# bepu/bepuphysics2

Measured on NVIDIA H100. Metric: constraint-iterations/sec (solver+integrator), higher is better.
Workload: dtype f32

## Files before the change

### bepuphysics2_b200/csrc/bepu_contacts.cuh

```cuda
#pragma once
#include "bepu_device_math.cuh"

namespace BEPU_NS {

constexpr int kLanes = 32;

struct GlobalRows { const float* ptr; };
struct GlobalAcc { float* ptr; };
struct StagedRows { uint32_t addr, bar, parity; };
struct StagedAcc { uint32_t addr; float* ptr; };
BEPU_DI float lds_f32(uint32_t addr) {
    float v;
    asm("ld.shared.f32 %0, [%1];" : "=f"(v) : "r"(addr));
    return v;
}
BEPU_DI void rows_ready(GlobalRows) {}
BEPU_DI void rows_ready(StagedRows p) {
    asm volatile(
        "{\n"
        ".reg .pred p;\n"
        "MBAR_WAIT:\n"
        "mbarrier.try_wait.parity.shared::cta.b64 p, [%0], %1;\n"
        "@p bra MBAR_DONE;\n"
        "bra MBAR_WAIT;\n"
        "MBAR_DONE:\n"
        "}\n" ::"r"(p.bar), "r"(p.parity)
        : "memory");
}
BEPU_DI float ldrow(const float* p, int r) { return __ldcg(p + r * kLanes); }
BEPU_DI float ldrow(GlobalRows p, int r) { return __ldcg(p.ptr + r * kLanes); }
BEPU_DI float ldrow(StagedRows p, int r) { return lds_f32(p.addr + r * (kLanes * 4)); }
template <class PR> BEPU_DI V3 ldrow3(PR p, int r) { return {ldrow(p, r), ldrow(p, r + 1), ldrow(p, r + 2)}; }
template <class PR> BEPU_DI Q4 ldrow4(PR p, int r) { return {ldrow(p, r), ldrow(p, r + 1), ldrow(p, r + 2), ldrow(p, r + 3)}; }
BEPU_DI float ldacc(GlobalAcc a, int r) { return a.ptr[r * kLanes]; }
BEPU_DI void stacc(GlobalAcc a, int r, float v) { a.ptr[r * kLanes] = v; }
BEPU_DI float ldacc(StagedAcc a, int r) { return lds_f32(a.addr + r * (kLanes * 4)); }
BEPU_DI void stacc(StagedAcc a, int r, float v) { __stcs(a.ptr + r * kLanes, v); }

BEPU_DI void penetration_apply(const Inertia& iA, const Inertia& iB, V3 normal, V3 angularA, V3 angularB, float impulse, Velocity& vA, Velocity& vB) {
    V3 dLinA = normal * (impulse * iA.inv_mass);
    V3 dAngA = transform(angularA * impulse, iA.t);
    V3 dLinB = normal * (impulse * iB.inv_mass);
    V3 dAngB = transform(angularB * impulse, iB.t);
    vA.lin = vA.lin + dLinA;
    vA.ang = vA.ang + dAngA;
    vB.lin = vB.lin - dLinB;
    vB.ang = vB.ang + dAngB;
}
BEPU_DI void penetration_warm_start(const Inertia& iA, const Inertia& iB, V3 normal, V3 offsetA, V3 offsetB, float accumulated, Velocity& vA, Velocity& vB) {
    penetration_apply(iA, iB, normal, cross(offsetA, normal), cross(normal, offsetB), accumulated, vA, vB);
}
BEPU_DI void penetration_solve(const Inertia& iA, const Inertia& iB, V3 normal, V3 offsetA, V3 offsetB, float depth, const Springiness& sp, float maxRecovery,
                               float inverseDt, float& accumulated, Velocity& vA, Velocity& vB) {
    V3 angularA = cross(offsetA, normal);
    V3 angularB = cross(normal, offsetB);
    float angularA0 = vector_sandwich(angularA, iA.t);
    float angularB0 = vector_sandwich(angularB, iB.t);
    float linear = iA.inv_mass + iB.inv_mass;
    float effectiveMass = sp.effective_mass_cfm_scale / (linear + angularA0 + angularB0);
    float biasVelocity = fmin_ps(depth * inverseDt, fmin_ps(depth * sp.position_error_to_velocity, maxRecovery));
    float csvaLinear = dot(vA.lin, normal);
    float csvaAngular = dot(vA.ang, angularA);
    float negatedCSVBLinear = dot(vB.lin, normal);
    float csvbAngular = dot(vB.ang, angularB);
    float negatedCSI = accumulated * sp.softness_impulse_scale + (csvaLinear - negatedCSVBLinear + csvaAngular + csvbAngular - biasVelocity) * effectiveMass;
    float previous = accumulated;
    accumulated = fmax_ps(0.0f, accumulated - negatedCSI);
    penetration_apply(iA, iB, normal, angularA, angularB, accumulated - previous, vA, vB);
}
BEPU_DI float updated_depth(float dt, V3 contactOffsetA, V3 offsetB, V3 normal, const Velocity& vA, const Velocity& vB, float depth) {
    V3 contactVelocityA = cross(vA.ang, contactOffsetA) + vA.lin;
    V3 contactOffsetB = contactOffsetA - offsetB;
    V3 contactVelocityB = cross(vB.ang, contactOffsetB) + vB.lin;
    float estimatedDepthChangeVelocity = dot(normal, contactVelocityA - contactVelocityB);
    return depth - estimatedDepthChangeVelocity * dt;
}

BEPU_DI void penetration1_apply(const Inertia& iA, V3 normal, V3 angularA, float impulse, Velocity& vA) {
    V3 dLinA = normal * (impulse * iA.inv_mass);
    V3 dAngA = transform(angularA * impulse, iA.t);
    vA.lin = vA.lin + dLinA;
    vA.ang = vA.ang + dAngA;
}
BEPU_DI void penetration1_solve(const Inertia& iA, V3 normal, V3 offsetA, float depth, const Springiness& sp, float maxRecovery, float inverseDt, float& accumulated,
                                Velocity& vA) {
    V3 angularA = cross(offsetA, normal);
    float angularA0 = vector_sandwich(angularA, iA.t);
    float effectiveMass = sp.effective_mass_cfm_scale / (iA.inv_mass + angularA0);
    float biasVelocity = fmin_ps(depth * inverseDt, fmin_ps(depth * sp.position_error_to_velocity, maxRecovery));
    float csvaLinear = dot(vA.lin, normal);
    float csvaAngular = dot(vA.ang, angularA);
    float negatedCSI = accumulated * sp.softness_impulse_scale + (csvaLinear + csvaAngular - biasVelocity) * effectiveMass;
    float previous = accumulated;
    accumulated = fmax_ps(0.0f, accumulated - negatedCSI);
    penetration1_apply(iA, normal, angularA, accumulated - previous, vA);
}
BEPU_DI float updated_depth1(float dt, V3 contactOffset, V3 normal, const Velocity& v, float depth) {
    V3 contactVelocity = cross(v.ang, contactOffset) + v.lin;
    return depth - dot(normal, contactVelocity) * dt;
}

struct TangentJacobians { M23 linearA, angularA, angularB; };
BEPU_DI TangentJacobians tangent_jacobians(V3 tX, V3 tY, V3 offsetA, V3 offsetB) {
    TangentJacobians j;
    j.linearA = {tX, tY};
    j.angularA = {cross(offsetA, tX), cross(offsetA, tY)};
    j.angularB = {cross(tX, offsetB), cross(tY, offsetB)};
    return j;
}
BEPU_DI void tangent_apply(const TangentJacobians& j, const Inertia& iA, const Inertia& iB, V2 impulse, Velocity& vA, Velocity& vB) {
    V3 linearImpulseA = transform(impulse, j.linearA);
    V3 angularImpulseA = transform(impulse, j.angularA);
    V3 angularImpulseB = transform(impulse, j.angularB);
    vA.lin = vA.lin + linearImpulseA * iA.inv_mass;
    vA.ang = vA.ang + transform(angularImpulseA, iA.t);
    vB.lin = vB.lin - linearImpulseA * iB.inv_mass;
    vB.ang = vB.ang + transform(angularImpulseB, iB.t);
}
BEPU_DI void tangent_solve(V3 tX, V3 tY, V3 offsetA, V3 offsetB, const Inertia& iA, const Inertia& iB, float maximumImpulse, V2& accumulated, Velocity& vA, Velocity& vB) {
    TangentJacobians j = tangent_jacobians(tX, tY, offsetA, offsetB);
    Sym2 linear = sandwich_scale(j.linearA, iA.inv_mass) + sandwich_scale(j.linearA, iB.inv_mass);
    Sym2 angular = matrix_sandwich(j.angularA, iA.t) + matrix_sandwich(j.angularB, iB.t);
    Sym2 effectiveMass = invert(linear + angular);
    V2 csvaLinear = transform_by_transpose(vA.lin, j.linearA);
    V2 csvaAngular = transform_by_transpose(vA.ang, j.angularA);
    V2 csvbLinear = transform_by_transpose(vB.lin, j.linearA);
    V2 csvbAngular = transform_by_transpose(vB.ang, j.angularB);
    V2 csv = (csvbLinear - csvaLinear) - (csvaAngular + csvbAngular);
    V2 csi = transform(csv, effectiveMass);
    V2 previous = accumulated;
    accumulated = accumulated + csi;
    float magnitude = length(accumulated);
    float scl = fmin_ps(1.0f, maximumImpulse / fmax_ps(1e-16f, magnitude));
    accumulated = accumulated * scl;
    tangent_apply(j, iA, iB, accumulated - previous, vA, vB);
}
BEPU_DI void tangent1_apply(const M23& linearA, const M23& angularA, const Inertia& iA, V2 impulse, Velocity& vA) {
    V3 linearImpulseA = transform(impulse, linearA);
    V3 angularImpulseA = transform(impulse, angularA);
    vA.lin = vA.lin + linearImpulseA * iA.inv_mass;
    vA.ang = vA.ang + transform(angularImpulseA, iA.t);
}
BEPU_DI void tangent1_solve(V3 tX, V3 tY, V3 offsetA, const Inertia& iA, float maximumImpulse, V2& accumulated, Velocity& vA) {
    M23 linearA{tX, tY};
    M23 angularA{cross(offsetA, tX), cross(offsetA, tY)};
    Sym2 effectiveMass = invert(sandwich_scale(linearA, iA.inv_mass) + matrix_sandwich(angularA, iA.t));
    V2 csv = transform_by_transpose(vA.lin, linearA) + transform_by_transpose(vA.ang, angularA);
    V2 negativeCSI = transform(csv, effectiveMass);
    V2 previous = accumulated;
    accumulated = accumulated - negativeCSI;
    float magnitude = length(accumulated);
    float scl = fmin_ps(1.0f, maximumImpulse / fmax_ps(1e-16f, magnitude));
    accumulated = accumulated * scl;
    tangent1_apply(linearA, angularA, iA, accumulated - previous, vA);
}

BEPU_DI void twist_apply(V3 axis, const Inertia& iA, const Inertia& iB, float impulse, Velocity& vA, Velocity& vB) {
    V3 worldImpulseA = axis * impulse;
    vA.ang = vA.ang + transform(worldImpulseA, iA.t);
    vB.ang = vB.ang - transform(worldImpulseA, iB.t);
}
BEPU_DI void twist_solve(V3 axis, const Inertia& iA, const Inertia& iB, float maximumImpulse, float& accumulated, Velocity& vA, Velocity& vB) {
    float inverseEffectiveMass = vector_sandwich(axis, iA.t) + vector_sandwich(axis, iB.t);
    float effectiveMass = (0.0f == inverseEffectiveMass) ? 0.0f : 1.0f / inverseEffectiveMass;
    float negatedCSI = (dot(vA.ang, axis) - dot(vB.ang, axis)) * effectiveMass;
    float previous = accumulated;
    accumulated = fmin_ps(maximumImpulse, fmax_ps(-maximumImpulse, accumulated - negatedCSI));
    twist_apply(axis, iA, iB, accumulated - previous, vA, vB);
}
BEPU_DI void twist1_apply(V3 axis, const Inertia& iA, float impulse, Velocity& vA) { vA.ang = vA.ang + transform(axis * impulse, iA.t); }
BEPU_DI void twist1_solve(V3 axis, const Inertia& iA, float maximumImpulse, float& accumulated, Velocity& vA) {
    float angularA = vector_sandwich(axis, iA.t);
    float effectiveMass = (0.0f == angularA) ? 0.0f : 1.0f / angularA;
    float negativeCSI = dot(vA.ang, axis) * effectiveMass;
    float previous = accumulated;
    accumulated = fmin_ps(maximumImpulse, fmax_ps(-maximumImpulse, accumulated - negativeCSI));
    twist1_apply(axis, iA, accumulated - previous, vA);
}

template <int N, bool TwoBody> struct ConvexLayout {
    static constexpr int kOffsetB = 4 * N;
    static constexpr int kNormal = TwoBody ? 4 * N + 3 : 4 * N;
    static constexpr int kFriction = kNormal + 3;
    static constexpr int kAngularFrequency = kNormal + 4;
    static constexpr int kTwiceDampingRatio = kNormal + 5;
    static constexpr int kMaxRecovery = kNormal + 6;
    static constexpr int kPrestepRows = kNormal + 7;
    static constexpr int kImpulseRows = N + 3;
};

template <int N> BEPU_DI V3 friction_center(const V3 (&offs)[N], const float (&depths)[N]) {
    float w[N];
#pragma unroll
    for (int i = 0; i < N; ++i) w[i] = depths[i] < 0.0f ? 0.0f : 1.0f;
    float weightSum = w[0];
#pragma unroll
    for (int i = 1; i < N; ++i) weightSum = weightSum + w[i];
    bool useFallback = weightSum == 0.0f;
    weightSum = useFallback ? (float)N : weightSum;
    float inverseWeightSum = 1.0f / weightSum;
    V3 c[N];
#pragma unroll
    for (int i = 0; i < N; ++i) c[i] = offs[i] * (useFallback ? inverseWeightSum : w[i] * inverseWeightSum);
    if constexpr (N == 2) return c[0] + c[1];
    else if constexpr (N == 3) return (c[0] + c[1]) + c[2];
    else return (c[0] + c[1]) + (c[2] + c[3]);
}

template <int N> struct ConvexTwoBody {
    typedef ConvexLayout<N, true> L;
    static constexpr int kBodies = 2;
    static constexpr int kPrestepRows = L::kPrestepRows;
    static constexpr int kImpulseRows = L::kImpulseRows;
    static constexpr bool kIncremental = true;
    static constexpr bool kNeedsPose = false;

    template <class PR, class AR> BEPU_DI static void warm_start(const Inertia& iA, const Inertia& iB, PR p, AR a, Velocity& vA, Velocity& vB) {
        V3 normal = ldrow3(p, L::kNormal), offsetB = ldrow3(p, L::kOffsetB);
        V3 x, z;
        build_orthonormal_basis(normal, x, z);
        V3 offs[N];
        float depths[N];
#pragma unroll
        for (int i = 0; i < N; ++i) { offs[i] = ldrow3(p, 4 * i); depths[i] = ldrow(p, 4 * i + 3); }
        V3 centerA;
        if constexpr (N == 1) centerA = offs[0]; else centerA = friction_center<N>(offs, depths);
        V3 centerB = centerA - offsetB;
        tangent_apply(tangent_jacobians(x, z, centerA, centerB), iA, iB, V2{ldacc(a, 0), ldacc(a, 1)}, vA, vB);
#pragma unroll 1
        for (int i = 0; i < N; ++i) {
            V3 offset = ldrow3(p, 4 * i);
            penetration_warm_start(iA, iB, normal, offset, offset - offsetB, ldacc(a, 2 + i), vA, vB);
        }
        twist_apply(normal, iA, iB, ldacc(a, N + 2), vA, vB);
    }
    template <class PR, class AR> BEPU_DI static void solve(const Inertia& iA, const Inertia& iB, float dt, float inverseDt, PR p, AR a, Velocity& vA, Velocity& vB) {
        V3 normal = ldrow3(p, L::kNormal), offsetB = ldrow3(p, L::kOffsetB);
        float friction = ldrow(p, L::kFriction), maxRecovery = ldrow(p, L::kMaxRecovery);
        Springiness sp = compute_springiness(ldrow(p, L::kAngularFrequency), ldrow(p, L::kTwiceDampingRatio), dt);
        if constexpr (N > 1) {
            V3 offs[N];
            float depths[N];
#pragma unroll
            for (int i = 0; i < N; ++i) { offs[i] = ldrow3(p, 4 * i); depths[i] = ldrow(p, 4 * i + 3); }
            const V3 centerA = friction_center<N>(offs, depths);
            float penSum = 0.0f, twistSum = 0.0f;
#pragma unroll 1
            for (int i = 0; i < N; ++i) {
                V3 offset = ldrow3(p, 4 * i);
                float pen = ldacc(a, 2 + i);
                penetration_solve(iA, iB, normal, offset, offset - offsetB, ldrow(p, 4 * i + 3), sp, maxRecovery, inverseDt, pen, vA, vB);
                stacc(a, 2 + i, pen);
                const float lever = pen * distance(centerA, offset);
                penSum = i == 0 ? pen : penSum + pen;
                twistSum = i == 0 ? lever : twistSum + lever;
            }
            V3 x, z;
            build_orthonormal_basis(normal, x, z);
            V2 tangent{ldacc(a, 0), ldacc(a, 1)};
            float twist = ldacc(a, N + 2);
            const float premultiplied = (1.0f / N) * friction;
            tangent_solve(x, z, centerA, centerA - offsetB, iA, iB, premultiplied * penSum, tangent, vA, vB);
            twist_solve(normal, iA, iB, premultiplied * twistSum, twist, vA, vB);
            stacc(a, 0, tangent.x);
            stacc(a, 1, tangent.y);
            stacc(a, N + 2, twist);
        } else
        {
        V3 offs[N];
        float depths[N], pen[N];
#pragma unroll
        for (int i = 0; i < N; ++i) { offs[i] = ldrow3(p, 4 * i); depths[i] = ldrow(p, 4 * i + 3); pen[i] = ldacc(a, 2 + i); }
#pragma unroll
        for (int i = 0; i < N; ++i) penetration_solve(iA, iB, normal, offs[i], offs[i] - offsetB, depths[i], sp, maxRecovery, inverseDt, pen[i], vA, vB);
        V3 x, z;
        build_orthonormal_basis(normal, x, z);
        V2 tangent{ldacc(a, 0), ldacc(a, 1)};
        float twist = ldacc(a, N + 2);
        if constexpr (N == 1) {
            float maximumTangentImpulse = friction * pen[0];
            tangent_solve(x, z, offs[0], offs[0] - offsetB, iA, iB, maximumTangentImpulse, tangent, vA, vB);
            float maximumTwistImpulse = friction * pen[0] * fmax_ps(0.0f, depths[0]);
            twist_solve(normal, iA, iB, maximumTwistImpulse, twist, vA, vB);
        } else {
            float premultiplied = (1.0f / N) * friction;
            float penSum = pen[0];
#pragma unroll
            for (int i = 1; i < N; ++i) penSum = penSum + pen[i];
            V3 centerA = friction_center<N>(offs, depths);
            tangent_solve(x, z, centerA, centerA - offsetB, iA, iB, premultiplied * penSum, tangent, vA, vB);
            float twistSum = pen[0] * distance(centerA, offs[0]);
#pragma unroll
            for (int i = 1; i < N; ++i) twistSum = twistSum + pen[i] * distance(centerA, offs[i]);
            twist_solve(normal, iA, iB, premultiplied * twistSum, twist, vA, vB);
        }
        stacc(a, 0, tangent.x);
        stacc(a, 1, tangent.y);
#pragma unroll
        for (int i = 0; i < N; ++i) stacc(a, 2 + i, pen[i]);
        stacc(a, N + 2, twist);
        }
    }
    BEPU_DI static void incremental_update(float dt, const Velocity& vA, const Velocity& vB, float* p) {
        V3 normal = ldrow3(p, L::kNormal), offsetB = ldrow3(p, L::kOffsetB);
#pragma unroll
        for (int i = 0; i < N; ++i) p[(4 * i + 3) * kLanes] = updated_depth(dt, ldrow3(p, 4 * i), offsetB, normal, vA, vB, ldrow(p, 4 * i + 3));
    }
};

template <int N> struct ConvexOneBody {
    typedef ConvexLayout<N, false> L;
    static constexpr int kBodies = 1;
    static constexpr int kPrestepRows = L::kPrestepRows;
    static constexpr int kImpulseRows = L::kImpulseRows;
    static constexpr bool kIncremental = true;
    static constexpr bool kNeedsPose = false;

    template <class PR, class AR> BEPU_DI static void warm_start(const Inertia& iA, PR p, AR a, Velocity& vA) {
        V3 normal = ldrow3(p, L::kNormal);
        V3 x, z;
        build_orthonormal_basis(normal, x, z);
        V3 offs[N];
        float depths[N];
#pragma unroll
        for (int i = 0; i < N; ++i) { offs[i] = ldrow3(p, 4 * i); depths[i] = ldrow(p, 4 * i + 3); }
        V3 centerA;
        if constexpr (N == 1) centerA = offs[0]; else centerA = friction_center<N>(offs, depths);
        tangent1_apply(M23{x, z}, M23{cross(centerA, x), cross(centerA, z)}, iA, V2{ldacc(a, 0), ldacc(a, 1)}, vA);
#pragma unroll 1
        for (int i = 0; i < N; ++i) penetration1_apply(iA, normal, cross(ldrow3(p, 4 * i), normal), ldacc(a, 2 + i), vA);
        twist1_apply(normal, iA, ldacc(a, N + 2), vA);
    }
    template <class PR, class AR> BEPU_DI static void solve(const Inertia& iA, float dt, float inverseDt, PR p, AR a, Velocity& vA) {
        V3 normal = ldrow3(p, L::kNormal);
        float friction = ldrow(p, L::kFriction), maxRecovery = ldrow(p, L::kMaxRecovery);
        Springiness sp = compute_springiness(ldrow(p, L::kAngularFrequency), ldrow(p, L::kTwiceDampingRatio), dt);
        if constexpr (N > 1) {
            V3 offs[N];
            float depths[N];
#pragma unroll
            for (int i = 0; i < N; ++i) { offs[i] = ldrow3(p, 4 * i); depths[i] = ldrow(p, 4 * i + 3); }
            const V3 centerA = friction_center<N>(offs, depths);
            float penSum = 0.0f, twistSum = 0.0f;
#pragma unroll 1
            for (int i = 0; i < N; ++i) {
                V3 offset = ldrow3(p, 4 * i);
                float pen = ldacc(a, 2 + i);
                penetration1_solve(iA, normal, offset, ldrow(p, 4 * i + 3), sp, maxRecovery, inverseDt, pen, vA);
                stacc(a, 2 + i, pen);
                const float lever = pen * distance(centerA, offset);
                penSum = i == 0 ? pen : penSum + pen;
                twistSum = i == 0 ? lever : twistSum + lever;
            }
            V3 x, z;
            build_orthonormal_basis(normal, x, z);
            V2 tangent{ldacc(a, 0), ldacc(a, 1)};
            float twist = ldacc(a, N + 2);
            const float premultiplied = (1.0f / N) * friction;
            tangent1_solve(x, z, centerA, iA, premultiplied * penSum, tangent, vA);
            twist1_solve(normal, iA, premultiplied * twistSum, twist, vA);
            stacc(a, 0, tangent.x);
            stacc(a, 1, tangent.y);
            stacc(a, N + 2, twist);
        } else
        {
        V3 offs[N];
        float depths[N], pen[N];
#pragma unroll
        for (int i = 0; i < N; ++i) { offs[i] = ldrow3(p, 4 * i); depths[i] = ldrow(p, 4 * i + 3); pen[i] = ldacc(a, 2 + i); }
#pragma unroll
        for (int i = 0; i < N; ++i) penetration1_solve(iA, normal, offs[i], depths[i], sp, maxRecovery, inverseDt, pen[i], vA);
        V3 x, z;
        build_orthonormal_basis(normal, x, z);
        V2 tangent{ldacc(a, 0), ldacc(a, 1)};
        float twist = ldacc(a, N + 2);
        if constexpr (N == 1) {
            tangent1_solve(x, z, offs[0], iA, friction * pen[0], tangent, vA);
            twist1_solve(normal, iA, friction * pen[0] * fmax_ps(0.0f, depths[0]), twist, vA);
        } else {
            float premultiplied = (1.0f / N) * friction;
            float penSum = pen[0];
#pragma unroll
            for (int i = 1; i < N; ++i) penSum = penSum + pen[i];
            V3 centerA = friction_center<N>(offs, depths);
            tangent1_solve(x, z, centerA, iA, premultiplied * penSum, tangent, vA);
            float twistSum = pen[0] * distance(centerA, offs[0]);
#pragma unroll
            for (int i = 1; i < N; ++i) twistSum = twistSum + pen[i] * distance(centerA, offs[i]);
            twist1_solve(normal, iA, premultiplied * twistSum, twist, vA);
        }
        stacc(a, 0, tangent.x);
        stacc(a, 1, tangent.y);
#pragma unroll
        for (int i = 0; i < N; ++i) stacc(a, 2 + i, pen[i]);
        stacc(a, N + 2, twist);
        }
    }
    BEPU_DI static void incremental_update(float dt, const Velocity& vA, float* p) {
        V3 normal = ldrow3(p, L::kNormal);
#pragma unroll
        for (int i = 0; i < N; ++i) p[(4 * i + 3) * kLanes] = updated_depth1(dt, ldrow3(p, 4 * i), normal, vA, ldrow(p, 4 * i + 3));
    }
};

#define BEPU_CONTACT_LOOP _Pragma("unroll 1")
template <int N, bool TwoBody> struct NonconvexLayout {
    static constexpr int kOffsetB = 4;
    static constexpr int kContacts = TwoBody ? 7 : 4;
    static constexpr int kPrestepRows = kContacts + 7 * N;
    static constexpr int kImpulseRows = 3 * N;
};
template <int N> struct NonconvexTwoBody {
    typedef NonconvexLayout<N, true> L;
    static constexpr int kBodies = 2;
    static constexpr int kPrestepRows = L::kPrestepRows;
    static constexpr int kImpulseRows = L::kImpulseRows;
    static constexpr bool kIncremental = true;
    static constexpr bool kNeedsPose = false;
    template <class PR, class AR> BEPU_DI static void warm_start(const Inertia& iA, const Inertia& iB, PR p, AR a, Velocity& vA, Velocity& vB) {
        V3 offsetB = ldrow3(p, L::kOffsetB);
BEPU_CONTACT_LOOP
        for (int i = 0; i < N; ++i) {
            const int c = L::kContacts + 7 * i;
            V3 offset = ldrow3(p, c), normal = ldrow3(p, c + 4);
            V3 x, z;
            build_orthonormal_basis(normal, x, z);
            V3 contactOffsetB = offset - offsetB;
            tangent_apply(tangent_jacobians(x, z, offset, contactOffsetB), iA, iB, V2{ldacc(a, 3 * i), ldacc(a, 3 * i + 1)}, vA, vB);
            penetration_warm_start(iA, iB, normal, offset, contactOffsetB, ldacc(a, 3 * i + 2), vA, vB);
        }
    }
    template <class PR, class AR> BEPU_DI static void solve(const Inertia& iA, const Inertia& iB, float dt, float inverseDt, PR p, AR a, Velocity& vA, Velocity& vB) {
        V3 offsetB = ldrow3(p, L::kOffsetB);
        float friction = ldrow(p, 0), maxRecovery = ldrow(p, 3);
        Springiness sp = compute_springiness(ldrow(p, 1), ldrow(p, 2), dt);
BEPU_CONTACT_LOOP
        for (int i = 0; i < N; ++i) {
            const int c = L::kContacts + 7 * i;
            V3 offset = ldrow3(p, c), normal = ldrow3(p, c + 4);
            float depth = ldrow(p, c + 3);
            V2 tangent{ldacc(a, 3 * i), ldacc(a, 3 * i + 1)};
            float pen = ldacc(a, 3 * i + 2);
            V3 contactOffsetB = offset - offsetB;
            penetration_solve(iA, iB, normal, offset, contactOffsetB, depth, sp, maxRecovery, inverseDt, pen, vA, vB);
            V3 x, z;
            build_orthonormal_basis(normal, x, z);
            tangent_solve(x, z, offset, contactOffsetB, iA, iB, friction * pen, tangent, vA, vB);
            stacc(a, 3 * i, tangent.x);
            stacc(a, 3 * i + 1, tangent.y);
            stacc(a, 3 * i + 2, pen);
        }
    }
    BEPU_DI static void incremental_update(float dt, const Velocity& vA, const Velocity& vB, float* p) {
        V3 offsetB = ldrow3(p, L::kOffsetB);
#pragma unroll
        for (int i = 0; i < N; ++i) {
            const int c = L::kContacts + 7 * i;
            p[(c + 3) * kLanes] = updated_depth(dt, ldrow3(p, c), offsetB, ldrow3(p, c + 4), vA, vB, ldrow(p, c + 3));
        }
    }
};
template <int N> struct NonconvexOneBody {
    typedef NonconvexLayout<N, false> L;
    static constexpr int kBodies = 1;
    static constexpr int kPrestepRows = L::kPrestepRows;
    static constexpr int kImpulseRows = L::kImpulseRows;
    static constexpr bool kIncremental = true;
    static constexpr bool kNeedsPose = false;
    template <class PR, class AR> BEPU_DI static void warm_start(const Inertia& iA, PR p, AR a, Velocity& vA) {
BEPU_CONTACT_LOOP
        for (int i = 0; i < N; ++i) {
            const int c = L::kContacts + 7 * i;
            V3 offset = ldrow3(p, c), normal = ldrow3(p, c + 4);
            V3 x, z;
            build_orthonormal_basis(normal, x, z);
            tangent1_apply(M23{x, z}, M23{cross(offset, x), cross(offset, z)}, iA, V2{ldacc(a, 3 * i), ldacc(a, 3 * i + 1)}, vA);
            penetration1_apply(iA, normal, cross(offset, normal), ldacc(a, 3 * i + 2), vA);
        }
    }
    template <class PR, class AR> BEPU_DI static void solve(const Inertia& iA, float dt, float inverseDt, PR p, AR a, Velocity& vA) {
        float friction = ldrow(p, 0), maxRecovery = ldrow(p, 3);
        Springiness sp = compute_springiness(ldrow(p, 1), ldrow(p, 2), dt);
BEPU_CONTACT_LOOP
        for (int i = 0; i < N; ++i) {
            const int c = L::kContacts + 7 * i;
            V3 offset = ldrow3(p, c), normal = ldrow3(p, c + 4);
            float depth = ldrow(p, c + 3);
            V2 tangent{ldacc(a, 3 * i), ldacc(a, 3 * i + 1)};
            float pen = ldacc(a, 3 * i + 2);
            penetration1_solve(iA, normal, offset, depth, sp, maxRecovery, inverseDt, pen, vA);
            V3 x, z;
            build_orthonormal_basis(normal, x, z);
            tangent1_solve(x, z, offset, iA, friction * pen, tangent, vA);
            stacc(a, 3 * i, tangent.x);
            stacc(a, 3 * i + 1, tangent.y);
            stacc(a, 3 * i + 2, pen);
        }
    }
    BEPU_DI static void incremental_update(float dt, const Velocity& vA, float* p) {
#pragma unroll
        for (int i = 0; i < N; ++i) {
            const int c = L::kContacts + 7 * i;
            p[(c + 3) * kLanes] = updated_depth1(dt, ldrow3(p, c), ldrow3(p, c + 4), vA, ldrow(p, c + 3));
        }
    }
};

}
```

### bepuphysics2_b200/csrc/bepu_device_types.h

```cpp
#pragma once
#include <cuda_runtime.h>
#include <stdint.h>

namespace bepucuda {

constexpr uint32_t kRefIndexMask = 0x0FFFFFFFu;
constexpr uint32_t kRefBundleIntegratesBit = 1u << 28;
constexpr uint32_t kRefIntegrateBit = 1u << 29;
constexpr uint32_t kRefKinematicBit = 1u << 30;
constexpr int32_t kRefEmpty = -1;

struct BodyBuffers {
    float4* pose;
    float4* velocity;
    float4* inertia_local;
    float4* inertia_world;
    const uint8_t* constrained;
    int32_t count;
};

struct DeviceTypeBatch {
    int32_t type_id;
    int32_t bundle_count;
    int32_t device_batch;
    int32_t pad;
    int32_t* refs;
    float* prestep;
    float* impulses;
};

struct FrameParams {
    float dt;
    float inverse_dt;
    float gravity_dt[3];
    float linear_damping_dt;
    float angular_damping_dt;
    float final_dt;
    float final_gravity_dt[3];
    float final_linear_damping_dt;
    float final_angular_damping_dt;
    int32_t final_steps;
    int32_t angular_mode;
    int32_t integrate_velocity_for_kinematics;
    uint32_t exchange_base;
    uint32_t shard_solve_index;
    int32_t tune[4];
};

enum Stage : int32_t {
    kStageWarmStartFirst = 0,
    kStageWarmStart = 1,
    kStageSolve = 2,
    kStageIncremental = 3,
    kStageKinematicFirst = 4,
    kStageKinematic = 5,
    kStageFinalPose = 6,
};

struct WorkItem {
    int32_t type_batch;
    int32_t bundle;
};

struct alignas(32) WorkRecord {
    int32_t* refs;
    float* prestep;
    float* impulses;
    int32_t type_id;
    int32_t live_lanes;
};

struct StageOp {
    int32_t stage;
    int32_t work_begin;
    int32_t work_count;
    int32_t pad;
};

constexpr int kMaxShardRanks = 8;
struct ShardPeers {
    float4* pose[kMaxShardRanks];
    float4* velocity[kMaxShardRanks];
    float4* inertia_world[kMaxShardRanks];
    unsigned long long* flags[kMaxShardRanks];
    int32_t rank, rank_count;
};
struct ShardStage {
    uint32_t exchange_index;
    int32_t* error_flag;
};
constexpr int kShardCounterSlot = 16;
constexpr int kShardTargetSlot = 32;
constexpr int kShardMaxExchanges = 4096;
constexpr size_t kShardFlagBlockWords = kShardTargetSlot + (size_t)kMaxShardRanks * kShardMaxExchanges;
constexpr int32_t kRecordBoundaryBit = 1 << 30;
constexpr uint32_t kPushOwnerBit = 1u << 31;

struct TypeInfo {
    int32_t bodies, prestep_rows, impulse_rows, incremental;
    int32_t solve_bytes, warm_start_bytes, incremental_bytes;
    const char* name;
};
const TypeInfo* get_type_info(int type_id);

}
```

### bepuphysics2_b200/csrc/bepu_layout_kernels.h

```cpp
#pragma once
#include "bepu_device_types.h"

namespace bepucuda {

void launch_split_bodies(const void* raw, int body_count, const BodyBuffers& B, cudaStream_t s);
void launch_merge_bodies(void* raw, int body_count, const BodyBuffers& B, cudaStream_t s);
struct TransposeDesc {
    int32_t* src_refs;
    float* src_prestep;
    float* src_impulses;
    const int32_t* map;
    int32_t src_count;
    int32_t bodies, prestep_rows, impulse_rows;
    int32_t src_bundle_base;
    int32_t flags;
    const int32_t* features_old;
    const int32_t* features_new;
};
constexpr int32_t kDescResidentImpulses = 1, kDescRedistribute = 2;
enum { kTransposeRefs = 1, kTransposePrestep = 2, kTransposeImpulses = 4 };
void launch_transpose_in_all(const DeviceTypeBatch* tbs, const TransposeDesc* descs, const WorkItem* work, int work_count, int W, int what, cudaStream_t s);
void launch_transpose_out_all(const DeviceTypeBatch* tbs, const TransposeDesc* descs, const WorkItem* work, int work_count, int W, int what, cudaStream_t s);
void launch_fill_i32(int32_t* p, size_t n, int32_t v, cudaStream_t s);
void launch_redistribute_impulses(const DeviceTypeBatch* tbs, const TransposeDesc* descs, const WorkItem* work, int work_count, cudaStream_t s);
void launch_scatter_body_motion(const void* raw, int body_count, const BodyBuffers& B, cudaStream_t s);
void launch_gather_body_motion(void* raw, int body_count, const BodyBuffers& B, cudaStream_t s);
struct CopyChunk {
    void* dst;
    const void* src;
    size_t bytes;
};
void launch_batched_copy(const CopyChunk* chunks, int chunk_count, cudaStream_t s);
void launch_ownership_pass1(const DeviceTypeBatch* tbs, const WorkItem* work, int work_count, const int32_t* bodies_per_type, int sync_batch_count, int body_count,
                            int32_t* first_batch, int32_t* sync_refcount, unsigned long long* sync_mask, int32_t* error_flag, cudaStream_t s);
void launch_ownership_rest(const DeviceTypeBatch* tbs, const WorkItem* work, int work_count, const int32_t* bodies_per_type, int body_count, const int32_t* first_batch,
                           const int32_t* sync_refcount, const unsigned long long* sync_mask, uint8_t* constrained, const int32_t* kinematics, int kinematic_count,
                           int32_t* error_flag, const TransposeDesc* descs, int W, int32_t* source_bundle_flags, cudaStream_t s);
void launch_collect_stage(const DeviceTypeBatch* tbs, const WorkItem* work, int work_count, const int32_t* bodies_per_type, int stage, const BodyBuffers& B, int32_t* staging,
                          cudaStream_t s);
void launch_apply_stage(const int32_t* staging, int planes, const BodyBuffers& B, cudaStream_t s);
void launch_widen_u8(const uint8_t* in, int32_t* out, size_t n, cudaStream_t s);
void launch_narrow_i32(const int32_t* in, uint8_t* out, size_t n, cudaStream_t s);

void launch_shard_exchange(const uint32_t* pushes, int push_count, int what, const BodyBuffers& B, const ShardPeers& peers, const FrameParams* fp, uint32_t exchange_index,
                           int32_t* error_flag, cudaStream_t s);

void launch_fill_peer_masks(const int32_t* refs, uint32_t* peer_masks, size_t count, const uint8_t* body_masks, int rank, cudaStream_t s);
void launch_boundary_flags(const WorkRecord* records, int count, const int32_t* bodies_per_type, long long peer_delta, uint8_t* flags, cudaStream_t s);

void launch_pack_ref_rows(const WorkRecord* records, int count, int32_t* rows, cudaStream_t s);

constexpr int kLaunchPdl = 1, kLaunchPrefetchRows = 2;
struct SolverLaunchers {
    void (*constraint_stage)(int stage, const WorkRecord* records, const int32_t* ref_rows, int work_count, const BodyBuffers& B, const FrameParams* fp, int launch_flags, cudaStream_t s);
    void (*kinematic_stage)(int stage, const int32_t* kinematics, int count, const BodyBuffers& B, const FrameParams* fp, cudaStream_t s);
    void (*final_pose)(const BodyBuffers& B, const FrameParams* fp, cudaStream_t s);
    void (*constraint_stage_sharded)(int stage, const WorkRecord* records, const int32_t* ref_rows, int work_count, const BodyBuffers& B, const FrameParams* fp, int launch_flags, const ShardPeers& peers,
                                     long long peer_delta, const ShardStage& shard, cudaStream_t s);
};
const SolverLaunchers* get_launchers_bepu_fast();
const SolverLaunchers* get_launchers_bepu_strict();

}
```

### bepuphysics2_b200/csrc/bepu_solver_kernels.cu

```cuda
#include <atomic>
#include "bepu_solver_kernels.cuh"
#include "bepu_layout_kernels.h"

namespace BEPU_NS {

void launch_stage_warm_start_first(const WorkRecord* records, const int32_t* ref_rows, int work_count, const BodyBuffers& B, const FrameParams* fp, int launch_flags, cudaStream_t s);
void launch_stage_warm_start(const WorkRecord* records, const int32_t* ref_rows, int work_count, const BodyBuffers& B, const FrameParams* fp, int launch_flags, cudaStream_t s);
void launch_stage_solve(const WorkRecord* records, const int32_t* ref_rows, int work_count, const BodyBuffers& B, const FrameParams* fp, int launch_flags, cudaStream_t s);
void launch_stage_warm_start_first_sharded(const WorkRecord* records, const int32_t* ref_rows, int work_count, const BodyBuffers& B, const FrameParams* fp, int launch_flags, const ShardPeers& peers, long long peer_delta, const ShardStage& shard, cudaStream_t s);
void launch_stage_warm_start_sharded(const WorkRecord* records, const int32_t* ref_rows, int work_count, const BodyBuffers& B, const FrameParams* fp, int launch_flags, const ShardPeers& peers, long long peer_delta, const ShardStage& shard, cudaStream_t s);
void launch_stage_solve_sharded(const WorkRecord* records, const int32_t* ref_rows, int work_count, const BodyBuffers& B, const FrameParams* fp, int launch_flags, const ShardPeers& peers, long long peer_delta, const ShardStage& shard, cudaStream_t s);

#ifndef BEPU_DEEP_MINB
#define BEPU_DEEP_MINB 12
#endif
constexpr int kDeepBatchBundles = 2150;
template <int STAGE, int MINB>
static void launch_stage_variant(const WorkRecord* records, const int32_t* ref_rows, int work_count, const BodyBuffers& B, const FrameParams* fp, int launch_flags, cudaStream_t s) {
    static std::atomic<bool> carveout_set[64] = {};
    int device = 0;
    cudaGetDevice(&device);
    if (!carveout_set[device & 63]) {
        cudaFuncSetAttribute(constraint_stage_kernel<STAGE, MINB>, cudaFuncAttributePreferredSharedMemoryCarveout, cudaSharedmemCarveoutMaxShared);
        carveout_set[device & 63] = true;
    }
    const unsigned blocks = (unsigned)(((size_t)work_count * 32 + kStageBlockThreads - 1) / kStageBlockThreads);
    cudaLaunchConfig_t cfg{};
    cfg.gridDim = dim3(blocks);
    cfg.blockDim = dim3(kStageBlockThreads);
    cfg.dynamicSmemBytes = 0;
    cfg.stream = s;
    cudaLaunchAttribute attr[1];
    attr[0].id = cudaLaunchAttributeProgrammaticStreamSerialization;
    attr[0].val.programmaticStreamSerializationAllowed = 1;
    cfg.attrs = attr;
    cfg.numAttrs = (launch_flags & bepucuda::kLaunchPdl) ? 1 : 0;
    cudaLaunchKernelEx(&cfg, constraint_stage_kernel<STAGE, MINB>, records, ref_rows, work_count, B, fp, (launch_flags & bepucuda::kLaunchPrefetchRows) ? kStagePrefetchRows : 0);
}
template <int STAGE, int MINB>
static void launch_stage_variant_sharded(const WorkRecord* records, const int32_t* ref_rows, int work_count, const BodyBuffers& B, const FrameParams* fp, int launch_flags, const ShardPeers& peers, long long peer_delta,
                                         const ShardStage& shard, cudaStream_t s) {
    static std::atomic<bool> carveout_set[64] = {};
    int device = 0;
    cudaGetDevice(&device);
    if (!carveout_set[device & 63]) {
        cudaFuncSetAttribute(constraint_stage_kernel_sharded<STAGE, MINB>, cudaFuncAttributePreferredSharedMemoryCarveout, cudaSharedmemCarveoutMaxShared);
        carveout_set[device & 63] = true;
    }
    const unsigned blocks = (unsigned)(((size_t)work_count * 32 + kStageBlockThreads - 1) / kStageBlockThreads);
    cudaLaunchConfig_t cfg{};
    cfg.gridDim = dim3(blocks);
    cfg.blockDim = dim3(kStageBlockThreads);
    cfg.stream = s;
    cudaLaunchAttribute attr[1];
    attr[0].id = cudaLaunchAttributeProgrammaticStreamSerialization;
    attr[0].val.programmaticStreamSerializationAllowed = 1;
    cfg.attrs = attr;
    cfg.numAttrs = (launch_flags & bepucuda::kLaunchPdl) ? 1 : 0;
    cudaLaunchKernelEx(&cfg, constraint_stage_kernel_sharded<STAGE, MINB>, records, ref_rows, work_count, B, fp, (launch_flags & bepucuda::kLaunchPrefetchRows) ? kStagePrefetchRows : 0, peers,
                       peer_delta, shard);
}
template <int STAGE>
static void launch_stage_sharded_t(const WorkRecord* records, const int32_t* ref_rows, int work_count, const BodyBuffers& B, const FrameParams* fp, int launch_flags, const ShardPeers& peers, long long peer_delta,
                                   const ShardStage& shard, cudaStream_t s) {
    if (work_count >= kDeepBatchBundles) launch_stage_variant_sharded<STAGE, BEPU_DEEP_MINB>(records, ref_rows, work_count, B, fp, launch_flags, peers, peer_delta, shard, s);
    else launch_stage_variant_sharded<STAGE, 1>(records, ref_rows, work_count, B, fp, launch_flags, peers, peer_delta, shard, s);
}
template <int STAGE>
static void launch_stage_t(const WorkRecord* records, const int32_t* ref_rows, int work_count, const BodyBuffers& B, const FrameParams* fp, int launch_flags, cudaStream_t s) {
    if (STAGE != kStageIncremental && work_count >= kDeepBatchBundles) launch_stage_variant<STAGE, BEPU_DEEP_MINB>(records, ref_rows, work_count, B, fp, launch_flags, s);
    else launch_stage_variant<STAGE, 1>(records, ref_rows, work_count, B, fp, launch_flags, s);
}

#if BEPU_UNIT == 0
void launch_stage_warm_start_first(const WorkRecord* records, const int32_t* ref_rows, int work_count, const BodyBuffers& B, const FrameParams* fp, int launch_flags, cudaStream_t s) {
    launch_stage_t<kStageWarmStartFirst>(records, ref_rows, work_count, B, fp, launch_flags, s);
}
void launch_stage_warm_start_first_sharded(const WorkRecord* records, const int32_t* ref_rows, int work_count, const BodyBuffers& B, const FrameParams* fp, int launch_flags, const ShardPeers& peers, long long peer_delta, const ShardStage& shard, cudaStream_t s) {
    launch_stage_sharded_t<kStageWarmStartFirst>(records, ref_rows, work_count, B, fp, launch_flags, peers, peer_delta, shard, s);
}
#elif BEPU_UNIT == 1
void launch_stage_warm_start(const WorkRecord* records, const int32_t* ref_rows, int work_count, const BodyBuffers& B, const FrameParams* fp, int launch_flags, cudaStream_t s) {
    launch_stage_t<kStageWarmStart>(records, ref_rows, work_count, B, fp, launch_flags, s);
}
void launch_stage_warm_start_sharded(const WorkRecord* records, const int32_t* ref_rows, int work_count, const BodyBuffers& B, const FrameParams* fp, int launch_flags, const ShardPeers& peers, long long peer_delta, const ShardStage& shard, cudaStream_t s) {
    launch_stage_sharded_t<kStageWarmStart>(records, ref_rows, work_count, B, fp, launch_flags, peers, peer_delta, shard, s);
}
#elif BEPU_UNIT == 2
void launch_stage_solve(const WorkRecord* records, const int32_t* ref_rows, int work_count, const BodyBuffers& B, const FrameParams* fp, int launch_flags, cudaStream_t s) {
    launch_stage_t<kStageSolve>(records, ref_rows, work_count, B, fp, launch_flags, s);
}
void launch_stage_solve_sharded(const WorkRecord* records, const int32_t* ref_rows, int work_count, const BodyBuffers& B, const FrameParams* fp, int launch_flags, const ShardPeers& peers, long long peer_delta, const ShardStage& shard, cudaStream_t s) {
    launch_stage_sharded_t<kStageSolve>(records, ref_rows, work_count, B, fp, launch_flags, peers, peer_delta, shard, s);
}
#elif BEPU_UNIT == 3
static void launch_constraint_stage(int stage, const WorkRecord* records, const int32_t* ref_rows, int work_count, const BodyBuffers& B, const FrameParams* fp, int launch_flags, cudaStream_t s) {
    if (work_count <= 0) return;
    switch (stage) {
        case kStageWarmStartFirst: launch_stage_warm_start_first(records, ref_rows, work_count, B, fp, launch_flags, s); break;
        case kStageWarmStart: launch_stage_warm_start(records, ref_rows, work_count, B, fp, launch_flags, s); break;
        case kStageSolve: launch_stage_solve(records, ref_rows, work_count, B, fp, launch_flags, s); break;
        case kStageIncremental: launch_stage_t<kStageIncremental>(records, ref_rows, work_count, B, fp, launch_flags, s); break;
        default: break;
    }
}
static void launch_constraint_stage_sharded(int stage, const WorkRecord* records, const int32_t* ref_rows, int work_count, const BodyBuffers& B, const FrameParams* fp, int launch_flags, const ShardPeers& peers,
                                            long long peer_delta, const ShardStage& shard, cudaStream_t s) {
    if (work_count <= 0) return;
    switch (stage) {
        case kStageWarmStartFirst: launch_stage_warm_start_first_sharded(records, ref_rows, work_count, B, fp, launch_flags, peers, peer_delta, shard, s); break;
        case kStageWarmStart: launch_stage_warm_start_sharded(records, ref_rows, work_count, B, fp, launch_flags, peers, peer_delta, shard, s); break;
        case kStageSolve: launch_stage_solve_sharded(records, ref_rows, work_count, B, fp, launch_flags, peers, peer_delta, shard, s); break;
        default: break;
    }
}
static void launch_kinematic_stage(int stage, const int32_t* kinematics, int count, const BodyBuffers& B, const FrameParams* fp, cudaStream_t s) {
    if (count <= 0) return;
    const unsigned blocks = (unsigned)((count + 127) / 128);
    if (stage == kStageKinematicFirst) kinematic_stage_kernel<kStageKinematicFirst><<<blocks, 128, 0, s>>>(kinematics, count, B, fp);
    else kinematic_stage_kernel<kStageKinematic><<<blocks, 128, 0, s>>>(kinematics, count, B, fp);
}
static void launch_final_pose(const BodyBuffers& B, const FrameParams* fp, cudaStream_t s) {
    if (B.count <= 0) return;
    final_pose_kernel<<<(unsigned)((B.count + 255) / 256), 256, 0, s>>>(B, fp);
}
static const bepucuda::SolverLaunchers kLaunchers = {&launch_constraint_stage, &launch_kinematic_stage, &launch_final_pose, &launch_constraint_stage_sharded};
#else
#error "BEPU_UNIT must be 0..3"
#endif

}

#if BEPU_UNIT == 3
namespace bepucuda {
#define BEPU_CAT2(a, b) a##b
#define BEPU_CAT(a, b) BEPU_CAT2(a, b)
const SolverLaunchers* BEPU_CAT(get_launchers_, BEPU_NS)() { return &BEPU_NS::kLaunchers; }
}
#endif
```

### bepuphysics2_b200/csrc/bepu_solver_kernels.cuh

```cuda
#pragma once
#include "bepu_contacts.cuh"
#include "bepu_joints_more.cuh"
#include "bepu_integration.cuh"
#include "bepu_device_types.h"

namespace BEPU_NS {

using namespace bepucuda;

struct F8 { float a, b, c, d, e, f, g, h; };
#define BEPU_BODY_LD "ld.global.L1::no_allocate.L2::cache_hint.v4.f32"
#define BEPU_BODY_ST "st.global.L1::no_allocate.L2::cache_hint.v4.f32"
BEPU_DI uint64_t l2_evict_last_policy() {
    uint64_t policy;
    asm("createpolicy.fractional.L2::evict_last.b64 %0, 1.0;" : "=l"(policy));
    return policy;
}
BEPU_DI F8 ld256(const float4* p) {
    F8 r;
    asm volatile(BEPU_BODY_LD " {%0,%1,%2,%3}, [%8], %9;\n\t" BEPU_BODY_LD " {%4,%5,%6,%7}, [%8+16], %9;"
                 : "=f"(r.a), "=f"(r.b), "=f"(r.c), "=f"(r.d), "=f"(r.e), "=f"(r.f), "=f"(r.g), "=f"(r.h)
                 : "l"(p), "l"(l2_evict_last_policy())
                 : "memory");
    return r;
}
BEPU_DI void st256(float4* p, float a, float b, float c, float d, float e, float f, float g, float h) {
    asm volatile(BEPU_BODY_ST " [%0], {%1,%2,%3,%4}, %9;\n\t" BEPU_BODY_ST " [%0+16], {%5,%6,%7,%8}, %9;" ::"l"(p), "f"(a), "f"(b), "f"(c), "f"(d), "f"(e), "f"(f), "f"(g), "f"(h),
                 "l"(l2_evict_last_policy())
                 : "memory");
}
BEPU_DI void load_velocity(const float4* vel, uint32_t i, Velocity& v) {
    const F8 r = ld256(vel + 2 * (size_t)i);
    v.lin = {r.a, r.b, r.c};
    v.ang = {r.e, r.f, r.g};
}
BEPU_DI void store_velocity(float4* vel, uint32_t i, const Velocity& v) { st256(vel + 2 * (size_t)i, v.lin.x, v.lin.y, v.lin.z, 0.0f, v.ang.x, v.ang.y, v.ang.z, 0.0f); }
BEPU_DI void load_inertia(const float4* in, uint32_t i, Inertia& r) {
    const F8 x = ld256(in + 2 * (size_t)i);
    r.t = {x.a, x.b, x.c, x.d, x.e, x.f};
    r.inv_mass = x.g;
}
BEPU_DI void store_inertia(float4* in, uint32_t i, const Inertia& r) { st256(in + 2 * (size_t)i, r.t.xx, r.t.yx, r.t.yy, r.t.zx, r.t.zy, r.t.zz, r.inv_mass, 0.0f); }
BEPU_DI void load_pose(const float4* pose, uint32_t i, V3& pos, Q4& q) {
    const F8 x = ld256(pose + 2 * (size_t)i);
    q = {x.a, x.b, x.c, x.d};
    pos = {x.e, x.f, x.g};
}
BEPU_DI void store_pose(float4* pose, uint32_t i, V3 pos, Q4 q) { st256(pose + 2 * (size_t)i, q.x, q.y, q.z, q.w, pos.x, pos.y, pos.z, 0.0f); }

template <int STAGE, bool NeedsPose>
BEPU_DI void warm_start_body(uint32_t enc, const BodyBuffers& B, const FrameParams& fp, BodyState& b, Velocity& v) {
    const uint32_t idx = enc & kRefIndexMask;
    if (enc & kRefIntegrateBit) {
        Inertia local;
        load_inertia(B.inertia_local, idx, local);
        load_pose(B.pose, idx, b.pos, b.q);
        b.inertia.inv_mass = local.inv_mass;
        if (STAGE == kStageWarmStart) {
            b.pos = b.pos + v.lin * fp.dt;
            Q4 previousOrientation = b.q;
            b.q = integrate_orientation(b.q, v.ang, fp.dt * 0.5f);
            b.inertia.t = rotate_inverse_inertia(local.t, b.q);
            if (fp.angular_mode == 1) integrate_angular_conserve_momentum(previousOrientation, local.t, b.inertia.t, v.ang);
            else if (fp.angular_mode == 2) integrate_angular_gyroscopic(b.q, local.t, v.ang, fp.dt);
            store_pose(B.pose, idx, b.pos, b.q);
        } else {
            b.inertia.t = rotate_inverse_inertia(local.t, b.q);
            if (fp.angular_mode == 1) {
                Q4 previousOrientation = integrate_orientation(b.q, v.ang, fp.dt * -0.5f);
                integrate_angular_conserve_momentum(previousOrientation, local.t, b.inertia.t, v.ang);
            } else if (fp.angular_mode == 2) {
                integrate_angular_gyroscopic(b.q, local.t, v.ang, fp.dt);
            }
        }
        callback_integrate_velocity(v, fp.gravity_dt[0], fp.gravity_dt[1], fp.gravity_dt[2], fp.linear_damping_dt, fp.angular_damping_dt);
        store_inertia(B.inertia_world, idx, b.inertia);
    } else {
        load_inertia(B.inertia_world, idx, b.inertia);
        if (NeedsPose) load_pose(B.pose, idx, b.pos, b.q);
        if (STAGE == kStageWarmStartFirst && fp.angular_mode != 0 && (enc & kRefBundleIntegratesBit) && !(enc & kRefKinematicBit)) {
            Inertia local;
            load_inertia(B.inertia_local, idx, local);
            V3 pos;
            Q4 q;
            load_pose(B.pose, idx, pos, q);
            if (fp.angular_mode == 1) integrate_angular_conserve_momentum(integrate_orientation(q, v.ang, fp.dt * -0.5f), local.t, b.inertia.t, v.ang);
            else integrate_angular_gyroscopic(q, local.t, v.ang, fp.dt);
        }
    }
}
template <int STAGE, bool NeedsPose>
BEPU_DI void gather_for_warm_start(uint32_t enc, const BodyBuffers& B, const FrameParams& fp, BodyState& b, Velocity& v) {
    load_velocity(B.velocity, enc & kRefIndexMask, v);
    warm_start_body<STAGE, NeedsPose>(enc, B, fp, b, v);
}

template <class T, class PR, class AR> BEPU_DI void call_warm_start(const BodyState* b, PR p, AR a, Velocity* v) {
    if constexpr (T::kNeedsPose) T::warm_start(b, p, a, v);
    else if constexpr (T::kBodies == 2) T::warm_start(b[0].inertia, b[1].inertia, p, a, v[0], v[1]);
    else T::warm_start(b[0].inertia, p, a, v[0]);
}
template <class T, class PR, class AR> BEPU_DI void call_solve(const BodyState* b, float dt, float inverseDt, PR p, AR a, Velocity* v) {
    if constexpr (T::kNeedsPose) T::solve(b, dt, inverseDt, p, a, v);
    else if constexpr (T::kBodies == 2) T::solve(b[0].inertia, b[1].inertia, dt, inverseDt, p, a, v[0], v[1]);
    else T::solve(b[0].inertia, dt, inverseDt, p, a, v[0]);
}
template <class T> BEPU_DI void call_incremental(float dt, const Velocity* v, float* p) {
    if constexpr (T::kIncremental) {
        if constexpr (T::kBodies == 2) T::incremental_update(dt, v[0], v[1], p);
        else T::incremental_update(dt, v[0], p);
    }
}

BEPU_DI uint32_t ldg_nc_u32(const void* p) {
    uint32_t v;
    asm volatile("ld.global.nc.u32 %0, [%1];" : "=r"(v) : "l"(p));
    return v;
}
BEPU_DI void push_record(float4* const* arrays, uint32_t mask, uint32_t idx, float a, float b, float c, float d, float e, float f, float g, float h) {
    while (mask) {
        const int q = __ffs((int)mask) - 1;
        mask &= mask - 1u;
        float4* dst = arrays[q] + 2 * (size_t)idx;
        dst[0] = make_float4(a, b, c, d);
        dst[1] = make_float4(e, f, g, h);
    }
}
template <class T, int STAGE, bool kSharded, class PR, class AR>
BEPU_DI void run_lane(const int32_t* refs, PR p, AR a, float* p_rw, uint32_t enc0, uint32_t enc1, const BodyBuffers& B, const FrameParams& fp, const ShardPeers* peers = nullptr,
                      long long peer_delta = 0) {
    constexpr int NB = T::kBodies;
    uint32_t enc[NB];
    enc[0] = enc0;
    if constexpr (NB > 1) enc[1] = enc1;
#pragma unroll
    for (int s = 2; s < NB; ++s) enc[s] = (uint32_t)__ldg(refs + s * kLanes);
    uint32_t push_to[kSharded ? NB : 1];
    if constexpr (kSharded) {
#pragma unroll
        for (int s = 0; s < NB; ++s) push_to[s] = peer_delta != 0 ? ldg_nc_u32(refs + peer_delta + s * kLanes) : 0u;
    }
    if ((int32_t)enc[0] == kRefEmpty) return;
    BodyState b[NB];
    Velocity v[NB];
    if constexpr (STAGE == kStageIncremental) {
#pragma unroll
        for (int s = 0; s < NB; ++s) load_velocity(B.velocity, enc[s] & kRefIndexMask, v[s]);
        call_incremental<T>(fp.dt, v, p_rw);
    } else if constexpr (STAGE == kStageSolve) {
#pragma unroll
        for (int s = 0; s < NB; ++s) {
            const uint32_t idx = enc[s] & kRefIndexMask;
            load_velocity(B.velocity, idx, v[s]);
            load_inertia(B.inertia_world, idx, b[s].inertia);
            if (T::kNeedsPose) load_pose(B.pose, idx, b[s].pos, b[s].q);
        }
        rows_ready(p);
        call_solve<T>(b, fp.dt, fp.inverse_dt, p, a, v);
#pragma unroll
        for (int s = 0; s < NB; ++s)
            if (!(enc[s] & kRefKinematicBit)) {
                store_velocity(B.velocity, enc[s] & kRefIndexMask, v[s]);
                if constexpr (kSharded) {
                    const uint32_t mask = push_to[s];
                    if (mask) push_record(peers->velocity, mask, enc[s] & kRefIndexMask, v[s].lin.x, v[s].lin.y, v[s].lin.z, 0.0f, v[s].ang.x, v[s].ang.y, v[s].ang.z, 0.0f);
                }
            }
    } else {
#pragma unroll
        for (int s = 0; s < NB; ++s) gather_for_warm_start<STAGE, T::kNeedsPose>(enc[s], B, fp, b[s], v[s]);
        rows_ready(p);
        call_warm_start<T>(b, p, a, v);
#pragma unroll
        for (int s = 0; s < NB; ++s)
            if (!(enc[s] & kRefKinematicBit)) {
                const uint32_t idx = enc[s] & kRefIndexMask;
                store_velocity(B.velocity, idx, v[s]);
                if constexpr (kSharded) {
                    const uint32_t mask = push_to[s];
                    if (mask) {
                        push_record(peers->velocity, mask, idx, v[s].lin.x, v[s].lin.y, v[s].lin.z, 0.0f, v[s].ang.x, v[s].ang.y, v[s].ang.z, 0.0f);
                        if (enc[s] & kRefIntegrateBit) {
                            const Inertia& in = b[s].inertia;
                            push_record(peers->inertia_world, mask, idx, in.t.xx, in.t.yx, in.t.yy, in.t.zx, in.t.zy, in.t.zz, in.inv_mass, 0.0f);
                            if (STAGE == kStageWarmStart) push_record(peers->pose, mask, idx, b[s].q.x, b[s].q.y, b[s].q.z, b[s].q.w, b[s].pos.x, b[s].pos.y, b[s].pos.z, 0.0f);
                        }
                    }
                }
            }
    }
}
template <class T, int STAGE, class PR, class AR>
BEPU_DI void run_lane(const int32_t* refs, PR p, AR a, float* p_rw, uint32_t enc0, uint32_t enc1, const BodyBuffers& B, const FrameParams& fp) {
    run_lane<T, STAGE, false>(refs, p, a, p_rw, enc0, enc1, B, fp);
}

BEPU_DI int4 ldg_nc_v4(const void* p) {
    int4 v;
    asm volatile("ld.global.nc.v4.s32 {%0,%1,%2,%3}, [%4];" : "=r"(v.x), "=r"(v.y), "=r"(v.z), "=r"(v.w) : "l"(p));
    return v;
}
BEPU_DI WorkRecord load_record(const WorkRecord* r) {
    const int4 lo = ldg_nc_v4(r), hi = ldg_nc_v4(reinterpret_cast<const int4*>(r) + 1);
    WorkRecord w;
    w.refs = reinterpret_cast<int32_t*>((unsigned long long)(unsigned int)lo.x | ((unsigned long long)(unsigned int)lo.y << 32));
    w.prestep = reinterpret_cast<float*>((unsigned long long)(unsigned int)lo.z | ((unsigned long long)(unsigned int)lo.w << 32));
    w.impulses = reinterpret_cast<float*>((unsigned long long)(unsigned int)hi.x | ((unsigned long long)(unsigned int)hi.y << 32));
    w.type_id = hi.z;
    w.live_lanes = hi.w;
    return w;
}

#define BEPU_CONTACT_TYPES(X)                                                                                                     \
    X(0, ConvexOneBody<1>) X(1, ConvexOneBody<2>) X(2, ConvexOneBody<3>) X(3, ConvexOneBody<4>)                                   \
    X(4, ConvexTwoBody<1>) X(5, ConvexTwoBody<2>) X(6, ConvexTwoBody<3>) X(7, ConvexTwoBody<4>)                                   \
    X(8, NonconvexOneBody<2>) X(9, NonconvexOneBody<3>) X(10, NonconvexOneBody<4>)                                                \
    X(15, NonconvexTwoBody<2>) X(16, NonconvexTwoBody<3>) X(17, NonconvexTwoBody<4>)

template <int STAGE, bool kSharded, class PR, class AR>
BEPU_DI void run_bundle_rows(const WorkRecord& rec, int lane, PR p, AR a, uint32_t enc0, uint32_t enc1, const BodyBuffers& B, const FrameParams& fp, const ShardPeers* peers = nullptr,
                             long long peer_delta = 0) {
    const int32_t* refs = rec.refs + lane;
    float* p_rw = rec.prestep + lane;
    switch (rec.type_id) {
#define BEPU_CASE(ID, T) \
    case ID: run_lane<T, STAGE, kSharded>(refs, p, a, p_rw, enc0, enc1, B, fp, peers, peer_delta); break;
        BEPU_CONTACT_TYPES(BEPU_CASE)
        BEPU_JOINT_TYPES(BEPU_CASE)
        BEPU_JOINT_TYPES_MORE(BEPU_CASE)
#undef BEPU_CASE
        default: break;
    }
}
template <int STAGE, class PR, class AR>
BEPU_DI void run_bundle_rows(const WorkRecord& rec, int lane, PR p, AR a, uint32_t enc0, uint32_t enc1, const BodyBuffers& B, const FrameParams& fp) {
    run_bundle_rows<STAGE, false>(rec, lane, p, a, enc0, enc1, B, fp);
}
template <int STAGE>
BEPU_DI void run_bundle(const WorkRecord& rec, int lane, uint32_t enc0, uint32_t enc1, const BodyBuffers& B, const FrameParams& fp) {
    run_bundle_rows<STAGE>(rec, lane, GlobalRows{rec.prestep + lane}, GlobalAcc{rec.impulses + lane}, enc0, enc1, B, fp);
}
template <int STAGE> BEPU_DI void run_bundle(const WorkRecord& rec, int lane, const BodyBuffers& B, const FrameParams& fp) {
    const uint32_t enc0 = ldg_nc_u32(rec.refs + lane), enc1 = ldg_nc_u32(rec.refs + kLanes + lane);
    run_bundle<STAGE>(rec, lane, enc0, enc1, B, fp);
}

struct StageRowCounts { uint8_t prestep[64], impulses[64]; };
__host__ __device__ constexpr StageRowCounts make_stage_row_counts() {
    StageRowCounts c{};
#define BEPU_ROWS(ID, T) c.prestep[ID] = (uint8_t)T::kPrestepRows; c.impulses[ID] = (uint8_t)T::kImpulseRows;
    BEPU_CONTACT_TYPES(BEPU_ROWS)
    BEPU_JOINT_TYPES(BEPU_ROWS)
    BEPU_JOINT_TYPES_MORE(BEPU_ROWS)
#undef BEPU_ROWS
    return c;
}
__constant__ StageRowCounts kStageRowCounts = make_stage_row_counts();
constexpr int kStageSlabRows = 48;
constexpr int kStageSlabBytes = kStageSlabRows * kLanes * 4;

BEPU_DI uint32_t smem_u32(const void* p) { return (uint32_t)__cvta_generic_to_shared(p); }
BEPU_DI void mbar_init(uint32_t bar, uint32_t count) {
    asm volatile("mbarrier.init.shared::cta.b64 [%0], %1;" ::"r"(bar), "r"(count) : "memory");
    asm volatile("fence.mbarrier_init.release.cluster;" ::: "memory");
    asm volatile("fence.proxy.async.shared::cta;" ::: "memory");
}
BEPU_DI void mbar_expect_tx(uint32_t bar, uint32_t bytes) { asm volatile("mbarrier.arrive.expect_tx.shared::cta.b64 _, [%0], %1;" ::"r"(bar), "r"(bytes) : "memory"); }
BEPU_DI uint64_t l2_evict_first_policy() {
    uint64_t policy;
    asm volatile("createpolicy.fractional.L2::evict_first.b64 %0, 1.0;" : "=l"(policy));
    return policy;
}
BEPU_DI void bulk_copy_g2s(uint32_t dst, const void* src, uint32_t bytes, uint32_t bar, uint64_t policy) {
    asm volatile("cp.async.bulk.shared::cluster.global.mbarrier::complete_tx::bytes.L2::cache_hint [%0], [%1], %2, [%3], %4;" ::"r"(dst), "l"(src), "r"(bytes), "r"(bar),
                 "l"(policy)
                 : "memory");
}

#ifndef BEPU_STAGE_BLOCK_THREADS
#define BEPU_STAGE_BLOCK_THREADS 64
#endif
constexpr int kStageBlockThreads = BEPU_STAGE_BLOCK_THREADS;

constexpr int kStagePrefetchRows = 1;
BEPU_DI void shard_announce(const ShardPeers& peers, int lane) {
    if (lane < peers.rank_count && lane != peers.rank)
        asm volatile("red.release.sys.global.add.u64 [%0], 1;" ::"l"(peers.flags[lane] + kShardCounterSlot + peers.rank) : "memory");
}
BEPU_DI void shard_wait(const ShardPeers& peers, int lane, uint32_t solve_index, uint32_t exchange_point, int32_t* error_flag) {
    if (lane < peers.rank_count && lane != peers.rank) {
        const unsigned long long* mine = peers.flags[peers.rank];
        const unsigned long long* targets = mine + kShardTargetSlot + (size_t)lane * kShardMaxExchanges;
        const unsigned long long want = (unsigned long long)solve_index * targets[kShardMaxExchanges - 1] + targets[exchange_point];
        unsigned long long seen;
        unsigned int spins = 0;
        do {
            asm volatile("ld.acquire.sys.global.u64 %0, [%1];" : "=l"(seen) : "l"(mine + kShardCounterSlot + lane) : "memory");
        } while (seen < want && ++spins < 100000000u);
        if (seen < want) atomicExch(error_flag, 5);
    }
    __syncwarp();
}
template <int STAGE, bool kSharded>
BEPU_DI void constraint_stage_body(const WorkRecord* __restrict__ records, const int32_t* __restrict__ ref_rows, int work_count, const BodyBuffers& B, const FrameParams* __restrict__ fpp, int flags, const ShardPeers* peers,
                                   long long peer_delta, const ShardStage* shard = nullptr) {
    constexpr bool kStaged = STAGE != kStageIncremental;
    constexpr int kWarps = kStageBlockThreads / 32;
    __shared__ __align__(128) float slab[kStaged ? kWarps * kStageSlabRows * kLanes : 1];
    __shared__ __align__(8) unsigned long long bars[kWarps];
    const int warp_in_block = threadIdx.x >> 5;
    const int global_warp = (blockIdx.x * kStageBlockThreads + threadIdx.x) >> 5;
    const int lane = threadIdx.x & 31;
    WorkRecord rec{};
    uint32_t enc0 = (uint32_t)kRefEmpty, enc1 = 0;
    const int warp = global_warp;
    const bool active = warp < work_count;
    const uint32_t slab_addr = kStaged ? smem_u32(slab) + warp_in_block * kStageSlabBytes : 0;
    const uint32_t bar = smem_u32(&bars[warp_in_block]);
    const bool early_rows = kStaged && (flags & kStagePrefetchRows);
    uint32_t prestep_bytes = 0, impulse_bytes = 0;
    if (active) {
        rec = load_record(records + warp);
        if constexpr (kStaged) {
            prestep_bytes = kStageRowCounts.prestep[rec.type_id] * (kLanes * 4);
            impulse_bytes = kStageRowCounts.impulses[rec.type_id] * (kLanes * 4);
            if (lane == 0) {
                mbar_init(bar, 1);
                if (early_rows) {
                    const uint64_t policy = l2_evict_first_policy();
                    mbar_expect_tx(bar, prestep_bytes + impulse_bytes);
                    bulk_copy_g2s(slab_addr, rec.prestep, prestep_bytes, bar, policy);
                    bulk_copy_g2s(slab_addr + prestep_bytes, rec.impulses, impulse_bytes, bar, policy);
                }
            }
        }
        enc0 = ldg_nc_u32(ref_rows + (size_t)warp * (2 * kLanes) + lane);
        enc1 = ldg_nc_u32(ref_rows + (size_t)warp * (2 * kLanes) + kLanes + lane);
    }
    const FrameParams fp = *fpp;
    asm volatile("griddepcontrol.wait;" ::: "memory");
    asm volatile("griddepcontrol.launch_dependents;");
    bool boundary = false;
    if constexpr (kSharded) {
        boundary = active && (rec.live_lanes & kRecordBoundaryBit) != 0;
        if (boundary && shard->exchange_index > 0 && !(fp.tune[0] & 1)) shard_wait(*peers, lane, fp.shard_solve_index, shard->exchange_index - 1u, shard->error_flag);
    }
    if (!active) return;
    if constexpr (kStaged) {
        if (!early_rows && lane == 0) {
            const uint64_t policy = l2_evict_first_policy();
            mbar_expect_tx(bar, prestep_bytes + impulse_bytes);
            bulk_copy_g2s(slab_addr, rec.prestep, prestep_bytes, bar, policy);
            bulk_copy_g2s(slab_addr + prestep_bytes, rec.impulses, impulse_bytes, bar, policy);
        }
        __syncwarp();
        run_bundle_rows<STAGE, kSharded>(rec, lane, StagedRows{slab_addr + lane * 4, bar, 0u}, StagedAcc{slab_addr + prestep_bytes + lane * 4, rec.impulses + lane}, enc0, enc1, B, fp,
                                         peers, boundary && !(fp.tune[0] & 4) ? peer_delta : 0);
        if constexpr (kSharded) {
            if (boundary && !(fp.tune[0] & 2)) {
                __syncwarp();
                shard_announce(*peers, lane);
            }
        }
    } else {
        run_bundle<STAGE>(rec, lane, enc0, enc1, B, fp);
    }
}

template <int STAGE, int MINB>
__global__ void __launch_bounds__(kStageBlockThreads, MINB) constraint_stage_kernel(const WorkRecord* __restrict__ records, const int32_t* __restrict__ ref_rows, int work_count, BodyBuffers B, const FrameParams* __restrict__ fpp, int flags) {
    constraint_stage_body<STAGE, false>(records, ref_rows, work_count, B, fpp, flags, nullptr, 0);
}
template <int STAGE, int MINB>
__global__ void __launch_bounds__(kStageBlockThreads, MINB)
constraint_stage_kernel_sharded(const WorkRecord* __restrict__ records, const int32_t* __restrict__ ref_rows, int work_count, BodyBuffers B, const FrameParams* __restrict__ fpp, int flags, const __grid_constant__ ShardPeers peers,
                                long long peer_delta, const __grid_constant__ ShardStage shard) {
    constraint_stage_body<STAGE, true>(records, ref_rows, work_count, B, fpp, flags, &peers, peer_delta, &shard);
}

template <int STAGE> BEPU_DI void run_kinematic(int i, const int32_t* kinematics, const BodyBuffers& B, const FrameParams& fp) {
    const uint32_t idx = (uint32_t)kinematics[i];
    Velocity v;
    load_velocity(B.velocity, idx, v);
    if (STAGE == kStageKinematic) {
        V3 pos;
        Q4 q;
        load_pose(B.pose, idx, pos, q);
        pos = pos + v.lin * fp.dt;
        q = integrate_orientation(q, v.ang, fp.dt * 0.5f);
        store_pose(B.pose, idx, pos, q);
    }
    if (fp.integrate_velocity_for_kinematics) {
        callback_integrate_velocity(v, fp.gravity_dt[0], fp.gravity_dt[1], fp.gravity_dt[2], fp.linear_damping_dt, fp.angular_damping_dt);
        store_velocity(B.velocity, idx, v);
    }
}
template <int STAGE>
__global__ void kinematic_stage_kernel(const int32_t* __restrict__ kinematics, int count, BodyBuffers B, const FrameParams* __restrict__ fpp) {
    const int i = blockIdx.x * blockDim.x + threadIdx.x;
    if (i >= count) return;
    const FrameParams fp = *fpp;
    run_kinematic<STAGE>(i, kinematics, B, fp);
}

BEPU_DI void run_final_pose(int i, const BodyBuffers& B, const FrameParams& fp) {
    V3 pos;
    Q4 q;
    Velocity v;
    load_pose(B.pose, i, pos, q);
    load_velocity(B.velocity, i, v);
    if (B.constrained[i]) {
        q = integrate_orientation(q, v.ang, fp.dt * 0.5f);
        pos = pos + v.lin * fp.dt;
        store_pose(B.pose, i, pos, q);
        return;
    }
    Inertia local;
    load_inertia(B.inertia_local, i, local);
    const bool kinematic = local.inv_mass == 0.0f && local.t.xx == 0.0f && local.t.yx == 0.0f && local.t.yy == 0.0f && local.t.zx == 0.0f && local.t.zy == 0.0f && local.t.zz == 0.0f;
    const bool integrateVelocity = fp.integrate_velocity_for_kinematics || !kinematic;
    const float dt = fp.final_dt, halfDt = fp.final_dt * 0.5f;
    for (int step = 0; step < fp.final_steps; ++step) {
        if (integrateVelocity)
            callback_integrate_velocity(v, fp.final_gravity_dt[0], fp.final_gravity_dt[1], fp.final_gravity_dt[2], fp.final_linear_damping_dt, fp.final_angular_damping_dt);
        pos = pos + v.lin * dt;
        if (fp.angular_mode == 1) {
            Q4 previousOrientation = q;
            q = integrate_orientation(q, v.ang, halfDt);
            integrate_angular_conserve_momentum(previousOrientation, local.t, rotate_inverse_inertia(local.t, q), v.ang);
        } else if (fp.angular_mode == 2) {
            q = integrate_orientation(q, v.ang, halfDt);
            integrate_angular_gyroscopic(q, local.t, v.ang, dt);
        } else {
            q = integrate_orientation(q, v.ang, halfDt);
        }
    }
    store_pose(B.pose, i, pos, q);
    if (integrateVelocity) store_velocity(B.velocity, i, v);
}
static __global__ void final_pose_kernel(BodyBuffers B, const FrameParams* __restrict__ fpp) {
    const int i = blockIdx.x * blockDim.x + threadIdx.x;
    if (i >= B.count) return;
    const FrameParams fp = *fpp;
    run_final_pose(i, B, fp);
}

}
```

### bepuphysics2_b200/csrc/bepucuda_api.cu

```cuda
#include <algorithm>
#include <cmath>
#include <cstdio>
#include <cstdlib>
#include <cstring>
#include <map>
#include <string>
#include <vector>

#include "../../include/bepucuda.h"
#include "bepu_layout_kernels.h"
#include "bepu_coloring.h"
#include "bepu_bounds.h"

using namespace bepucuda;

namespace bepucuda {

static TypeInfo make_contact(int bodies, int prestep, int impulses, int contacts, const char* name) {
    TypeInfo t{};
    t.bodies = bodies; t.prestep_rows = prestep; t.impulse_rows = impulses; t.incremental = 1; t.name = name;
    const int body_rw = 13 + 6;
    t.solve_bytes = 4 * (prestep + 2 * impulses + bodies + bodies * body_rw);
    t.warm_start_bytes = 4 * (prestep + impulses + bodies + bodies * body_rw);
    t.incremental_bytes = 4 * (prestep + contacts + bodies + 6 * bodies);
    return t;
}
static TypeInfo make_joint(int bodies, int prestep, int impulses, int solve_r, int solve_w, int ws_r, int ws_w, const char* name) {
    TypeInfo t{};
    t.bodies = bodies; t.prestep_rows = prestep; t.impulse_rows = impulses; t.incremental = 0; t.name = name;
    t.solve_bytes = 4 * (prestep + 2 * impulses + bodies + solve_r + solve_w);
    t.warm_start_bytes = 4 * (prestep + impulses + bodies + ws_r + ws_w);
    t.incremental_bytes = 0;
    return t;
}
struct Registry {
    TypeInfo types[64];
    bool present[64];
    Registry() {
        std::memset(present, 0, sizeof(present));
        auto add = [&](int id, TypeInfo t) { types[id] = t; present[id] = true; };
        add(0, make_contact(1, 11, 4, 1, "Contact1OneBody")); add(1, make_contact(1, 15, 5, 2, "Contact2OneBody"));
        add(2, make_contact(1, 19, 6, 3, "Contact3OneBody")); add(3, make_contact(1, 23, 7, 4, "Contact4OneBody"));
        add(4, make_contact(2, 14, 4, 1, "Contact1")); add(5, make_contact(2, 18, 5, 2, "Contact2"));
        add(6, make_contact(2, 22, 6, 3, "Contact3")); add(7, make_contact(2, 26, 7, 4, "Contact4"));
        add(8, make_contact(1, 18, 6, 2, "Contact2NonconvexOneBody")); add(9, make_contact(1, 25, 9, 3, "Contact3NonconvexOneBody"));
        add(10, make_contact(1, 32, 12, 4, "Contact4NonconvexOneBody"));
        add(15, make_contact(2, 21, 6, 2, "Contact2Nonconvex")); add(16, make_contact(2, 28, 9, 3, "Contact3Nonconvex"));
        add(17, make_contact(2, 35, 12, 4, "Contact4Nonconvex"));
#define BEPU_REGISTER_JOINTS
#include "bepu_joint_registry.inc"
#undef BEPU_REGISTER_JOINTS
    }
};
static const Registry& registry() {
    static Registry r;
    return r;
}
const TypeInfo* get_type_info(int type_id) {
    if (type_id < 0 || type_id >= 64 || !registry().present[type_id]) return nullptr;
    return &registry().types[type_id];
}

struct DeviceBuffer {
    void* ptr = nullptr;
    size_t capacity = 0;
    cudaError_t reserve(size_t bytes) {
        if (bytes <= capacity) return cudaSuccess;
        if (ptr) cudaFree(ptr);
        ptr = nullptr;
        capacity = 0;
        size_t want = bytes + bytes / 4 + 256;
        cudaError_t e = cudaMalloc(&ptr, want);
        if (e == cudaSuccess) capacity = want;
        return e;
    }
    void release() {
        if (ptr) cudaFree(ptr);
        ptr = nullptr;
        capacity = 0;
    }
    template <class T> T* as() const { return (T*)ptr; }
};

struct ChunkArena {
    struct Chunk { char* base; size_t size, used; };
    std::vector<Chunk> chunks;
    bool pinned_host = false;
    size_t min_chunk = (size_t)64 << 20;
    void reset() { for (auto& c : chunks) c.used = 0; }
    void* alloc(size_t bytes, cudaError_t* err) {
        bytes = (bytes + 255) & ~(size_t)255;
        for (auto& c : chunks)
            if (c.size - c.used >= bytes) {
                void* p = c.base + c.used;
                c.used += bytes;
                return p;
            }
        Chunk c{};
        c.size = std::max(bytes, min_chunk);
        cudaError_t e = pinned_host ? cudaMallocHost((void**)&c.base, c.size) : cudaMalloc((void**)&c.base, c.size);
        if (e != cudaSuccess) { if (err) *err = e; return nullptr; }
        c.used = bytes;
        chunks.push_back(c);
        return chunks.back().base;
    }
    void release() {
        for (auto& c : chunks) { if (pinned_host) cudaFreeHost(c.base); else cudaFree(c.base); }
        chunks.clear();
    }
};

struct SourceTypeBatch {
    int batch_index, type_batch_index, type_id, count;
    int live = 0;
    float* host_impulses;
    int32_t* raw_refs;
    float* raw_prestep;
    float* raw_impulses;
    size_t refs_bytes, prestep_bytes, impulse_bytes;
    std::vector<int32_t> host_refs;
    std::vector<int> device_tbs;
    int32_t* raw_features_old = nullptr;
    int32_t* raw_features_new = nullptr;
    size_t feature_bytes = 0;
    bool resident_impulses = false, redistribute = false;
};

}

struct bepucuda_ctx {
    bepucuda_config cfg{};
    int32_t tune[4] = {0, 0, 0, 0};
    int device = 0;
    cudaStream_t stream = nullptr;
    cudaEvent_t ev_solve_begin = nullptr, ev_solve_end = nullptr, ev_up_begin = nullptr, ev_up_end = nullptr, ev_down_begin = nullptr, ev_down_end = nullptr;
    bool up_open = false, have_solve = false, have_down = false, have_up = false;
    std::string error;
    const SolverLaunchers* launchers = nullptr;

    std::vector<int32_t> iterations{1};
    int fallback_threshold = 64;
    bepucuda_integrator_desc integ{};
    bool integ_set = false;

    int body_count = 0;
    DeviceBuffer raw_bodies, pose, velocity, inertia_local, inertia_world, constrained, first_batch, sync_refcount, sync_mask;
    BodyBuffers B{};

    int W = 8;
    int batch_count = 0;
    bool constraints_open = false, constraints_ready = false, data_dirty = false, descs_dirty = false;
    std::vector<SourceTypeBatch> sources;
    ChunkArena raw_arena, pinned_arena;
    DeviceBuffer record_table, ref_rows, source_bundle_flags, refs32, prestep32, impulses32, tb_table, tdesc_table, work_table, map_table, bodies_per_type, kinematics_dev, program_dev, frame_params_dev, error_dev;
    std::vector<DeviceTypeBatch> tbs;
    std::vector<TransposeDesc> tdescs;
    std::vector<WorkItem> work;
    std::vector<int32_t> bundle_live;
    std::vector<WorkRecord> records;
    std::vector<std::pair<int, int>> batch_work;
    bool exchange_failed = false;
    bepucuda_exchange_fn exchange = nullptr;
    void* exchange_user = nullptr;
    DeviceBuffer exchange_staging;
    bool peer_mode = false;
    ShardPeers peers{};
    DeviceBuffer shard_flags, pushes_dev, peer32, body_masks_dev, boundary_flags_dev;
    uint32_t shard_solve_index = 0;
    std::vector<int> boundary_count;
    std::vector<uint8_t> body_masks;
    size_t refs_words = 0;
    std::vector<void*> opened_ipc;
    std::vector<int32_t> global_first_batch;
    std::vector<uint8_t> global_constrained;
    std::map<int, std::vector<uint32_t>> pushes_by_batch;
    std::vector<std::pair<size_t, int>> push_range;
    uint32_t exchange_counter = 0;
    uint32_t exchanges_per_solve = 0;
    int inc_work_begin = 0, inc_work_count = 0;
    int all_work_count = 0;
    int sync_batch_count = 0, fallback_levels = 0;
    std::vector<int32_t> kinematics;
    std::vector<StageOp> program;
    FrameParams* frame_params_host = nullptr;

    cudaGraph_t graph = nullptr;
    cudaGraphExec_t graph_exec = nullptr;
    bool graph_valid = false;

    bepucuda_timings timings{};
    int64_t h2d_accum = 0;
    struct HostRange { char* host; size_t bytes; char* dev; };
    std::vector<HostRange> host_ranges;
    std::vector<CopyChunk> pending_h2d;
    DeviceBuffer chunk_table;
    struct ChunkStage { void* host = nullptr; size_t capacity = 0; cudaEvent_t done = nullptr; };
    ChunkStage chunk_stage[4];
    int chunk_stage_next = 0;
    cudaEvent_t user_events[16] = {};
    DeviceBuffer body_shapes, body_activities, body_bounds;
    int shape_count = -1;
    DeviceBuffer color_refs, color_priorities, color_body_min, color_body_mask, color_out, color_lists, color_counts;
    std::vector<cudaEvent_t> profile_events;
};

namespace {

int fail(bepucuda_ctx* c, int code, const std::string& msg) {
    if (c) c->error = msg;
    return code;
}
int cuda_fail(bepucuda_ctx* c, cudaError_t e, const char* what) {
    return fail(c, e == cudaErrorMemoryAllocation ? BEPUCUDA_ERR_OUT_OF_MEMORY : BEPUCUDA_ERR_CUDA, std::string(what) + ": " + cudaGetErrorString(e));
}
#define CK(call)                                                  \
    do {                                                          \
        cudaError_t _e = (call);                                  \
        if (_e != cudaSuccess) return cuda_fail(ctx, _e, #call);  \
    } while (0)

void open_upload_window(bepucuda_ctx* ctx) {
    if (!ctx->up_open) {
        cudaEventRecord(ctx->ev_up_begin, ctx->stream);
        ctx->up_open = true;
    }
}

char* map_host(bepucuda_ctx* ctx, const void* ptr, size_t bytes) {
    const char* p = (const char*)ptr;
    for (auto& r : ctx->host_ranges)
        if (p >= r.host && p + bytes <= r.host + r.bytes) return r.dev + (p - r.host);
    return nullptr;
}
void queue_chunks(std::vector<CopyChunk>& list, void* dst, const void* src, size_t bytes) {
    const size_t kChunk = (size_t)64 << 10;
    for (size_t off = 0; off < bytes; off += kChunk) list.push_back({(char*)dst + off, (const char*)src + off, std::min(kChunk, bytes - off)});
}
int flush_chunks(bepucuda_ctx* ctx, std::vector<CopyChunk>& list) {
    if (list.empty()) return BEPUCUDA_OK;
    const size_t bytes = list.size() * sizeof(CopyChunk);
    CK(ctx->chunk_table.reserve(bytes));
    auto& st = ctx->chunk_stage[ctx->chunk_stage_next];
    ctx->chunk_stage_next = (ctx->chunk_stage_next + 1) & 3;
    if (!st.done) CK(cudaEventCreateWithFlags(&st.done, cudaEventDisableTiming));
    CK(cudaEventSynchronize(st.done));
    if (st.capacity < bytes) {
        if (st.host) cudaFreeHost(st.host);
        st.host = nullptr;
        st.capacity = 0;
        CK(cudaMallocHost(&st.host, bytes * 2));
        st.capacity = bytes * 2;
    }
    std::memcpy(st.host, list.data(), bytes);
    CK(cudaMemcpyAsync(ctx->chunk_table.ptr, st.host, bytes, cudaMemcpyHostToDevice, ctx->stream));
    launch_batched_copy(ctx->chunk_table.as<CopyChunk>(), (int)list.size(), ctx->stream);
    CK(cudaGetLastError());
    CK(cudaEventRecord(st.done, ctx->stream));
    list.clear();
    return BEPUCUDA_OK;
}

int copy_in(bepucuda_ctx* ctx, void* dst, const void* src, size_t bytes) {
    if (bytes == 0) return BEPUCUDA_OK;
    if (char* alias = map_host(ctx, src, bytes)) {
        queue_chunks(ctx->pending_h2d, dst, alias, bytes);
        ctx->h2d_accum += (int64_t)bytes;
        return BEPUCUDA_OK;
    }
    if (bytes < ((size_t)256 << 10)) {
        cudaError_t e = cudaSuccess;
        void* stage = ctx->pinned_arena.alloc(bytes, &e);
        if (!stage) return cuda_fail(ctx, e, "pinned staging");
        std::memcpy(stage, src, bytes);
        CK(cudaMemcpyAsync(dst, stage, bytes, cudaMemcpyHostToDevice, ctx->stream));
    } else {
        CK(cudaMemcpyAsync(dst, src, bytes, cudaMemcpyHostToDevice, ctx->stream));
    }
    ctx->h2d_accum += (int64_t)bytes;
    return BEPUCUDA_OK;
}

void invalidate_graph(bepucuda_ctx* ctx) {
    if (ctx->graph_exec) cudaGraphExecDestroy(ctx->graph_exec);
    if (ctx->graph) cudaGraphDestroy(ctx->graph);
    ctx->graph_exec = nullptr;
    ctx->graph = nullptr;
    ctx->graph_valid = false;
}

void issue_stage_sequence(bepucuda_ctx* ctx, cudaStream_t s, int64_t* launches) {
    const WorkRecord* records = ctx->record_table.as<WorkRecord>();
    const int32_t* ref_rows = ctx->ref_rows.as<int32_t>();
    const FrameParams* fp = ctx->frame_params_dev.as<FrameParams>();
    const int32_t* kin = ctx->kinematics_dev.as<int32_t>();
    int64_t n = 0;
    const bool pdl = ctx->cfg.reserved[1] == 0;
    const StageOp* previous = nullptr;
    uint32_t exchange_index = 0;
    const bool fused_pushes = ctx->peer_mode && !ctx->body_masks.empty();
    for (const StageOp& op : ctx->program) {
        if (ctx->peer_mode && op.pad == -1) {
            launch_shard_exchange(nullptr, 0, 1, ctx->B, ctx->peers, fp, exchange_index++, ctx->error_dev.as<int32_t>(), s);
            ++n;
            continue;
        }
        if (ctx->peer_mode && op.pad >= 2 && op.stage <= kStageSolve) {
            if (op.work_count > 0) {
                bool prefetch = previous != nullptr && previous->stage != kStageIncremental && !(previous->stage <= kStageSolve && previous->work_begin == op.work_begin && previous->work_count > 0);
                const int launch_flags = (pdl ? kLaunchPdl : 0) | (prefetch ? kLaunchPrefetchRows : 0);
                if (fused_pushes) {
                    const ShardStage shard{exchange_index, ctx->error_dev.as<int32_t>()};
                    ctx->launchers->constraint_stage_sharded(op.stage, records + op.work_begin, ref_rows + (size_t)op.work_begin * 64, op.work_count, ctx->B, fp, launch_flags, ctx->peers,
                                                             (long long)(ctx->peer32.as<int32_t>() - ctx->refs32.as<int32_t>()), shard, s);
                    ++exchange_index;
                    ++n;
                    previous = &op;
                    continue;
                }
                ctx->launchers->constraint_stage(op.stage, records + op.work_begin, ref_rows + (size_t)op.work_begin * 64, op.work_count, ctx->B, fp, launch_flags, s);
                ++n;
            }
            if (fused_pushes) { ++exchange_index; continue; }
            const auto& range = ctx->push_range[op.pad - 2];
            launch_shard_exchange(ctx->pushes_dev.as<uint32_t>() + range.first, range.second, op.stage == kStageSolve ? 1 : (op.stage == kStageWarmStart ? 3 : 2), ctx->B, ctx->peers, fp,
                                  exchange_index++, ctx->error_dev.as<int32_t>(), s);
            ++n;
            if (op.work_count > 0) previous = &op;
            continue;
        }
        switch (op.stage) {
            case kStageWarmStartFirst: case kStageWarmStart: case kStageSolve: case kStageIncremental:
                if (op.work_count > 0) {
                    bool prefetch = op.stage != kStageIncremental && previous != nullptr && previous->stage != kStageIncremental;
                    if (prefetch && previous->stage <= kStageSolve && previous->work_begin == op.work_begin) prefetch = false;
                    if (ctx->exchange) {
                        ctx->launchers->constraint_stage(op.stage, records + op.work_begin, ref_rows + (size_t)op.work_begin * 64, op.work_count, ctx->B, fp, 0, s);
                        ++n;
                        if (op.stage != kStageIncremental) {
                            const int planes = op.stage == kStageSolve ? 1 : (op.stage == kStageWarmStart ? 3 : 2);
                            const size_t words = (size_t)ctx->body_count * 8 * planes;
                            cudaMemsetAsync(ctx->exchange_staging.ptr, 0, words * 4, s);
                            launch_collect_stage(ctx->tb_table.as<DeviceTypeBatch>(), ctx->work_table.as<WorkItem>() + op.work_begin, op.work_count, ctx->bodies_per_type.as<int32_t>(), op.stage,
                                                 ctx->B, ctx->exchange_staging.as<int32_t>(), s);
                            if (ctx->exchange(ctx->exchange_user, ctx->exchange_staging.ptr, (int64_t)words, 0, (void*)s) != 0) ctx->exchange_failed = true;
                            launch_apply_stage(ctx->exchange_staging.as<int32_t>(), planes, ctx->B, s);
                            n += 2;
                        }
                        previous = &op;
                        break;
                    }
                    ctx->launchers->constraint_stage(op.stage, records + op.work_begin, ref_rows + (size_t)op.work_begin * 64, op.work_count, ctx->B, fp, (pdl ? kLaunchPdl : 0) | (prefetch ? kLaunchPrefetchRows : 0), s);
                    previous = &op;
                    ++n;
                }
                break;
            case kStageKinematicFirst: case kStageKinematic:
                if (op.work_count > 0) { ctx->launchers->kinematic_stage(op.stage, kin, op.work_count, ctx->B, fp, s); previous = &op; ++n; }
                break;
            case kStageFinalPose:
                if (ctx->B.count > 0) { ctx->launchers->final_pose(ctx->B, fp, s); previous = &op; ++n; }
                break;
        }
    }
    if (launches) *launches = n;
    ctx->exchanges_per_solve = exchange_index;
}

void build_program(bepucuda_ctx* ctx) {
    ctx->program.clear();
    const int substeps = (int)ctx->iterations.size();
    const int kin = (int)ctx->kinematics.size();
    for (int s = 0; s < substeps; ++s) {
        if (s > 0) {
            if (ctx->peer_mode) ctx->program.push_back({kStageKinematic, 0, 0, -1});
            if (ctx->inc_work_count > 0) ctx->program.push_back({kStageIncremental, ctx->inc_work_begin, ctx->inc_work_count, 0});
            if (kin > 0) ctx->program.push_back({kStageKinematic, 0, kin, 0});
        } else if (ctx->integ.integrate_velocity_for_kinematics && kin > 0) {
            ctx->program.push_back({kStageKinematicFirst, 0, kin, 0});
        }
        if (ctx->peer_mode) ctx->program.push_back({kStageKinematic, 0, 0, -1});
        for (size_t b = 0; b < ctx->batch_work.size(); ++b) {
            auto& bw = ctx->batch_work[b];
            if (bw.second > 0 || (ctx->peer_mode && (int)b < ctx->sync_batch_count)) ctx->program.push_back({s == 0 ? kStageWarmStartFirst : kStageWarmStart, bw.first, bw.second, ctx->peer_mode ? (int)b + 2 : 0});
        }
        for (int it = 0; it < ctx->iterations[s]; ++it)
            for (size_t b = 0; b < ctx->batch_work.size(); ++b) {
                auto& bw = ctx->batch_work[b];
                if (bw.second > 0 || (ctx->peer_mode && (int)b < ctx->sync_batch_count)) ctx->program.push_back({kStageSolve, bw.first, bw.second, ctx->peer_mode ? (int)b + 2 : 0});
            }
    }
    if (ctx->peer_mode) ctx->program.push_back({kStageKinematic, 0, 0, -1});
    ctx->program.push_back({kStageFinalPose, 0, ctx->body_count, 0});
}

int upload_program(bepucuda_ctx* ctx) {
    build_program(ctx);
    if (ctx->peer_mode && !ctx->body_masks.empty() && ctx->boundary_count.size() == ctx->batch_work.size()) {
        std::vector<unsigned long long> targets((size_t)kShardMaxExchanges, 0ull);
        unsigned long long arrived = 0;
        size_t e = 0;
        for (const StageOp& op : ctx->program) {
            if (op.pad != -1 && !(op.pad >= 2 && op.stage <= kStageSolve)) continue;
            if (e + 1 >= (size_t)kShardMaxExchanges) return fail(ctx, BEPUCUDA_ERR_BAD_STATE, "peer sharding: more than 4095 exchange points per solve");
            if (op.pad >= 2 && op.work_count > 0) arrived += (unsigned long long)ctx->boundary_count[(size_t)(op.pad - 2)];
            targets[e++] = arrived;
        }
        targets[(size_t)kShardMaxExchanges - 1] = arrived;
        CK(cudaStreamSynchronize(ctx->stream));
        for (int q = 0; q < ctx->peers.rank_count; ++q)
            if (q != ctx->peers.rank)
                CK(cudaMemcpy(ctx->peers.flags[q] + kShardTargetSlot + (size_t)ctx->peers.rank * kShardMaxExchanges, targets.data(), targets.size() * 8, cudaMemcpyDefault));
        CK(cudaMemset((unsigned long long*)ctx->shard_flags.ptr + kShardCounterSlot, 0, kMaxShardRanks * 8));
        ctx->shard_solve_index = 0;
    }
    CK(ctx->program_dev.reserve(ctx->program.size() * sizeof(StageOp)));
    CK(cudaMemcpyAsync(ctx->program_dev.ptr, ctx->program.data(), ctx->program.size() * sizeof(StageOp), cudaMemcpyHostToDevice, ctx->stream));
    CK(cudaStreamSynchronize(ctx->stream));
    invalidate_graph(ctx);
    int64_t stages = 0;
    for (auto& op : ctx->program) stages += (op.work_count > 0 || op.stage == kStageFinalPose) ? 1 : 0;
    ctx->timings.stage_count = stages;
    return BEPUCUDA_OK;
}

void compute_frame_params(bepucuda_ctx* ctx, float dt, FrameParams* fp) {
    const int substeps = (int)ctx->iterations.size();
    const float substepDt = dt / substeps;
    auto clamp01 = [](float v) { return v < 0.f ? 0.f : (v > 1.f ? 1.f : v); };
    const bepucuda_integrator_desc& d = ctx->integ;
    fp->dt = substepDt;
    fp->inverse_dt = 1.0f / substepDt;
    fp->linear_damping_dt = powf(clamp01(1 - d.linear_damping), substepDt);
    fp->angular_damping_dt = powf(clamp01(1 - d.angular_damping), substepDt);
    for (int i = 0; i < 3; ++i) fp->gravity_dt[i] = d.gravity[i] * substepDt;
    const float finalDt = d.allow_substeps_for_unconstrained ? substepDt : dt;
    fp->final_dt = finalDt;
    fp->final_linear_damping_dt = powf(clamp01(1 - d.linear_damping), finalDt);
    fp->final_angular_damping_dt = powf(clamp01(1 - d.angular_damping), finalDt);
    for (int i = 0; i < 3; ++i) fp->final_gravity_dt[i] = d.gravity[i] * finalDt;
    fp->final_steps = d.allow_substeps_for_unconstrained ? substeps : 1;
    fp->angular_mode = d.angular_integration_mode;
    fp->integrate_velocity_for_kinematics = d.integrate_velocity_for_kinematics;
    for (int i = 0; i < 4; ++i) fp->tune[i] = ctx->tune[i];
}

int refresh_device_rows(bepucuda_ctx* ctx) {
    if (!ctx->data_dirty) return BEPUCUDA_OK;
    { int rc = flush_chunks(ctx, ctx->pending_h2d); if (rc != BEPUCUDA_OK) return rc; }
    bool any_redistribute = false;
    if (ctx->descs_dirty) {
        for (SourceTypeBatch& s : ctx->sources)
            for (int tb : s.device_tbs) {
                TransposeDesc& d = ctx->tdescs[tb];
                d.flags = (s.resident_impulses ? kDescResidentImpulses : 0) | (s.redistribute ? kDescRedistribute : 0);
                d.features_old = s.raw_features_old;
                d.features_new = s.raw_features_new;
                any_redistribute |= s.redistribute;
            }
        CK(cudaMemcpyAsync(ctx->tdesc_table.ptr, ctx->tdescs.data(), ctx->tdescs.size() * sizeof(TransposeDesc), cudaMemcpyHostToDevice, ctx->stream));
    }
    launch_transpose_in_all(ctx->tb_table.as<DeviceTypeBatch>(), ctx->tdesc_table.as<TransposeDesc>(), ctx->work_table.as<WorkItem>(), ctx->all_work_count, ctx->W,
                            kTransposePrestep | kTransposeImpulses, ctx->stream);
    if (any_redistribute) {
        launch_redistribute_impulses(ctx->tb_table.as<DeviceTypeBatch>(), ctx->tdesc_table.as<TransposeDesc>(), ctx->work_table.as<WorkItem>(), ctx->all_work_count, ctx->stream);
        for (SourceTypeBatch& s : ctx->sources)
            if (s.redistribute) {
                std::swap(s.raw_features_old, s.raw_features_new);
                s.redistribute = false;
            }
    } else {
        ctx->descs_dirty = false;
    }
    CK(cudaGetLastError());
    ctx->data_dirty = false;
    return BEPUCUDA_OK;
}

}

extern "C" {

int32_t bepucuda_type_info(int32_t type_id, int32_t* bodies_per_constraint, int32_t* prestep_floats, int32_t* impulse_floats) {
    const TypeInfo* t = get_type_info(type_id);
    if (!t) return BEPUCUDA_ERR_UNSUPPORTED_TYPE;
    if (bodies_per_constraint) *bodies_per_constraint = t->bodies;
    if (prestep_floats) *prestep_floats = t->prestep_rows;
    if (impulse_floats) *impulse_floats = t->impulse_rows;
    return BEPUCUDA_OK;
}

int32_t bepucuda_create(const bepucuda_config* cfg, bepucuda_ctx** out) {
    if (!cfg || !out) return BEPUCUDA_ERR_INVALID_ARGUMENT;
    *out = nullptr;
    int count = 0;
    if (cudaGetDeviceCount(&count) != cudaSuccess || count <= 0) return BEPUCUDA_ERR_NO_DEVICE;
    if (cfg->device_ordinal < 0 || cfg->device_ordinal >= count) return BEPUCUDA_ERR_INVALID_ARGUMENT;
    if (cfg->execution_mode != BEPUCUDA_EXEC_GRAPH && cfg->execution_mode != BEPUCUDA_EXEC_STREAM) return BEPUCUDA_ERR_INVALID_ARGUMENT;
    bepucuda_ctx* ctx = new bepucuda_ctx();
    ctx->cfg = *cfg;
    if (const char* tune = getenv("BEPUCUDA_TUNE")) sscanf(tune, "%d,%d,%d,%d", &ctx->tune[0], &ctx->tune[1], &ctx->tune[2], &ctx->tune[3]);
    ctx->device = cfg->device_ordinal;
    ctx->launchers = cfg->strict_fp ? get_launchers_bepu_strict() : get_launchers_bepu_fast();
    ctx->pinned_arena.pinned_host = true;
    ctx->pinned_arena.min_chunk = (size_t)16 << 20;
    cudaError_t e = cudaSetDevice(ctx->device);
    if (e == cudaSuccess) e = cudaStreamCreateWithFlags(&ctx->stream, cudaStreamNonBlocking);
    cudaEvent_t* evs[] = {&ctx->ev_solve_begin, &ctx->ev_solve_end, &ctx->ev_up_begin, &ctx->ev_up_end, &ctx->ev_down_begin, &ctx->ev_down_end};
    for (auto ev : evs)
        if (e == cudaSuccess) e = cudaEventCreate(ev);
    if (e == cudaSuccess) e = cudaMallocHost((void**)&ctx->frame_params_host, sizeof(FrameParams));
    if (e == cudaSuccess) e = ctx->frame_params_dev.reserve(sizeof(FrameParams));
    if (e == cudaSuccess) e = ctx->error_dev.reserve(8 * sizeof(int32_t));
    if (e != cudaSuccess) {
        bepucuda_destroy(ctx);
        return e == cudaErrorMemoryAllocation ? BEPUCUDA_ERR_OUT_OF_MEMORY : BEPUCUDA_ERR_CUDA;
    }
    ctx->integ.gravity[0] = 0; ctx->integ.gravity[1] = -10; ctx->integ.gravity[2] = 0;
    ctx->integ.linear_damping = 0.03f;
    ctx->integ.angular_damping = 0.03f;
    *out = ctx;
    return BEPUCUDA_OK;
}

int32_t bepucuda_destroy(bepucuda_ctx* ctx) {
    if (!ctx) return BEPUCUDA_OK;
    cudaSetDevice(ctx->device);
    if (ctx->stream) cudaStreamSynchronize(ctx->stream);
    invalidate_graph(ctx);
    for (void* p : ctx->opened_ipc) cudaIpcCloseMemHandle(p);
    DeviceBuffer* bufs[] = {&ctx->shard_flags, &ctx->pushes_dev, &ctx->peer32, &ctx->body_masks_dev, &ctx->boundary_flags_dev, &ctx->raw_bodies, &ctx->pose, &ctx->velocity, &ctx->inertia_local, &ctx->inertia_world, &ctx->constrained, &ctx->first_batch, &ctx->sync_refcount,
                            &ctx->sync_mask, &ctx->chunk_table, &ctx->record_table, &ctx->ref_rows, &ctx->body_shapes, &ctx->body_activities, &ctx->body_bounds, &ctx->color_refs, &ctx->color_priorities, &ctx->color_body_min, &ctx->color_body_mask, &ctx->color_out, &ctx->color_lists, &ctx->color_counts, &ctx->source_bundle_flags, &ctx->refs32, &ctx->prestep32, &ctx->impulses32, &ctx->tb_table, &ctx->tdesc_table, &ctx->work_table, &ctx->map_table,
                            &ctx->bodies_per_type, &ctx->kinematics_dev, &ctx->program_dev, &ctx->frame_params_dev, &ctx->error_dev, &ctx->exchange_staging};
    for (auto b : bufs) b->release();
    ctx->raw_arena.release();
    ctx->pinned_arena.release();
    if (ctx->frame_params_host) cudaFreeHost(ctx->frame_params_host);
    for (auto ev : ctx->user_events)
        if (ev) cudaEventDestroy(ev);
    for (auto& st : ctx->chunk_stage) {
        if (st.host) cudaFreeHost(st.host);
        if (st.done) cudaEventDestroy(st.done);
    }
    for (auto ev : ctx->profile_events) cudaEventDestroy(ev);
    cudaEvent_t evs[] = {ctx->ev_solve_begin, ctx->ev_solve_end, ctx->ev_up_begin, ctx->ev_up_end, ctx->ev_down_begin, ctx->ev_down_end};
    for (auto ev : evs)
        if (ev) cudaEventDestroy(ev);
    if (ctx->stream) cudaStreamDestroy(ctx->stream);
    delete ctx;
    return BEPUCUDA_OK;
}

const char* bepucuda_last_error(bepucuda_ctx* ctx) { return ctx ? ctx->error.c_str() : "null context"; }

int32_t bepucuda_host_register(bepucuda_ctx* ctx, void* ptr, int64_t bytes) {
    if (!ctx || !ptr || bytes <= 0) return fail(ctx, BEPUCUDA_ERR_INVALID_ARGUMENT, "host_register: bad arguments");
    CK(cudaSetDevice(ctx->device));
    CK(cudaHostRegister(ptr, (size_t)bytes, cudaHostRegisterMapped | cudaHostRegisterPortable));
    void* dev = nullptr;
    CK(cudaHostGetDevicePointer(&dev, ptr, 0));
    ctx->host_ranges.push_back({(char*)ptr, (size_t)bytes, (char*)dev});
    return BEPUCUDA_OK;
}
int32_t bepucuda_host_unregister(bepucuda_ctx* ctx, void* ptr) {
    if (!ctx || !ptr) return fail(ctx, BEPUCUDA_ERR_INVALID_ARGUMENT, "host_unregister: bad arguments");
    CK(cudaSetDevice(ctx->device));
    CK(cudaStreamSynchronize(ctx->stream));
    CK(cudaHostUnregister(ptr));
    for (size_t i = 0; i < ctx->host_ranges.size(); ++i)
        if (ctx->host_ranges[i].host == (char*)ptr) { ctx->host_ranges.erase(ctx->host_ranges.begin() + i); break; }
    return BEPUCUDA_OK;
}

int32_t bepucuda_set_solve_description(bepucuda_ctx* ctx, int32_t substep_count, const int32_t* its, int32_t fallback_batch_threshold) {
    if (!ctx || substep_count < 1 || !its || fallback_batch_threshold < 1) return fail(ctx, BEPUCUDA_ERR_INVALID_ARGUMENT, "set_solve_description: bad arguments");
    for (int i = 0; i < substep_count; ++i)
        if (its[i] < 0) return fail(ctx, BEPUCUDA_ERR_INVALID_ARGUMENT, "set_solve_description: negative iteration count");
    std::vector<int32_t> v(its, its + substep_count);
    const bool threshold_changed = fallback_batch_threshold != ctx->fallback_threshold;
    const bool changed = v != ctx->iterations || threshold_changed;
    ctx->iterations = v;
    ctx->fallback_threshold = fallback_batch_threshold;
    if (threshold_changed && ctx->constraints_ready) ctx->constraints_ready = false;
    if (changed && ctx->constraints_ready) {
        CK(cudaSetDevice(ctx->device));
        return upload_program(ctx);
    }
    return BEPUCUDA_OK;
}

int32_t bepucuda_set_integrator(bepucuda_ctx* ctx, const bepucuda_integrator_desc* desc) {
    if (!ctx || !desc) return fail(ctx, BEPUCUDA_ERR_INVALID_ARGUMENT, "set_integrator: bad arguments");
    if (desc->angular_integration_mode < 0 || desc->angular_integration_mode > 2) return fail(ctx, BEPUCUDA_ERR_INVALID_ARGUMENT, "set_integrator: unknown AngularIntegrationMode");
    const bool kin_changed = (desc->integrate_velocity_for_kinematics != 0) != (ctx->integ.integrate_velocity_for_kinematics != 0);
    ctx->integ = *desc;
    ctx->integ_set = true;
    if (kin_changed && ctx->constraints_ready) {
        CK(cudaSetDevice(ctx->device));
        return upload_program(ctx);
    }
    return BEPUCUDA_OK;
}

int32_t bepucuda_upload_bodies(bepucuda_ctx* ctx, const void* body_dynamics, int32_t body_count) {
    if (!ctx || body_count < 0 || (body_count > 0 && !body_dynamics)) return fail(ctx, BEPUCUDA_ERR_INVALID_ARGUMENT, "upload_bodies: bad arguments");
    if ((uint32_t)body_count > kRefIndexMask) return fail(ctx, BEPUCUDA_ERR_INVALID_ARGUMENT, "upload_bodies: too many bodies");
    CK(cudaSetDevice(ctx->device));
    open_upload_window(ctx);
    const size_t n = (size_t)body_count;
    if (body_count != ctx->body_count) {
        if (ctx->constraints_ready) ctx->constraints_ready = false;
        invalidate_graph(ctx);
    }
    CK(ctx->raw_bodies.reserve(n * 128));
    CK(ctx->pose.reserve(n * 32));
    CK(ctx->velocity.reserve(n * 32));
    CK(ctx->inertia_local.reserve(n * 32));
    CK(ctx->inertia_world.reserve(n * 32));
    const size_t old_constrained_cap = ctx->constrained.capacity;
    CK(ctx->constrained.reserve(n + 1));
    if (ctx->constrained.capacity != old_constrained_cap) CK(cudaMemsetAsync(ctx->constrained.ptr, 0, ctx->constrained.capacity, ctx->stream));
    ctx->body_count = body_count;
    BodyBuffers B{};
    B.pose = ctx->pose.as<float4>();
    B.velocity = ctx->velocity.as<float4>();
    B.inertia_local = ctx->inertia_local.as<float4>();
    B.inertia_world = ctx->inertia_world.as<float4>();
    B.constrained = ctx->constrained.as<uint8_t>();
    B.count = body_count;
    if (B.pose != ctx->B.pose || B.velocity != ctx->B.velocity || B.inertia_local != ctx->B.inertia_local || B.inertia_world != ctx->B.inertia_world ||
        B.constrained != ctx->B.constrained || B.count != ctx->B.count)
        invalidate_graph(ctx);
    ctx->B = B;
    if (body_count > 0) {
        CK(cudaMemcpyAsync(ctx->raw_bodies.ptr, body_dynamics, n * 128, cudaMemcpyHostToDevice, ctx->stream));
        ctx->h2d_accum += (int64_t)n * 128;
        launch_split_bodies(ctx->raw_bodies.ptr, body_count, ctx->B, ctx->stream);
        CK(cudaGetLastError());
    }
    return BEPUCUDA_OK;
}

int32_t bepucuda_begin_constraints(bepucuda_ctx* ctx, int32_t source_bundle_width, int32_t batch_count) {
    if (!ctx || source_bundle_width < 1 || source_bundle_width > 64 || batch_count < 0) return fail(ctx, BEPUCUDA_ERR_INVALID_ARGUMENT, "begin_constraints: bad arguments");
    CK(cudaSetDevice(ctx->device));
    CK(cudaStreamSynchronize(ctx->stream));
    open_upload_window(ctx);
    ctx->W = source_bundle_width;
    ctx->batch_count = batch_count;
    ctx->sources.clear();
    ctx->pending_h2d.clear();
    ctx->raw_arena.reset();
    ctx->pinned_arena.reset();
    ctx->constraints_open = true;
    ctx->constraints_ready = false;
    invalidate_graph(ctx);
    return BEPUCUDA_OK;
}

int32_t bepucuda_upload_type_batch(bepucuda_ctx* ctx, int32_t batch_index, int32_t type_batch_index, int32_t type_id, int32_t constraint_count,
                                   const int32_t* body_references, const float* prestep, float* accumulated_impulses) {
    if (!ctx) return BEPUCUDA_ERR_INVALID_ARGUMENT;
    if (!ctx->constraints_open) return fail(ctx, BEPUCUDA_ERR_BAD_STATE, "upload_type_batch outside begin/end_constraints");
    if (batch_index < 0 || batch_index >= ctx->batch_count || type_batch_index < 0 || constraint_count < 0)
        return fail(ctx, BEPUCUDA_ERR_INVALID_ARGUMENT, "upload_type_batch: bad indices");
    const TypeInfo* t = get_type_info(type_id);
    if (!t) return fail(ctx, BEPUCUDA_ERR_UNSUPPORTED_TYPE, "upload_type_batch: unsupported constraint type id " + std::to_string(type_id));
    if (constraint_count == 0) return BEPUCUDA_OK;
    if (!body_references || !prestep || !accumulated_impulses) return fail(ctx, BEPUCUDA_ERR_INVALID_ARGUMENT, "upload_type_batch: null buffer");
    CK(cudaSetDevice(ctx->device));
    const int W = ctx->W;
    const size_t bundles = ((size_t)constraint_count + W - 1) / W;
    SourceTypeBatch s{};
    s.batch_index = batch_index; s.type_batch_index = type_batch_index; s.type_id = type_id; s.count = constraint_count;
    s.host_impulses = accumulated_impulses;
    s.refs_bytes = bundles * t->bodies * W * 4;
    s.prestep_bytes = bundles * t->prestep_rows * W * 4;
    s.impulse_bytes = bundles * t->impulse_rows * W * 4;
    cudaError_t e = cudaSuccess;
    s.raw_refs = (int32_t*)ctx->raw_arena.alloc(s.refs_bytes, &e);
    s.raw_prestep = (float*)ctx->raw_arena.alloc(s.prestep_bytes, &e);
    s.raw_impulses = (float*)ctx->raw_arena.alloc(s.impulse_bytes, &e);
    if (!s.raw_refs || !s.raw_prestep || !s.raw_impulses) return cuda_fail(ctx, e, "raw arena");
    int rc;
    if ((rc = copy_in(ctx, s.raw_refs, body_references, s.refs_bytes)) != BEPUCUDA_OK) return rc;
// ... 49 lines not shown
            d.bundle_count = (s.count + 31) / 32;
            d.device_batch = s.batch_index;
            TransposeDesc td{s.raw_refs, s.raw_prestep, s.raw_impulses, nullptr, s.count, t->bodies, t->prestep_rows, t->impulse_rows, source_bundle_base[si], 0, nullptr, nullptr};
            s.device_tbs.push_back((int)ctx->tbs.size());
            batch_tbs[s.batch_index].push_back((int)ctx->tbs.size());
            ctx->tbs.push_back(d);
            ctx->tdescs.push_back(td);
            map_offset.push_back(SIZE_MAX);
            s.live = s.count;
            constraint_count += s.count;
        }
        if (ctx->peer_mode) {
            while ((int)batch_tbs.size() < std::min(ctx->batch_count, ctx->fallback_threshold)) batch_tbs.emplace_back();
            for (const SourceTypeBatch& src : ctx->sources)
                if (src.batch_index >= ctx->fallback_threshold) return fail(ctx, BEPUCUDA_ERR_BAD_STATE, "end_constraints: the sequential fallback batch is not supported across ranks");
        }
        if (ctx->exchange && !ctx->peer_mode) {
            for (const SourceTypeBatch& src : ctx->sources)
                if (src.batch_index >= ctx->fallback_threshold) return fail(ctx, BEPUCUDA_ERR_BAD_STATE, "end_constraints: the sequential fallback batch is not supported with an exchange callback");
        }
        (void)current_batch;
        ctx->sync_batch_count = (int)batch_tbs.size();
    }
    {
        std::vector<int32_t> last_level;
        struct Slot { int level; int source; int constraint; };
        std::vector<Slot> slots;
        bool any = false;
        for (size_t si = 0; si < ctx->sources.size(); ++si) {
            SourceTypeBatch& s = ctx->sources[si];
            if (s.batch_index < ctx->fallback_threshold) continue;
            if (!any) { last_level.assign((size_t)ctx->body_count, 0); any = true; }
            s.live = 0;
            const TypeInfo* t = get_type_info(s.type_id);
            const int nb = t->bodies;
            const int bundles = (s.count + W - 1) / W;
            std::vector<int> lane_level(W);
            for (int k = 0; k < bundles; ++k) {
                for (int l = 0; l < W; ++l) {
                    lane_level[l] = 0;
                    const int c = k * W + l;
                    if (c >= s.count) continue;
                    const int32_t first = s.host_refs[((size_t)k * nb) * W + l];
                    if (first < 0) continue;
                    int lvl = 0;
                    for (int b = 0; b < nb; ++b) {
                        const int32_t enc = s.host_refs[((size_t)k * nb + b) * W + l];
                        if (enc < 0 || ((uint32_t)enc & kRefKinematicBit)) continue;
                        const uint32_t idx = (uint32_t)enc & kRefIndexMask;
                        if ((int)idx >= ctx->body_count) return fail(ctx, BEPUCUDA_ERR_INVALID_ARGUMENT, "end_constraints: body reference out of range");
                        lvl = std::max(lvl, last_level[idx]);
                    }
                    lane_level[l] = lvl + 1;
                }
                for (int l = 0; l < W; ++l) {
                    if (lane_level[l] == 0) continue;
                    for (int b = 0; b < nb; ++b) {
                        const int32_t enc = s.host_refs[((size_t)k * nb + b) * W + l];
                        if (enc < 0 || ((uint32_t)enc & kRefKinematicBit)) continue;
                        last_level[(uint32_t)enc & kRefIndexMask] = lane_level[l];
                    }
                    for (int l2 = 0; l2 < l; ++l2) {
                        if (lane_level[l2] == 0) continue;
                        for (int b = 0; b < nb; ++b) {
                            const int32_t e1 = s.host_refs[((size_t)k * nb + b) * W + l];
                            if (e1 < 0 || ((uint32_t)e1 & kRefKinematicBit)) continue;
                            for (int b2 = 0; b2 < nb; ++b2) {
                                const int32_t e2 = s.host_refs[((size_t)k * nb + b2) * W + l2];
                                if (e2 >= 0 && !((uint32_t)e2 & kRefKinematicBit) && (((uint32_t)e1 ^ (uint32_t)e2) & kRefIndexMask) == 0)
                                    return fail(ctx, BEPUCUDA_ERR_BATCH_INVARIANT, "end_constraints: a fallback bundle references the same dynamic body more than once");
                            }
                        }
                    }
                    slots.push_back({lane_level[l], (int)si, k * W + l});
                    ++s.live;
                    ++constraint_count;
                }
            }
        }
        if (any) {
            std::stable_sort(slots.begin(), slots.end(), [](const Slot& a, const Slot& b) { return a.level != b.level ? a.level < b.level : a.source < b.source; });
            size_t i = 0;
            while (i < slots.size()) {
                const int level = slots[i].level;
                batch_tbs.emplace_back();
                ++ctx->fallback_levels;
                while (i < slots.size() && slots[i].level == level) {
                    const int source = slots[i].source;
                    size_t j = i;
                    while (j < slots.size() && slots[j].level == level && slots[j].source == source) ++j;
                    SourceTypeBatch& s = ctx->sources[source];
                    const TypeInfo* t = get_type_info(s.type_id);
                    const int n = (int)(j - i);
                    DeviceTypeBatch d{};
                    d.type_id = s.type_id;
                    d.bundle_count = (n + 31) / 32;
                    d.device_batch = (int)batch_tbs.size() - 1;
                    map_offset.push_back(maps.size());
                    for (size_t q = i; q < j; ++q) maps.push_back(slots[q].constraint);
                    for (int q = n; q < d.bundle_count * 32; ++q) maps.push_back(-1);
                    TransposeDesc td{s.raw_refs, s.raw_prestep, s.raw_impulses, nullptr, s.count, t->bodies, t->prestep_rows, t->impulse_rows, source_bundle_base[source], 0, nullptr, nullptr};
                    s.device_tbs.push_back((int)ctx->tbs.size());
                    batch_tbs.back().push_back((int)ctx->tbs.size());
                    ctx->tbs.push_back(d);
                    ctx->tdescs.push_back(td);
                    i = j;
                }
            }
        }
    }

    size_t refs_floats = 0, prestep_floats = 0, impulse_floats = 0;
    std::vector<size_t> ro(ctx->tbs.size()), po(ctx->tbs.size()), io(ctx->tbs.size());
    for (size_t i = 0; i < ctx->tbs.size(); ++i) {
        const TypeInfo* t = get_type_info(ctx->tbs[i].type_id);
        ro[i] = refs_floats; po[i] = prestep_floats; io[i] = impulse_floats;
        refs_floats += (size_t)ctx->tbs[i].bundle_count * t->bodies * 32;
        prestep_floats += (size_t)ctx->tbs[i].bundle_count * t->prestep_rows * 32;
        impulse_floats += (size_t)ctx->tbs[i].bundle_count * t->impulse_rows * 32;
    }
    CK(ctx->refs32.reserve(refs_floats * 4 + 1024));
    ctx->refs_words = refs_floats;
    CK(ctx->prestep32.reserve(prestep_floats * 4 + 4));
    CK(ctx->impulses32.reserve(impulse_floats * 4 + 4));
    CK(ctx->map_table.reserve(maps.size() * 4 + 4));
    for (size_t i = 0; i < ctx->tbs.size(); ++i) {
        ctx->tbs[i].refs = ctx->refs32.as<int32_t>() + ro[i];
        ctx->tbs[i].prestep = ctx->prestep32.as<float>() + po[i];
        ctx->tbs[i].impulses = ctx->impulses32.as<float>() + io[i];
        ctx->tdescs[i].map = map_offset[i] == SIZE_MAX ? nullptr : ctx->map_table.as<int32_t>() + map_offset[i];
    }

    ctx->work.clear();
    ctx->bundle_live.clear();
    ctx->batch_work.clear();
    auto live_in_bundle = [&](int tb, int k) {
        if (map_offset[tb] == SIZE_MAX) return std::max(0, std::min(32, ctx->tdescs[tb].src_count - k * 32));
        int n = 0;
        for (int l = 0; l < 32; ++l) n += maps[map_offset[tb] + (size_t)k * 32 + l] >= 0;
        return n;
    };
    for (auto& list : batch_tbs) {
        const int begin = (int)ctx->work.size();
        for (int tb : list)
            for (int k = 0; k < ctx->tbs[tb].bundle_count; ++k) { ctx->work.push_back({tb, k}); ctx->bundle_live.push_back(live_in_bundle(tb, k)); }
        ctx->batch_work.push_back({begin, (int)ctx->work.size() - begin});
    }
    ctx->all_work_count = (int)ctx->work.size();
    ctx->inc_work_begin = (int)ctx->work.size();
    for (size_t tb = 0; tb < ctx->tbs.size(); ++tb)
        if (get_type_info(ctx->tbs[tb].type_id)->incremental)
            for (int k = 0; k < ctx->tbs[tb].bundle_count; ++k) { ctx->work.push_back({(int)tb, k}); ctx->bundle_live.push_back(live_in_bundle((int)tb, k)); }
    ctx->inc_work_count = (int)ctx->work.size() - ctx->inc_work_begin;

    ctx->records.resize(ctx->work.size());
    for (size_t i = 0; i < ctx->work.size(); ++i) {
        const WorkItem& w = ctx->work[i];
        const DeviceTypeBatch& tb = ctx->tbs[w.type_batch];
        const TypeInfo* t = get_type_info(tb.type_id);
        WorkRecord r{};
        r.refs = tb.refs + (size_t)w.bundle * t->bodies * 32;
        r.prestep = tb.prestep + (size_t)w.bundle * t->prestep_rows * 32;
        r.impulses = tb.impulses + (size_t)w.bundle * t->impulse_rows * 32;
        r.type_id = tb.type_id;
        r.live_lanes = ctx->bundle_live[i];
        ctx->records[i] = r;
    }

    int32_t bodies_per_type[64];
    for (int i = 0; i < 64; ++i) bodies_per_type[i] = get_type_info(i) ? get_type_info(i)->bodies : 0;
    CK(ctx->tb_table.reserve(ctx->tbs.size() * sizeof(DeviceTypeBatch) + 16));
    CK(ctx->tdesc_table.reserve(ctx->tdescs.size() * sizeof(TransposeDesc) + 16));
    CK(ctx->work_table.reserve(ctx->work.size() * sizeof(WorkItem) + 16));
    CK(ctx->record_table.reserve(ctx->records.size() * sizeof(WorkRecord) + 64));
    CK(ctx->bodies_per_type.reserve(sizeof(bodies_per_type)));
    CK(ctx->kinematics_dev.reserve(ctx->kinematics.size() * 4 + 4));
    if (!ctx->tbs.empty()) CK(cudaMemcpyAsync(ctx->tb_table.ptr, ctx->tbs.data(), ctx->tbs.size() * sizeof(DeviceTypeBatch), cudaMemcpyHostToDevice, ctx->stream));
    if (!ctx->tdescs.empty()) CK(cudaMemcpyAsync(ctx->tdesc_table.ptr, ctx->tdescs.data(), ctx->tdescs.size() * sizeof(TransposeDesc), cudaMemcpyHostToDevice, ctx->stream));
    if (!ctx->work.empty()) CK(cudaMemcpyAsync(ctx->work_table.ptr, ctx->work.data(), ctx->work.size() * sizeof(WorkItem), cudaMemcpyHostToDevice, ctx->stream));
    if (!ctx->records.empty()) CK(cudaMemcpyAsync(ctx->record_table.ptr, ctx->records.data(), ctx->records.size() * sizeof(WorkRecord), cudaMemcpyHostToDevice, ctx->stream));
    if (!maps.empty()) CK(cudaMemcpyAsync(ctx->map_table.ptr, maps.data(), maps.size() * 4, cudaMemcpyHostToDevice, ctx->stream));
    CK(cudaMemcpyAsync(ctx->bodies_per_type.ptr, bodies_per_type, sizeof(bodies_per_type), cudaMemcpyHostToDevice, ctx->stream));
    if (!ctx->kinematics.empty()) CK(cudaMemcpyAsync(ctx->kinematics_dev.ptr, ctx->kinematics.data(), ctx->kinematics.size() * 4, cudaMemcpyHostToDevice, ctx->stream));

    { int rc = flush_chunks(ctx, ctx->pending_h2d); if (rc != BEPUCUDA_OK) return rc; }
    launch_transpose_in_all(ctx->tb_table.as<DeviceTypeBatch>(), ctx->tdesc_table.as<TransposeDesc>(), ctx->work_table.as<WorkItem>(), ctx->all_work_count, W,
                            kTransposeRefs | kTransposePrestep | kTransposeImpulses, ctx->stream);
    const size_t nb = (size_t)std::max(ctx->body_count, 1);
    CK(ctx->first_batch.reserve(nb * 4));
    CK(ctx->sync_refcount.reserve(nb * 4));
    CK(ctx->sync_mask.reserve(nb * 8));
    launch_fill_i32(ctx->first_batch.as<int32_t>(), nb, 0x7fffffff, ctx->stream);
    CK(cudaMemsetAsync(ctx->sync_refcount.ptr, 0, nb * 4, ctx->stream));
    CK(cudaMemsetAsync(ctx->sync_mask.ptr, 0, nb * 8, ctx->stream));
    CK(cudaMemsetAsync(ctx->constrained.ptr, 0, nb, ctx->stream));
    CK(cudaMemsetAsync(ctx->error_dev.ptr, 0, 32, ctx->stream));
    CK(ctx->source_bundle_flags.reserve((size_t)std::max(total_source_bundles, 1) * 16));
    CK(cudaMemsetAsync(ctx->source_bundle_flags.ptr, 0, (size_t)std::max(total_source_bundles, 1) * 16, ctx->stream));
    launch_ownership_pass1(ctx->tb_table.as<DeviceTypeBatch>(), ctx->work_table.as<WorkItem>(), ctx->all_work_count, ctx->bodies_per_type.as<int32_t>(), ctx->sync_batch_count,
                           ctx->body_count, ctx->first_batch.as<int32_t>(), ctx->sync_refcount.as<int32_t>(), (unsigned long long*)ctx->sync_mask.ptr, ctx->error_dev.as<int32_t>(),
                           ctx->stream);
    if (ctx->peer_mode && nb > 0) {
        if ((int)ctx->global_first_batch.size() != ctx->body_count) return fail(ctx, BEPUCUDA_ERR_BAD_STATE, "end_constraints: bepucuda_shard_set_global was not called for this body count");
        CK(cudaMemcpyAsync(ctx->first_batch.ptr, ctx->global_first_batch.data(), (size_t)ctx->body_count * 4, cudaMemcpyHostToDevice, ctx->stream));
    }
    if (ctx->exchange && !ctx->peer_mode && nb > 0) {
        if (ctx->exchange(ctx->exchange_user, ctx->first_batch.ptr, (int64_t)ctx->body_count, 1, (void*)ctx->stream) != 0)
            return fail(ctx, BEPUCUDA_ERR_CUDA, "end_constraints: the exchange callback failed (first-batch minimum)");
    }
    launch_ownership_rest(ctx->tb_table.as<DeviceTypeBatch>(), ctx->work_table.as<WorkItem>(), ctx->all_work_count, ctx->bodies_per_type.as<int32_t>(), ctx->body_count,
                          ctx->first_batch.as<int32_t>(), ctx->sync_refcount.as<int32_t>(), (const unsigned long long*)ctx->sync_mask.ptr, ctx->constrained.as<uint8_t>(),
                          ctx->kinematics_dev.as<int32_t>(), (int)ctx->kinematics.size(), ctx->error_dev.as<int32_t>(), ctx->tdesc_table.as<TransposeDesc>(), W,
                          ctx->source_bundle_flags.as<int32_t>(), ctx->stream);
    if (ctx->peer_mode && nb > 0) {
        CK(cudaMemcpyAsync(ctx->constrained.ptr, ctx->global_constrained.data(), (size_t)ctx->body_count, cudaMemcpyHostToDevice, ctx->stream));
        std::vector<uint32_t> all;
        ctx->push_range.assign(ctx->sync_batch_count, {0, 0});
        for (int b = 0; b < ctx->sync_batch_count; ++b) {
            auto it = ctx->pushes_by_batch.find(b);
            if (it == ctx->pushes_by_batch.end()) continue;
            ctx->push_range[b] = {all.size(), (int)it->second.size()};
            all.insert(all.end(), it->second.begin(), it->second.end());
        }
        CK(ctx->pushes_dev.reserve(all.size() * 4 + 16));
        if (!all.empty()) CK(cudaMemcpy(ctx->pushes_dev.ptr, all.data(), all.size() * 4, cudaMemcpyHostToDevice));
    }
    if (ctx->exchange && !ctx->peer_mode && nb > 0) {
        CK(ctx->exchange_staging.reserve((size_t)nb * 24 * 4));
        launch_widen_u8(ctx->constrained.as<uint8_t>(), ctx->exchange_staging.as<int32_t>(), (size_t)ctx->body_count, ctx->stream);
        if (ctx->exchange(ctx->exchange_user, ctx->exchange_staging.ptr, (int64_t)ctx->body_count, 0, (void*)ctx->stream) != 0)
            return fail(ctx, BEPUCUDA_ERR_CUDA, "end_constraints: the exchange callback failed (constrained mask)");
        launch_narrow_i32(ctx->exchange_staging.as<int32_t>(), ctx->constrained.as<uint8_t>(), (size_t)ctx->body_count, ctx->stream);
    }
    if (ctx->peer_mode && !ctx->body_masks.empty()) {
        if ((int)ctx->body_masks.size() != ctx->body_count) return fail(ctx, BEPUCUDA_ERR_BAD_STATE, "end_constraints: bepucuda_shard_set_body_masks was called for another body count");
        CK(ctx->peer32.reserve(ctx->refs_words * 4 + 1024));
        CK(ctx->body_masks_dev.reserve((size_t)ctx->body_count + 16));
        CK(cudaMemcpyAsync(ctx->body_masks_dev.ptr, ctx->body_masks.data(), (size_t)ctx->body_count, cudaMemcpyHostToDevice, ctx->stream));
        launch_fill_peer_masks(ctx->refs32.as<int32_t>(), ctx->peer32.as<uint32_t>(), ctx->refs_words, ctx->body_masks_dev.as<uint8_t>(), ctx->peers.rank, ctx->stream);
        const int n_rec = ctx->all_work_count;
        CK(ctx->boundary_flags_dev.reserve((size_t)n_rec + 16));
        launch_boundary_flags(ctx->record_table.as<WorkRecord>(), n_rec, ctx->bodies_per_type.as<int32_t>(), (long long)(ctx->peer32.as<int32_t>() - ctx->refs32.as<int32_t>()),
                              ctx->boundary_flags_dev.as<uint8_t>(), ctx->stream);
        std::vector<uint8_t> is_boundary((size_t)n_rec);
        if (n_rec > 0) CK(cudaMemcpyAsync(is_boundary.data(), ctx->boundary_flags_dev.ptr, (size_t)n_rec, cudaMemcpyDeviceToHost, ctx->stream));
        CK(cudaStreamSynchronize(ctx->stream));
        ctx->boundary_count.assign(ctx->batch_work.size(), 0);
        std::vector<WorkRecord> sorted;
        for (size_t b = 0; b < ctx->batch_work.size(); ++b) {
            const int begin = ctx->batch_work[b].first, count = ctx->batch_work[b].second;
            sorted.clear();
            for (int pass = 0; pass < 2; ++pass)
                for (int i = begin; i < begin + count; ++i)
                    if ((is_boundary[(size_t)i] != 0) == (pass == 0)) {
                        WorkRecord r = ctx->records[(size_t)i];
                        r.live_lanes = (r.live_lanes & ~kRecordBoundaryBit) | (pass == 0 ? kRecordBoundaryBit : 0);
                        sorted.push_back(r);
                        ctx->boundary_count[b] += pass == 0;
                    }
            std::copy(sorted.begin(), sorted.end(), ctx->records.begin() + begin);
        }
        if (n_rec > 0) CK(cudaMemcpyAsync(ctx->record_table.ptr, ctx->records.data(), (size_t)n_rec * sizeof(WorkRecord), cudaMemcpyHostToDevice, ctx->stream));
    }
    CK(ctx->ref_rows.reserve((size_t)std::max<size_t>(ctx->records.size(), 1) * 64 * 4));
    launch_pack_ref_rows(ctx->record_table.as<WorkRecord>(), (int)ctx->records.size(), ctx->ref_rows.as<int32_t>(), ctx->stream);
    CK(cudaGetLastError());
    int32_t err = 0;
    CK(cudaMemcpyAsync(&err, ctx->error_dev.ptr, 4, cudaMemcpyDeviceToHost, ctx->stream));
    CK(cudaStreamSynchronize(ctx->stream));
    if (err == 1) return fail(ctx, BEPUCUDA_ERR_BATCH_INVARIANT, "end_constraints: a synchronized batch references the same dynamic body more than once");
    if (err == 2) return fail(ctx, BEPUCUDA_ERR_INVALID_ARGUMENT, "end_constraints: body reference out of range");

    ctx->timings.constraint_count = constraint_count;
    ctx->timings.device_batch_count = (int)batch_tbs.size();
    ctx->timings.fallback_level_count = ctx->fallback_levels;
    ctx->constraints_open = false;
    ctx->constraints_ready = true;
    ctx->data_dirty = false;
    return upload_program(ctx);
}

int32_t bepucuda_update_type_batch(bepucuda_ctx* ctx, int32_t batch_index, int32_t type_batch_index, const float* prestep, float* accumulated_impulses) {
    if (!ctx || !prestep || !accumulated_impulses) return fail(ctx, BEPUCUDA_ERR_INVALID_ARGUMENT, "update_type_batch: bad arguments");
    if (!ctx->constraints_ready) return fail(ctx, BEPUCUDA_ERR_BAD_STATE, "update_type_batch before end_constraints");
    CK(cudaSetDevice(ctx->device));
    open_upload_window(ctx);
    for (auto& s : ctx->sources)
        if (s.batch_index == batch_index && s.type_batch_index == type_batch_index) {
            char* alias_p = map_host(ctx, prestep, s.prestep_bytes);
            char* alias_i = map_host(ctx, accumulated_impulses, s.impulse_bytes);
            if (alias_p && alias_i) {
                queue_chunks(ctx->pending_h2d, s.raw_prestep, alias_p, s.prestep_bytes);
                queue_chunks(ctx->pending_h2d, s.raw_impulses, alias_i, s.impulse_bytes);
            } else {
                CK(cudaMemcpyAsync(s.raw_prestep, prestep, s.prestep_bytes, cudaMemcpyHostToDevice, ctx->stream));
                CK(cudaMemcpyAsync(s.raw_impulses, accumulated_impulses, s.impulse_bytes, cudaMemcpyHostToDevice, ctx->stream));
            }
            ctx->h2d_accum += (int64_t)(s.prestep_bytes + s.impulse_bytes);
            s.host_impulses = accumulated_impulses;
            if (s.resident_impulses) { s.resident_impulses = false; s.redistribute = false; ctx->descs_dirty = true; }
            ctx->data_dirty = true;
            return BEPUCUDA_OK;
        }
    return fail(ctx, BEPUCUDA_ERR_INVALID_ARGUMENT, "update_type_batch: unknown type batch");
}

// ... 142 lines not shown
    }
    if (ctx->cfg.execution_mode == BEPUCUDA_EXEC_STREAM) {
        issue_stage_sequence(ctx, ctx->stream, &launches);
        CK(cudaGetLastError());
        if (ctx->exchange_failed) return fail(ctx, BEPUCUDA_ERR_CUDA, "solve: the exchange callback failed");
    }
    CK(cudaEventRecord(ctx->ev_solve_end, ctx->stream));
    if (ctx->peer_mode) { ctx->exchange_counter += ctx->exchanges_per_solve; ++ctx->shard_solve_index; }
    ctx->have_solve = true;
    ctx->timings.kernel_launches = launches;

    int64_t ci = 0, bytes = 0;
    const int substeps = (int)ctx->iterations.size();
    for (const SourceTypeBatch& s : ctx->sources) {
        const TypeInfo* t = get_type_info(s.type_id);
        const int64_t n = s.live;
        for (int sub = 0; sub < substeps; ++sub) {
            ci += n * ctx->iterations[sub];
            bytes += n * ((int64_t)t->warm_start_bytes + (int64_t)ctx->iterations[sub] * t->solve_bytes + (sub > 0 ? t->incremental_bytes : 0));
        }
    }
    bytes += (int64_t)ctx->body_count * 108;
    ctx->timings.constraint_iterations = ci;
    ctx->timings.algorithmic_bytes = bytes;
    return BEPUCUDA_OK;
}

static int check_device_error_flag(bepucuda_ctx* ctx) {
    if (ctx->peer_mode && ctx->tune[3]) {
        unsigned long long acc[4] = {};
        cudaMemcpy(acc, (unsigned long long*)ctx->shard_flags.ptr + kMaxShardRanks, sizeof(acc), cudaMemcpyDeviceToHost);
        if (acc[3]) fprintf(stderr, "[bepucuda shard rank %d] exchange phases, mean over %llu: push+fence %.2f us, signal %.2f us, wait %.2f us\n", ctx->peers.rank, acc[3],
                            acc[0] / 1e3 / acc[3], acc[1] / 1e3 / acc[3], acc[2] / 1e3 / acc[3]);
    }
    if (ctx->peer_mode) {
        int32_t e = 0;
        CK(cudaMemcpyAsync(&e, ctx->error_dev.ptr, 4, cudaMemcpyDeviceToHost, ctx->stream));
        CK(cudaStreamSynchronize(ctx->stream));
        if (e == 5) return fail(ctx, BEPUCUDA_ERR_CUDA, "sharded solve: a peer rank never reached an exchange point (flag barrier timed out); results are invalid");
    }
    return BEPUCUDA_OK;
}

int32_t bepucuda_synchronize(bepucuda_ctx* ctx) {
    if (!ctx) return BEPUCUDA_ERR_INVALID_ARGUMENT;
    CK(cudaSetDevice(ctx->device));
    CK(cudaStreamSynchronize(ctx->stream));
    return check_device_error_flag(ctx);
}

int32_t bepucuda_download_bodies(bepucuda_ctx* ctx, void* out, int32_t body_count) {
    if (!ctx || !out || body_count < 0 || body_count > ctx->body_count) return fail(ctx, BEPUCUDA_ERR_INVALID_ARGUMENT, "download_bodies: bad arguments");
    CK(cudaSetDevice(ctx->device));
    CK(cudaEventRecord(ctx->ev_down_begin, ctx->stream));
    launch_merge_bodies(ctx->raw_bodies.ptr, body_count, ctx->B, ctx->stream);
    CK(cudaGetLastError());
    CK(cudaMemcpyAsync(out, ctx->raw_bodies.ptr, (size_t)body_count * 128, cudaMemcpyDeviceToHost, ctx->stream));
    CK(cudaEventRecord(ctx->ev_down_end, ctx->stream));
    CK(cudaStreamSynchronize(ctx->stream));
    ctx->have_down = true;
    ctx->timings.d2h_bytes = (int64_t)body_count * 128;
    return BEPUCUDA_OK;
}

int32_t bepucuda_download_impulses(bepucuda_ctx* ctx) {
    if (!ctx) return BEPUCUDA_ERR_INVALID_ARGUMENT;
    if (!ctx->constraints_ready) return fail(ctx, BEPUCUDA_ERR_BAD_STATE, "download_impulses before end_constraints");
    CK(cudaSetDevice(ctx->device));
    launch_transpose_out_all(ctx->tb_table.as<DeviceTypeBatch>(), ctx->tdesc_table.as<TransposeDesc>(), ctx->work_table.as<WorkItem>(), ctx->all_work_count, ctx->W,
                             kTransposeImpulses, ctx->stream);
    CK(cudaGetLastError());
    int64_t bytes = 0;
    std::vector<CopyChunk> d2h;
    for (auto& s : ctx->sources) {
        if (char* alias = map_host(ctx, s.host_impulses, s.impulse_bytes)) queue_chunks(d2h, alias, s.raw_impulses, s.impulse_bytes);
        else CK(cudaMemcpyAsync(s.host_impulses, s.raw_impulses, s.impulse_bytes, cudaMemcpyDeviceToHost, ctx->stream));
        bytes += (int64_t)s.impulse_bytes;
    }
    { int rc = flush_chunks(ctx, d2h); if (rc != BEPUCUDA_OK) return rc; }
    CK(cudaStreamSynchronize(ctx->stream));
    ctx->timings.d2h_bytes += bytes;
    return BEPUCUDA_OK;
}

int32_t bepucuda_download_prestep(bepucuda_ctx* ctx, int32_t batch_index, int32_t type_batch_index, float* prestep_out) {
    if (!ctx || !prestep_out) return fail(ctx, BEPUCUDA_ERR_INVALID_ARGUMENT, "download_prestep: bad arguments");
    if (!ctx->constraints_ready) return fail(ctx, BEPUCUDA_ERR_BAD_STATE, "download_prestep before end_constraints");
    CK(cudaSetDevice(ctx->device));
    for (auto& s : ctx->sources)
        if (s.batch_index == batch_index && s.type_batch_index == type_batch_index) {
            launch_transpose_out_all(ctx->tb_table.as<DeviceTypeBatch>(), ctx->tdesc_table.as<TransposeDesc>(), ctx->work_table.as<WorkItem>(), ctx->all_work_count, ctx->W,
                                     kTransposePrestep, ctx->stream);
            CK(cudaGetLastError());
            CK(cudaMemcpyAsync(prestep_out, s.raw_prestep, s.prestep_bytes, cudaMemcpyDeviceToHost, ctx->stream));
            CK(cudaStreamSynchronize(ctx->stream));
            return BEPUCUDA_OK;
        }
    return fail(ctx, BEPUCUDA_ERR_INVALID_ARGUMENT, "download_prestep: unknown type batch");
}

int32_t bepucuda_get_timings(bepucuda_ctx* ctx, bepucuda_timings* out) {
    if (!ctx || !out) return BEPUCUDA_ERR_INVALID_ARGUMENT;
    CK(cudaSetDevice(ctx->device));
    CK(cudaStreamSynchronize(ctx->stream));
    { int rc = check_device_error_flag(ctx); if (rc != BEPUCUDA_OK) return rc; }
    if (ctx->have_solve) cudaEventElapsedTime(&ctx->timings.solve_ms, ctx->ev_solve_begin, ctx->ev_solve_end);
    if (ctx->have_up && !ctx->up_open) cudaEventElapsedTime(&ctx->timings.upload_ms, ctx->ev_up_begin, ctx->ev_up_end);
    if (ctx->have_down) cudaEventElapsedTime(&ctx->timings.download_ms, ctx->ev_down_begin, ctx->ev_down_end);
    *out = ctx->timings;
    return BEPUCUDA_OK;
}

int32_t bepucuda_event_record(bepucuda_ctx* ctx, int32_t slot) {
    if (!ctx || slot < 0 || slot >= 16) return fail(ctx, BEPUCUDA_ERR_INVALID_ARGUMENT, "event_record: bad slot");
    CK(cudaSetDevice(ctx->device));
    if (!ctx->user_events[slot]) CK(cudaEventCreate(&ctx->user_events[slot]));
    CK(cudaEventRecord(ctx->user_events[slot], ctx->stream));
    return BEPUCUDA_OK;
}
int32_t bepucuda_event_elapsed_ms(bepucuda_ctx* ctx, int32_t a, int32_t b, float* ms) {
    if (!ctx || !ms || a < 0 || a >= 16 || b < 0 || b >= 16 || !ctx->user_events[a] || !ctx->user_events[b]) return fail(ctx, BEPUCUDA_ERR_INVALID_ARGUMENT, "event_elapsed_ms: bad slots");
    CK(cudaSetDevice(ctx->device));
    CK(cudaEventSynchronize(ctx->user_events[b]));
    CK(cudaEventElapsedTime(ms, ctx->user_events[a], ctx->user_events[b]));
    return BEPUCUDA_OK;
}

int32_t bepucuda_profile_stages(bepucuda_ctx* ctx, float dt, bepucuda_stage_profile* out) {
    if (ctx && ctx->exchange) return fail(ctx, BEPUCUDA_ERR_BAD_STATE, "profile_stages: not available with sharded batches");
    if (!ctx || !out || !(dt > 0)) return fail(ctx, BEPUCUDA_ERR_INVALID_ARGUMENT, "profile_stages: bad arguments");
    if (!ctx->constraints_ready) return fail(ctx, BEPUCUDA_ERR_BAD_STATE, "profile_stages before end_constraints");
    CK(cudaSetDevice(ctx->device));
    std::memset(out, 0, sizeof(*out));
    { int rc = refresh_device_rows(ctx); if (rc != BEPUCUDA_OK) return rc; }
    CK(cudaStreamSynchronize(ctx->stream));
    compute_frame_params(ctx, dt, ctx->frame_params_host);
    CK(cudaMemcpyAsync(ctx->frame_params_dev.ptr, ctx->frame_params_host, sizeof(FrameParams), cudaMemcpyHostToDevice, ctx->stream));
    const size_t need = ctx->program.size() * 2;
    while (ctx->profile_events.size() < need) {
        cudaEvent_t ev;
        CK(cudaEventCreate(&ev));
        ctx->profile_events.push_back(ev);
    }
    const WorkRecord* records = ctx->record_table.as<WorkRecord>();
    const int32_t* ref_rows = ctx->ref_rows.as<int32_t>();
    const FrameParams* fp = ctx->frame_params_dev.as<FrameParams>();
    const int32_t* kin = ctx->kinematics_dev.as<int32_t>();
    std::vector<int> launched(ctx->program.size(), 0);
    for (size_t i = 0; i < ctx->program.size(); ++i) {
        const StageOp& op = ctx->program[i];
        const bool has_work = op.stage == kStageFinalPose ? ctx->B.count > 0 : op.work_count > 0;
        if (!has_work) continue;
        CK(cudaEventRecord(ctx->profile_events[2 * i], ctx->stream));
        if (op.stage <= kStageIncremental) ctx->launchers->constraint_stage(op.stage, records + op.work_begin, ref_rows + (size_t)op.work_begin * 64, op.work_count, ctx->B, fp, 0, ctx->stream);
        else if (op.stage <= kStageKinematic) ctx->launchers->kinematic_stage(op.stage, kin, op.work_count, ctx->B, fp, ctx->stream);
        else ctx->launchers->final_pose(ctx->B, fp, ctx->stream);
        CK(cudaEventRecord(ctx->profile_events[2 * i + 1], ctx->stream));
        launched[i] = 1;
    }
    CK(cudaStreamSynchronize(ctx->stream));
    CK(cudaGetLastError());
    for (size_t i = 0; i < ctx->program.size(); ++i) {
        if (!launched[i]) continue;
        float ms = 0;
        CK(cudaEventElapsedTime(&ms, ctx->profile_events[2 * i], ctx->profile_events[2 * i + 1]));
        const StageOp& op = ctx->program[i];
        out->ms[op.stage] += ms;
        out->launches[op.stage] += 1;
        int64_t bytes = 0;
        if (op.stage <= kStageIncremental) {
            for (int w = 0; w < op.work_count; ++w) {
                const WorkItem& wi = ctx->work[op.work_begin + w];
                const TypeInfo* t = get_type_info(ctx->tbs[wi.type_batch].type_id);
                const int per = op.stage == kStageSolve ? t->solve_bytes : op.stage == kStageIncremental ? t->incremental_bytes : t->warm_start_bytes;
                bytes += (int64_t)per * ctx->bundle_live[(size_t)op.work_begin + w];
            }
        } else if (op.stage == kStageFinalPose) {
            bytes = (int64_t)ctx->body_count * 108;
        } else {
            bytes = (int64_t)op.work_count * 108;
        }
        out->algorithmic_bytes[op.stage] += bytes;
    }
    return BEPUCUDA_OK;
}

static_assert(sizeof(bepucuda_body_shape) == sizeof(BodyShape) && sizeof(bepucuda_body_activity) == sizeof(BodyActivityRecord), "ABI structs mirror the device records");

int32_t bepucuda_set_body_shapes(bepucuda_ctx* ctx, const bepucuda_body_shape* shapes, int32_t body_count) {
    if (!ctx || body_count < 0 || (body_count > 0 && !shapes)) return fail(ctx, BEPUCUDA_ERR_INVALID_ARGUMENT, "set_body_shapes: bad arguments");
    CK(cudaSetDevice(ctx->device));
    CK(ctx->body_shapes.reserve((size_t)std::max(body_count, 1) * sizeof(BodyShape)));
    if (body_count > 0) CK(cudaMemcpyAsync(ctx->body_shapes.ptr, shapes, (size_t)body_count * sizeof(BodyShape), cudaMemcpyHostToDevice, ctx->stream));
    CK(cudaStreamSynchronize(ctx->stream));
    ctx->shape_count = body_count;
    return BEPUCUDA_OK;
}

int32_t bepucuda_predict_bounding_boxes(bepucuda_ctx* ctx, float dt, bepucuda_body_activity* activities, float* bounds_out) {
    if (!ctx || !(dt > 0) || !activities || !bounds_out) return fail(ctx, BEPUCUDA_ERR_INVALID_ARGUMENT, "predict_bounding_boxes: bad arguments");
    if (ctx->shape_count != ctx->body_count) return fail(ctx, BEPUCUDA_ERR_BAD_STATE, "predict_bounding_boxes: bepucuda_set_body_shapes was not called for the current body count");
    const int n = ctx->body_count;
    if (n == 0) return BEPUCUDA_OK;
    CK(cudaSetDevice(ctx->device));
    CK(ctx->body_activities.reserve((size_t)n * sizeof(BodyActivityRecord)));
    CK(ctx->body_bounds.reserve((size_t)n * 32));
    CK(cudaMemcpyAsync(ctx->body_activities.ptr, activities, (size_t)n * sizeof(BodyActivityRecord), cudaMemcpyHostToDevice, ctx->stream));
    auto clamp01 = [](float v) { return v < 0.f ? 0.f : (v > 1.f ? 1.f : v); };
    PredictParams p{};
    p.dt = dt;
    for (int i = 0; i < 3; ++i) p.gravity_dt[i] = ctx->integ.gravity[i] * dt;
    p.linear_damping_dt = powf(clamp01(1 - ctx->integ.linear_damping), dt);
    p.angular_damping_dt = powf(clamp01(1 - ctx->integ.angular_damping), dt);
    p.integrate_velocity_for_kinematics = ctx->integ.integrate_velocity_for_kinematics;
    launch_predict_bounding_boxes(ctx->B, ctx->body_shapes.as<BodyShape>(), ctx->body_activities.as<BodyActivityRecord>(), ctx->body_bounds.as<float4>(), p, ctx->stream);
    CK(cudaGetLastError());
    CK(cudaMemcpyAsync(activities, ctx->body_activities.ptr, (size_t)n * sizeof(BodyActivityRecord), cudaMemcpyDeviceToHost, ctx->stream));
    CK(cudaMemcpyAsync(bounds_out, ctx->body_bounds.ptr, (size_t)n * 32, cudaMemcpyDeviceToHost, ctx->stream));
    CK(cudaStreamSynchronize(ctx->stream));
    return BEPUCUDA_OK;
}

uint32_t bepucuda_color_hash(uint32_t constraint_index) { return color_hash(constraint_index); }

int32_t bepucuda_color_constraints(bepucuda_ctx* ctx, int32_t constraint_count, int32_t bodies_per_constraint, const int32_t* encoded_body_references, int32_t body_count,
                                   int32_t fallback_batch_threshold, int32_t order, const uint32_t* priorities, int32_t* batch_indices_out, int32_t* batch_count_out,
                                   int32_t* rounds_out) {
    if (!ctx) return BEPUCUDA_ERR_INVALID_ARGUMENT;
    if (constraint_count < 0 || bodies_per_constraint < 1 || bodies_per_constraint > 4 || body_count < 0 || fallback_batch_threshold < 1 || fallback_batch_threshold > 64)
        return fail(ctx, BEPUCUDA_ERR_INVALID_ARGUMENT, "color_constraints: counts out of range (1..4 body slots, fallback threshold 1..64)");
    if (order < BEPUCUDA_COLOR_INSERTION_ORDER || order > BEPUCUDA_COLOR_BY_PRIORITY || (order == BEPUCUDA_COLOR_BY_PRIORITY && !priorities))
        return fail(ctx, BEPUCUDA_ERR_INVALID_ARGUMENT, "color_constraints: unknown order, or BEPUCUDA_COLOR_BY_PRIORITY without priorities");
    if (constraint_count > 0 && (!encoded_body_references || !batch_indices_out)) return fail(ctx, BEPUCUDA_ERR_INVALID_ARGUMENT, "color_constraints: null buffer");
    if (batch_count_out) *batch_count_out = 0;
    if (rounds_out) *rounds_out = 0;
    if (constraint_count == 0) return BEPUCUDA_OK;
    CK(cudaSetDevice(ctx->device));
    const size_t words = (size_t)constraint_count * bodies_per_constraint;
    for (size_t i = 0; i < words; ++i) {
        const int32_t enc = encoded_body_references[i];
        if (enc >= 0 && (int32_t)((uint32_t)enc & ((1u << 30) - 1u)) >= body_count) return fail(ctx, BEPUCUDA_ERR_INVALID_ARGUMENT, "color_constraints: body reference out of range");
    }
    constexpr int kRoundsPerChunk = 32;
    const size_t nb = (size_t)std::max(body_count, 1), nc = (size_t)constraint_count;
    CK(ctx->color_refs.reserve(words * 4));
    CK(ctx->color_priorities.reserve(nc * 4));
    CK(ctx->color_body_min.reserve(nb * 8));
    CK(ctx->color_body_mask.reserve(nb * 8));
    CK(ctx->color_out.reserve(nc * 4));
    CK(ctx->color_lists.reserve(nc * 8));
    CK(ctx->color_counts.reserve((kRoundsPerChunk + 1) * 4));
    CK(cudaMemcpyAsync(ctx->color_refs.ptr, encoded_body_references, words * 4, cudaMemcpyHostToDevice, ctx->stream));
    if (order == BEPUCUDA_COLOR_BY_PRIORITY) CK(cudaMemcpyAsync(ctx->color_priorities.ptr, priorities, nc * 4, cudaMemcpyHostToDevice, ctx->stream));
    ColoringBuffers cb{};
    cb.refs = ctx->color_refs.as<int32_t>();
    cb.priorities = ctx->color_priorities.as<uint32_t>();
    cb.body_min = ctx->color_body_min.as<unsigned long long>();
    cb.body_mask = ctx->color_body_mask.as<unsigned long long>();
    cb.batch_out = ctx->color_out.as<int32_t>();
    cb.list[0] = ctx->color_lists.as<int32_t>();
    cb.list[1] = ctx->color_lists.as<int32_t>() + nc;
    cb.counts = ctx->color_counts.as<unsigned int>();
    cb.constraint_count = constraint_count;
    cb.bodies_per_constraint = bodies_per_constraint;
    cb.body_count = body_count;
    cb.fallback_threshold = fallback_batch_threshold;
    cb.order = order;
    CK(cudaMemsetAsync(ctx->color_counts.ptr, 0, (kRoundsPerChunk + 1) * 4, ctx->stream));
    launch_color_init(cb, ctx->stream);
    unsigned int counts[kRoundsPerChunk + 1];
    int64_t rounds = 0;
    for (;;) {
        for (int r = 0; r < kRoundsPerChunk; ++r) launch_color_round(cb, r, ctx->stream);
        CK(cudaMemcpyAsync(counts, ctx->color_counts.ptr, sizeof(counts), cudaMemcpyDeviceToHost, ctx->stream));
        CK(cudaStreamSynchronize(ctx->stream));
        CK(cudaGetLastError());
        int used = kRoundsPerChunk;
        for (int r = 0; r < kRoundsPerChunk; ++r)
            if (counts[r + 1] == 0) { used = r + 1; break; }
        rounds += used;
        if (counts[used] == 0) break;
        if (counts[kRoundsPerChunk] >= counts[0]) return fail(ctx, BEPUCUDA_ERR_CUDA, "color_constraints: no progress (internal error)");
        counts[0] = counts[kRoundsPerChunk];
        for (int r = 1; r <= kRoundsPerChunk; ++r) counts[r] = 0;
        CK(cudaMemcpyAsync(ctx->color_counts.ptr, counts, sizeof(counts), cudaMemcpyHostToDevice, ctx->stream));
        CK(cudaStreamSynchronize(ctx->stream));
    }
    CK(cudaMemcpyAsync(batch_indices_out, ctx->color_out.ptr, nc * 4, cudaMemcpyDeviceToHost, ctx->stream));
    CK(cudaStreamSynchronize(ctx->stream));
    int32_t highest = -1;
    for (size_t i = 0; i < nc; ++i) highest = std::max(highest, batch_indices_out[i]);
    if (batch_count_out) *batch_count_out = highest + 1;
    if (rounds_out) *rounds_out = (int32_t)std::min<int64_t>(rounds, 0x7fffffff);
    return BEPUCUDA_OK;
}

int32_t bepucuda_shard_export(bepucuda_ctx* ctx, bepucuda_ipc_handles* out) {
    if (!ctx || !out) return fail(ctx, BEPUCUDA_ERR_INVALID_ARGUMENT, "shard_export: bad arguments");
    if (ctx->body_count <= 0) return fail(ctx, BEPUCUDA_ERR_BAD_STATE, "shard_export before upload_bodies");
    CK(cudaSetDevice(ctx->device));
    CK(ctx->shard_flags.reserve(kShardFlagBlockWords * sizeof(unsigned long long)));
    CK(cudaMemset(ctx->shard_flags.ptr, 0, kShardFlagBlockWords * sizeof(unsigned long long)));
    void* ptrs[4] = {ctx->pose.ptr, ctx->velocity.ptr, ctx->inertia_world.ptr, ctx->shard_flags.ptr};
    for (int i = 0; i < 4; ++i) {
        cudaIpcMemHandle_t h;
        CK(cudaIpcGetMemHandle(&h, ptrs[i]));
        static_assert(sizeof(h) == 64, "cudaIpcMemHandle_t is 64 bytes");
// ... 107 lines not shown
```

Before: 2.010 billion.

## Precompute convex contact effective masses in warm start and reuse in solve iterations

Splits the convex contact solve into a projection step and a projected solve. The projection step, run during warm start, computes penetration/tangent/twist effective masses, bias velocities and softness and writes them to a new per-bundle projection buffer. Solve iterations then read these values instead of recomputing the inertia sandwiches and the 2x2 inverse every iteration. This trades ALU work for extra global memory traffic per iteration, and only applies to non-sync, non-exchange batches that are all convex.

```diff
diff --git a/bepuphysics2_b200/csrc/bepu_contacts.cuh b/bepuphysics2_b200/csrc/bepu_contacts.cuh
--- a/bepuphysics2_b200/csrc/bepu_contacts.cuh
+++ b/bepuphysics2_b200/csrc/bepu_contacts.cuh
@@ -36,6 +36,9 @@
 BEPU_DI void stacc(GlobalAcc a, int r, float v) { a.ptr[r * kLanes] = v; }
 BEPU_DI float ldacc(StagedAcc a, int r) { return lds_f32(a.addr + r * (kLanes * 4)); }
 BEPU_DI void stacc(StagedAcc a, int r, float v) { __stcs(a.ptr + r * kLanes, v); }
+struct ProjectionOut { float* ptr; };
+BEPU_DI void stacc(ProjectionOut q, int r, float v) { __stcs(q.ptr + r * kLanes, v); }
+
 
 BEPU_DI void penetration_apply(const Inertia& iA, const Inertia& iB, V3 normal, V3 angularA, V3 angularB, float impulse, Velocity& vA, Velocity& vB) {
     V3 dLinA = normal * (impulse * iA.inv_mass);
@@ -50,23 +53,33 @@
 BEPU_DI void penetration_warm_start(const Inertia& iA, const Inertia& iB, V3 normal, V3 offsetA, V3 offsetB, float accumulated, Velocity& vA, Velocity& vB) {
     penetration_apply(iA, iB, normal, cross(offsetA, normal), cross(normal, offsetB), accumulated, vA, vB);
 }
-BEPU_DI void penetration_solve(const Inertia& iA, const Inertia& iB, V3 normal, V3 offsetA, V3 offsetB, float depth, const Springiness& sp, float maxRecovery,
-                               float inverseDt, float& accumulated, Velocity& vA, Velocity& vB) {
-    V3 angularA = cross(offsetA, normal);
-    V3 angularB = cross(normal, offsetB);
+BEPU_DI float penetration_effective_mass(const Inertia& iA, const Inertia& iB, V3 angularA, V3 angularB, const Springiness& sp) {
     float angularA0 = vector_sandwich(angularA, iA.t);
     float angularB0 = vector_sandwich(angularB, iB.t);
     float linear = iA.inv_mass + iB.inv_mass;
-    float effectiveMass = sp.effective_mass_cfm_scale / (linear + angularA0 + angularB0);
-    float biasVelocity = fmin_ps(depth * inverseDt, fmin_ps(depth * sp.position_error_to_velocity, maxRecovery));
+    return sp.effective_mass_cfm_scale / (linear + angularA0 + angularB0);
+}
+BEPU_DI float penetration_bias_velocity(float depth, const Springiness& sp, float maxRecovery, float inverseDt) {
+    return fmin_ps(depth * inverseDt, fmin_ps(depth * sp.position_error_to_velocity, maxRecovery));
+}
+BEPU_DI void penetration_solve_projected(const Inertia& iA, const Inertia& iB, V3 normal, V3 offsetA, V3 offsetB, float effectiveMass, float biasVelocity, float softnessImpulseScale,
+                                         float& accumulated, Velocity& vA, Velocity& vB) {
+    V3 angularA = cross(offsetA, normal);
+    V3 angularB = cross(normal, offsetB);
     float csvaLinear = dot(vA.lin, normal);
     float csvaAngular = dot(vA.ang, angularA);
     float negatedCSVBLinear = dot(vB.lin, normal);
     float csvbAngular = dot(vB.ang, angularB);
-    float negatedCSI = accumulated * sp.softness_impulse_scale + (csvaLinear - negatedCSVBLinear + csvaAngular + csvbAngular - biasVelocity) * effectiveMass;
+    float negatedCSI = accumulated * softnessImpulseScale + (csvaLinear - negatedCSVBLinear + csvaAngular + csvbAngular - biasVelocity) * effectiveMass;
     float previous = accumulated;
     accumulated = fmax_ps(0.0f, accumulated - negatedCSI);
     penetration_apply(iA, iB, normal, angularA, angularB, accumulated - previous, vA, vB);
+}
+BEPU_DI void penetration_solve(const Inertia& iA, const Inertia& iB, V3 normal, V3 offsetA, V3 offsetB, float depth, const Springiness& sp, float maxRecovery,
+                               float inverseDt, float& accumulated, Velocity& vA, Velocity& vB) {
+    float effectiveMass = penetration_effective_mass(iA, iB, cross(offsetA, normal), cross(normal, offsetB), sp);
+    float biasVelocity = penetration_bias_velocity(depth, sp, maxRecovery, inverseDt);
+    penetration_solve_projected(iA, iB, normal, offsetA, offsetB, effectiveMass, biasVelocity, sp.softness_impulse_scale, accumulated, vA, vB);
 }
 BEPU_DI float updated_depth(float dt, V3 contactOffsetA, V3 offsetB, V3 normal, const Velocity& vA, const Velocity& vB, float depth) {
     V3 contactVelocityA = cross(vA.ang, contactOffsetA) + vA.lin;
@@ -82,18 +95,24 @@
     vA.lin = vA.lin + dLinA;
     vA.ang = vA.ang + dAngA;
 }
-BEPU_DI void penetration1_solve(const Inertia& iA, V3 normal, V3 offsetA, float depth, const Springiness& sp, float maxRecovery, float inverseDt, float& accumulated,
-                                Velocity& vA) {
+BEPU_DI float penetration1_effective_mass(const Inertia& iA, V3 angularA, const Springiness& sp) {
+    float angularA0 = vector_sandwich(angularA, iA.t);
+    return sp.effective_mass_cfm_scale / (iA.inv_mass + angularA0);
+}
+BEPU_DI void penetration1_solve_projected(const Inertia& iA, V3 normal, V3 offsetA, float effectiveMass, float biasVelocity, float softnessImpulseScale, float& accumulated, Velocity& vA) {
     V3 angularA = cross(offsetA, normal);
-    float angularA0 = vector_sandwich(angularA, iA.t);
-    float effectiveMass = sp.effective_mass_cfm_scale / (iA.inv_mass + angularA0);
-    float biasVelocity = fmin_ps(depth * inverseDt, fmin_ps(depth * sp.position_error_to_velocity, maxRecovery));
     float csvaLinear = dot(vA.lin, normal);
     float csvaAngular = dot(vA.ang, angularA);
-    float negatedCSI = accumulated * sp.softness_impulse_scale + (csvaLinear + csvaAngular - biasVelocity) * effectiveMass;
+    float negatedCSI = accumulated * softnessImpulseScale + (csvaLinear + csvaAngular - biasVelocity) * effectiveMass;
     float previous = accumulated;
     accumulated = fmax_ps(0.0f, accumulated - negatedCSI);
     penetration1_apply(iA, normal, angularA, accumulated - previous, vA);
+}
+BEPU_DI void penetration1_solve(const Inertia& iA, V3 normal, V3 offsetA, float depth, const Springiness& sp, float maxRecovery, float inverseDt, float& accumulated,
+                                Velocity& vA) {
+    float effectiveMass = penetration1_effective_mass(iA, cross(offsetA, normal), sp);
+    float biasVelocity = penetration_bias_velocity(depth, sp, maxRecovery, inverseDt);
+    penetration1_solve_projected(iA, normal, offsetA, effectiveMass, biasVelocity, sp.softness_impulse_scale, accumulated, vA);
 }
 BEPU_DI float updated_depth1(float dt, V3 contactOffset, V3 normal, const Velocity& v, float depth) {
     V3 contactVelocity = cross(v.ang, contactOffset) + v.lin;
@@ -117,11 +136,12 @@
     vB.lin = vB.lin - linearImpulseA * iB.inv_mass;
     vB.ang = vB.ang + transform(angularImpulseB, iB.t);
 }
-BEPU_DI void tangent_solve(V3 tX, V3 tY, V3 offsetA, V3 offsetB, const Inertia& iA, const Inertia& iB, float maximumImpulse, V2& accumulated, Velocity& vA, Velocity& vB) {
-    TangentJacobians j = tangent_jacobians(tX, tY, offsetA, offsetB);
+BEPU_DI Sym2 tangent_effective_mass(const TangentJacobians& j, const Inertia& iA, const Inertia& iB) {
     Sym2 linear = sandwich_scale(j.linearA, iA.inv_mass) + sandwich_scale(j.linearA, iB.inv_mass);
     Sym2 angular = matrix_sandwich(j.angularA, iA.t) + matrix_sandwich(j.angularB, iB.t);
-    Sym2 effectiveMass = invert(linear + angular);
+    return invert(linear + angular);
+}
+BEPU_DI void tangent_solve_projected(const TangentJacobians& j, const Sym2& effectiveMass, const Inertia& iA, const Inertia& iB, float maximumImpulse, V2& accumulated, Velocity& vA, Velocity& vB) {
     V2 csvaLinear = transform_by_transpose(vA.lin, j.linearA);
     V2 csvaAngular = transform_by_transpose(vA.ang, j.angularA);
     V2 csvbLinear = transform_by_transpose(vB.lin, j.linearA);
@@ -135,16 +155,20 @@
     accumulated = accumulated * scl;
     tangent_apply(j, iA, iB, accumulated - previous, vA, vB);
 }
+BEPU_DI void tangent_solve(V3 tX, V3 tY, V3 offsetA, V3 offsetB, const Inertia& iA, const Inertia& iB, float maximumImpulse, V2& accumulated, Velocity& vA, Velocity& vB) {
+    TangentJacobians j = tangent_jacobians(tX, tY, offsetA, offsetB);
+    tangent_solve_projected(j, tangent_effective_mass(j, iA, iB), iA, iB, maximumImpulse, accumulated, vA, vB);
+}
 BEPU_DI void tangent1_apply(const M23& linearA, const M23& angularA, const Inertia& iA, V2 impulse, Velocity& vA) {
     V3 linearImpulseA = transform(impulse, linearA);
     V3 angularImpulseA = transform(impulse, angularA);
     vA.lin = vA.lin + linearImpulseA * iA.inv_mass;
     vA.ang = vA.ang + transform(angularImpulseA, iA.t);
 }
-BEPU_DI void tangent1_solve(V3 tX, V3 tY, V3 offsetA, const Inertia& iA, float maximumImpulse, V2& accumulated, Velocity& vA) {
-    M23 linearA{tX, tY};
-    M23 angularA{cross(offsetA, tX), cross(offsetA, tY)};
-    Sym2 effectiveMass = invert(sandwich_scale(linearA, iA.inv_mass) + matrix_sandwich(angularA, iA.t));
+BEPU_DI Sym2 tangent1_effective_mass(const M23& linearA, const M23& angularA, const Inertia& iA) {
+    return invert(sandwich_scale(linearA, iA.inv_mass) + matrix_sandwich(angularA, iA.t));
+}
+BEPU_DI void tangent1_solve_projected(const M23& linearA, const M23& angularA, const Sym2& effectiveMass, const Inertia& iA, float maximumImpulse, V2& accumulated, Velocity& vA) {
     V2 csv = transform_by_transpose(vA.lin, linearA) + transform_by_transpose(vA.ang, angularA);
     V2 negativeCSI = transform(csv, effectiveMass);
     V2 previous = accumulated;
@@ -154,28 +178,43 @@
     accumulated = accumulated * scl;
     tangent1_apply(linearA, angularA, iA, accumulated - previous, vA);
 }
+BEPU_DI void tangent1_solve(V3 tX, V3 tY, V3 offsetA, const Inertia& iA, float maximumImpulse, V2& accumulated, Velocity& vA) {
+    M23 linearA{tX, tY};
+    M23 angularA{cross(offsetA, tX), cross(offsetA, tY)};
+    tangent1_solve_projected(linearA, angularA, tangent1_effective_mass(linearA, angularA, iA), iA, maximumImpulse, accumulated, vA);
+}
 
 BEPU_DI void twist_apply(V3 axis, const Inertia& iA, const Inertia& iB, float impulse, Velocity& vA, Velocity& vB) {
     V3 worldImpulseA = axis * impulse;
     vA.ang = vA.ang + transform(worldImpulseA, iA.t);
     vB.ang = vB.ang - transform(worldImpulseA, iB.t);
 }
-BEPU_DI void twist_solve(V3 axis, const Inertia& iA, const Inertia& iB, float maximumImpulse, float& accumulated, Velocity& vA, Velocity& vB) {
+BEPU_DI float twist_effective_mass(V3 axis, const Inertia& iA, const Inertia& iB) {
     float inverseEffectiveMass = vector_sandwich(axis, iA.t) + vector_sandwich(axis, iB.t);
-    float effectiveMass = (0.0f == inverseEffectiveMass) ? 0.0f : 1.0f / inverseEffectiveMass;
+    return (0.0f == inverseEffectiveMass) ? 0.0f : 1.0f / inverseEffectiveMass;
+}
+BEPU_DI void twist_solve_projected(V3 axis, float effectiveMass, const Inertia& iA, const Inertia& iB, float maximumImpulse, float& accumulated, Velocity& vA, Velocity& vB) {
     float negatedCSI = (dot(vA.ang, axis) - dot(vB.ang, axis)) * effectiveMass;
     float previous = accumulated;
     accumulated = fmin_ps(maximumImpulse, fmax_ps(-maximumImpulse, accumulated - negatedCSI));
     twist_apply(axis, iA, iB, accumulated - previous, vA, vB);
 }
+BEPU_DI void twist_solve(V3 axis, const Inertia& iA, const Inertia& iB, float maximumImpulse, float& accumulated, Velocity& vA, Velocity& vB) {
+    twist_solve_projected(axis, twist_effective_mass(axis, iA, iB), iA, iB, maximumImpulse, accumulated, vA, vB);
+}
 BEPU_DI void twist1_apply(V3 axis, const Inertia& iA, float impulse, Velocity& vA) { vA.ang = vA.ang + transform(axis * impulse, iA.t); }
-BEPU_DI void twist1_solve(V3 axis, const Inertia& iA, float maximumImpulse, float& accumulated, Velocity& vA) {
+BEPU_DI float twist1_effective_mass(V3 axis, const Inertia& iA) {
     float angularA = vector_sandwich(axis, iA.t);
-    float effectiveMass = (0.0f == angularA) ? 0.0f : 1.0f / angularA;
+    return (0.0f == angularA) ? 0.0f : 1.0f / angularA;
+}
+BEPU_DI void twist1_solve_projected(V3 axis, float effectiveMass, const Inertia& iA, float maximumImpulse, float& accumulated, Velocity& vA) {
     float negativeCSI = dot(vA.ang, axis) * effectiveMass;
     float previous = accumulated;
     accumulated = fmin_ps(maximumImpulse, fmax_ps(-maximumImpulse, accumulated - negativeCSI));
     twist1_apply(axis, iA, accumulated - previous, vA);
+}
+BEPU_DI void twist1_solve(V3 axis, const Inertia& iA, float maximumImpulse, float& accumulated, Velocity& vA) {
+    twist1_solve_projected(axis, twist1_effective_mass(axis, iA), iA, maximumImpulse, accumulated, vA);
 }
 
 template <int N, bool TwoBody> struct ConvexLayout {
@@ -187,6 +226,12 @@
     static constexpr int kMaxRecovery = kNormal + 6;
     static constexpr int kPrestepRows = kNormal + 7;
     static constexpr int kImpulseRows = N + 3;
+    static constexpr int kPenetrationMass = 0;
+    static constexpr int kBiasVelocity = N;
+    static constexpr int kTangentMass = 2 * N;
+    static constexpr int kTwistMass = 2 * N + 3;
+    static constexpr int kSoftness = 2 * N + 4;
+    static constexpr int kProjectionRows = 2 * N + 5;
 };
 
 template <int N> BEPU_DI V3 friction_center(const V3 (&offs)[N], const float (&depths)[N]) {
@@ -301,6 +346,76 @@
         stacc(a, N + 2, twist);
         }
     }
+    template <class PR, class QR> BEPU_DI static void project(const Inertia& iA, const Inertia& iB, float dt, float inverseDt, PR p, QR q) {
+        V3 normal = ldrow3(p, L::kNormal), offsetB = ldrow3(p, L::kOffsetB);
+        float maxRecovery = ldrow(p, L::kMaxRecovery);
+        Springiness sp = compute_springiness(ldrow(p, L::kAngularFrequency), ldrow(p, L::kTwiceDampingRatio), dt);
+#pragma unroll 1
+        for (int i = 0; i < N; ++i) {
+            V3 offset = ldrow3(p, 4 * i);
+            stacc(q, L::kPenetrationMass + i, penetration_effective_mass(iA, iB, cross(offset, normal), cross(normal, offset - offsetB), sp));
+            stacc(q, L::kBiasVelocity + i, penetration_bias_velocity(ldrow(p, 4 * i + 3), sp, maxRecovery, inverseDt));
+        }
+        V3 offs[N];
+        float depths[N];
+#pragma unroll
+        for (int i = 0; i < N; ++i) { offs[i] = ldrow3(p, 4 * i); depths[i] = ldrow(p, 4 * i + 3); }
+        V3 centerA;
+        if constexpr (N == 1) centerA = offs[0]; else centerA = friction_center<N>(offs, depths);
+        V3 x, z;
+        build_orthonormal_basis(normal, x, z);
+        const Sym2 tangentMass = tangent_effective_mass(tangent_jacobians(x, z, centerA, centerA - offsetB), iA, iB);
+        stacc(q, L::kTangentMass, tangentMass.xx);
+        stacc(q, L::kTangentMass + 1, tangentMass.yx);
+        stacc(q, L::kTangentMass + 2, tangentMass.yy);
+        stacc(q, L::kTwistMass, twist_effective_mass(normal, iA, iB));
+        stacc(q, L::kSoftness, sp.softness_impulse_scale);
+    }
+    template <class PR, class AR, class QR> BEPU_DI static void solve_projected(const Inertia& iA, const Inertia& iB, PR p, AR a, QR q, Velocity& vA, Velocity& vB) {
+        V3 normal = ldrow3(p, L::kNormal), offsetB = ldrow3(p, L::kOffsetB);
+        float friction = ldrow(p, L::kFriction);
+        const float softness = ldacc(q, L::kSoftness);
+        V3 centerA;
+        float maximumTangentImpulse, maximumTwistImpulse;
+        if constexpr (N > 1) {
+            V3 offs[N];
+            float depths[N];
+#pragma unroll
+            for (int i = 0; i < N; ++i) { offs[i] = ldrow3(p, 4 * i); depths[i] = ldrow(p, 4 * i + 3); }
+            centerA = friction_center<N>(offs, depths);
+            float penSum = 0.0f, twistSum = 0.0f;
+#pragma unroll 1
+            for (int i = 0; i < N; ++i) {
+                V3 offset = ldrow3(p, 4 * i);
+                float pen = ldacc(a, 2 + i);
+                penetration_solve_projected(iA, iB, normal, offset, offset - offsetB, ldacc(q, L::kPenetrationMass + i), ldacc(q, L::kBiasVelocity + i), softness, pen, vA, vB);
+                stacc(a, 2 + i, pen);
+                const float lever = pen * distance(centerA, offset);
+                penSum = i == 0 ? pen : penSum + pen;
+                twistSum = i == 0 ? lever : twistSum + lever;
+            }
+            const float premultiplied = (1.0f / N) * friction;
+            maximumTangentImpulse = premultiplied * penSum;
+            maximumTwistImpulse = premultiplied * twistSum;
+        } else {
+            centerA = ldrow3(p, 0);
+            float pen = ldacc(a, 2);
+            penetration_solve_projected(iA, iB, normal, centerA, centerA - offsetB, ldacc(q, L::kPenetrationMass), ldacc(q, L::kBiasVelocity), softness, pen, vA, vB);
+            stacc(a, 2, pen);
+            maximumTangentImpulse = friction * pen;
+            maximumTwistImpulse = friction * pen * fmax_ps(0.0f, ldrow(p, 3));
+        }
+        V3 x, z;
+        build_orthonormal_basis(normal, x, z);
+        V2 tangent{ldacc(a, 0), ldacc(a, 1)};
+        float twist = ldacc(a, N + 2);
+        tangent_solve_projected(tangent_jacobians(x, z, centerA, centerA - offsetB), Sym2{ldacc(q, L::kTangentMass), ldacc(q, L::kTangentMass + 1), ldacc(q, L::kTangentMass + 2)}, iA, iB,
+                                maximumTangentImpulse, tangent, vA, vB);
+        twist_solve_projected(normal, ldacc(q, L::kTwistMass), iA, iB, maximumTwistImpulse, twist, vA, vB);
+        stacc(a, 0, tangent.x);
+        stacc(a, 1, tangent.y);
+        stacc(a, N + 2, twist);
+    }
     BEPU_DI static void incremental_update(float dt, const Velocity& vA, const Velocity& vB, float* p) {
         V3 normal = ldrow3(p, L::kNormal), offsetB = ldrow3(p, L::kOffsetB);
 #pragma unroll
@@ -396,6 +511,75 @@
         stacc(a, N + 2, twist);
         }
     }
+    template <class PR, class QR> BEPU_DI static void project(const Inertia& iA, float dt, float inverseDt, PR p, QR q) {
+        V3 normal = ldrow3(p, L::kNormal);
+        float maxRecovery = ldrow(p, L::kMaxRecovery);
+        Springiness sp = compute_springiness(ldrow(p, L::kAngularFrequency), ldrow(p, L::kTwiceDampingRatio), dt);
+#pragma unroll 1
+        for (int i = 0; i < N; ++i) {
+            stacc(q, L::kPenetrationMass + i, penetration1_effective_mass(iA, cross(ldrow3(p, 4 * i), normal), sp));
+            stacc(q, L::kBiasVelocity + i, penetration_bias_velocity(ldrow(p, 4 * i + 3), sp, maxRecovery, inverseDt));
+        }
+        V3 offs[N];
+        float depths[N];
+#pragma unroll
+        for (int i = 0; i < N; ++i) { offs[i] = ldrow3(p, 4 * i); depths[i] = ldrow(p, 4 * i + 3); }
+        V3 centerA;
+        if constexpr (N == 1) centerA = offs[0]; else centerA = friction_center<N>(offs, depths);
+        V3 x, z;
+        build_orthonormal_basis(normal, x, z);
+        const Sym2 tangentMass = tangent1_effective_mass(M23{x, z}, M23{cross(centerA, x), cross(centerA, z)}, iA);
+        stacc(q, L::kTangentMass, tangentMass.xx);
+        stacc(q, L::kTangentMass + 1, tangentMass.yx);
+        stacc(q, L::kTangentMass + 2, tangentMass.yy);
+        stacc(q, L::kTwistMass, twist1_effective_mass(normal, iA));
+        stacc(q, L::kSoftness, sp.softness_impulse_scale);
+    }
+    template <class PR, class AR, class QR> BEPU_DI static void solve_projected(const Inertia& iA, PR p, AR a, QR q, Velocity& vA) {
+        V3 normal = ldrow3(p, L::kNormal);
+        float friction = ldrow(p, L::kFriction);
+        const float softness = ldacc(q, L::kSoftness);
+        V3 centerA;
+        float maximumTangentImpulse, maximumTwistImpulse;
+        if constexpr (N > 1) {
+            V3 offs[N];
+            float depths[N];
+#pragma unroll
+            for (int i = 0; i < N; ++i) { offs[i] = ldrow3(p, 4 * i); depths[i] = ldrow(p, 4 * i + 3); }
+            centerA = friction_center<N>(offs, depths);
+            float penSum = 0.0f, twistSum = 0.0f;
+#pragma unroll 1
+            for (int i = 0; i < N; ++i) {
+                V3 offset = ldrow3(p, 4 * i);
+                float pen = ldacc(a, 2 + i);
+                penetration1_solve_projected(iA, normal, offset, ldacc(q, L::kPenetrationMass + i), ldacc(q, L::kBiasVelocity + i), softness, pen, vA);
+                stacc(a, 2 + i, pen);
+                const float lever = pen * distance(centerA, offset);
+                penSum = i == 0 ? pen : penSum + pen;
+                twistSum = i == 0 ? lever : twistSum + lever;
+            }
+            const float premultiplied = (1.0f / N) * friction;
+            maximumTangentImpulse = premultiplied * penSum;
+            maximumTwistImpulse = premultiplied * twistSum;
+        } else {
+            centerA = ldrow3(p, 0);
+            float pen = ldacc(a, 2);
+            penetration1_solve_projected(iA, normal, centerA, ldacc(q, L::kPenetrationMass), ldacc(q, L::kBiasVelocity), softness, pen, vA);
+            stacc(a, 2, pen);
+            maximumTangentImpulse = friction * pen;
+            maximumTwistImpulse = friction * pen * fmax_ps(0.0f, ldrow(p, 3));
+        }
+        V3 x, z;
+        build_orthonormal_basis(normal, x, z);
+        V2 tangent{ldacc(a, 0), ldacc(a, 1)};
+        float twist = ldacc(a, N + 2);
+        tangent1_solve_projected(M23{x, z}, M23{cross(centerA, x), cross(centerA, z)}, Sym2{ldacc(q, L::kTangentMass), ldacc(q, L::kTangentMass + 1), ldacc(q, L::kTangentMass + 2)}, iA,
+                                 maximumTangentImpulse, tangent, vA);
+        twist1_solve_projected(normal, ldacc(q, L::kTwistMass), iA, maximumTwistImpulse, twist, vA);
+        stacc(a, 0, tangent.x);
+        stacc(a, 1, tangent.y);
+        stacc(a, N + 2, twist);
+    }
     BEPU_DI static void incremental_update(float dt, const Velocity& vA, float* p) {
         V3 normal = ldrow3(p, L::kNormal);
 #pragma unroll
diff --git a/bepuphysics2_b200/csrc/bepu_device_types.h b/bepuphysics2_b200/csrc/bepu_device_types.h
--- a/bepuphysics2_b200/csrc/bepu_device_types.h
+++ b/bepuphysics2_b200/csrc/bepu_device_types.h
@@ -70,11 +70,15 @@
     int32_t live_lanes;
 };
 
+constexpr int kProjectionStrideRows = 13;
+constexpr int32_t kConvexTypeCount = 8;
+
 struct StageOp {
     int32_t stage;
     int32_t work_begin;
     int32_t work_count;
     int32_t pad;
+    int32_t projected;
 };
 
 constexpr int kMaxShardRanks = 8;
diff --git a/bepuphysics2_b200/csrc/bepu_layout_kernels.h b/bepuphysics2_b200/csrc/bepu_layout_kernels.h
--- a/bepuphysics2_b200/csrc/bepu_layout_kernels.h
+++ b/bepuphysics2_b200/csrc/bepu_layout_kernels.h
@@ -52,7 +52,8 @@
 
 constexpr int kLaunchPdl = 1, kLaunchPrefetchRows = 2;
 struct SolverLaunchers {
-    void (*constraint_stage)(int stage, const WorkRecord* records, const int32_t* ref_rows, int work_count, const BodyBuffers& B, const FrameParams* fp, int launch_flags, cudaStream_t s);
+    void (*constraint_stage)(int stage, const WorkRecord* records, const int32_t* ref_rows, int work_count, const BodyBuffers& B, const FrameParams* fp, int launch_flags, float* projection,
+                             cudaStream_t s);
     void (*kinematic_stage)(int stage, const int32_t* kinematics, int count, const BodyBuffers& B, const FrameParams* fp, cudaStream_t s);
     void (*final_pose)(const BodyBuffers& B, const FrameParams* fp, cudaStream_t s);
     void (*constraint_stage_sharded)(int stage, const WorkRecord* records, const int32_t* ref_rows, int work_count, const BodyBuffers& B, const FrameParams* fp, int launch_flags, const ShardPeers& peers,
diff --git a/bepuphysics2_b200/csrc/bepu_solver_kernels.cu b/bepuphysics2_b200/csrc/bepu_solver_kernels.cu
--- a/bepuphysics2_b200/csrc/bepu_solver_kernels.cu
+++ b/bepuphysics2_b200/csrc/bepu_solver_kernels.cu
@@ -4,9 +4,9 @@
 
 namespace BEPU_NS {
 
-void launch_stage_warm_start_first(const WorkRecord* records, const int32_t* ref_rows, int work_count, const BodyBuffers& B, const FrameParams* fp, int launch_flags, cudaStream_t s);
-void launch_stage_warm_start(const WorkRecord* records, const int32_t* ref_rows, int work_count, const BodyBuffers& B, const FrameParams* fp, int launch_flags, cudaStream_t s);
-void launch_stage_solve(const WorkRecord* records, const int32_t* ref_rows, int work_count, const BodyBuffers& B, const FrameParams* fp, int launch_flags, cudaStream_t s);
+void launch_stage_warm_start_first(const WorkRecord* records, const int32_t* ref_rows, int work_count, const BodyBuffers& B, const FrameParams* fp, int launch_flags, float* projection, cudaStream_t s);
+void launch_stage_warm_start(const WorkRecord* records, const int32_t* ref_rows, int work_count, const BodyBuffers& B, const FrameParams* fp, int launch_flags, float* projection, cudaStream_t s);
+void launch_stage_solve(const WorkRecord* records, const int32_t* ref_rows, int work_count, const BodyBuffers& B, const FrameParams* fp, int launch_flags, float* projection, cudaStream_t s);
 void launch_stage_warm_start_first_sharded(const WorkRecord* records, const int32_t* ref_rows, int work_count, const BodyBuffers& B, const FrameParams* fp, int launch_flags, const ShardPeers& peers, long long peer_delta, const ShardStage& shard, cudaStream_t s);
 void launch_stage_warm_start_sharded(const WorkRecord* records, const int32_t* ref_rows, int work_count, const BodyBuffers& B, const FrameParams* fp, int launch_flags, const ShardPeers& peers, long long peer_delta, const ShardStage& shard, cudaStream_t s);
 void launch_stage_solve_sharded(const WorkRecord* records, const int32_t* ref_rows, int work_count, const BodyBuffers& B, const FrameParams* fp, int launch_flags, const ShardPeers& peers, long long peer_delta, const ShardStage& shard, cudaStream_t s);
@@ -16,12 +16,14 @@
 #endif
 constexpr int kDeepBatchBundles = 2150;
 template <int STAGE, int MINB>
-static void launch_stage_variant(const WorkRecord* records, const int32_t* ref_rows, int work_count, const BodyBuffers& B, const FrameParams* fp, int launch_flags, cudaStream_t s) {
+static void launch_stage_variant(const WorkRecord* records, const int32_t* ref_rows, int work_count, const BodyBuffers& B, const FrameParams* fp, int launch_flags, float* projection, cudaStream_t s) {
     static std::atomic<bool> carveout_set[64] = {};
     int device = 0;
     cudaGetDevice(&device);
     if (!carveout_set[device & 63]) {
         cudaFuncSetAttribute(constraint_stage_kernel<STAGE, MINB>, cudaFuncAttributePreferredSharedMemoryCarveout, cudaSharedmemCarveoutMaxShared);
+        if constexpr (STAGE != kStageIncremental)
+            cudaFuncSetAttribute(constraint_stage_kernel_projected<STAGE, MINB>, cudaFuncAttributePreferredSharedMemoryCarveout, cudaSharedmemCarveoutMaxShared);
         carveout_set[device & 63] = true;
     }
     const unsigned blocks = (unsigned)(((size_t)work_count * 32 + kStageBlockThreads - 1) / kStageBlockThreads);
@@ -35,7 +37,14 @@
     attr[0].val.programmaticStreamSerializationAllowed = 1;
     cfg.attrs = attr;
     cfg.numAttrs = (launch_flags & bepucuda::kLaunchPdl) ? 1 : 0;
-    cudaLaunchKernelEx(&cfg, constraint_stage_kernel<STAGE, MINB>, records, ref_rows, work_count, B, fp, (launch_flags & bepucuda::kLaunchPrefetchRows) ? kStagePrefetchRows : 0);
+    const int flags = (launch_flags & bepucuda::kLaunchPrefetchRows) ? kStagePrefetchRows : 0;
+    if constexpr (STAGE != kStageIncremental) {
+        if (projection) {
+            cudaLaunchKernelEx(&cfg, constraint_stage_kernel_projected<STAGE, MINB>, records, ref_rows, work_count, B, fp, flags, projection);
+            return;
+        }
+    }
+    cudaLaunchKernelEx(&cfg, constraint_stage_kernel<STAGE, MINB>, records, ref_rows, work_count, B, fp, flags);
 }
 template <int STAGE, int MINB>
 static void launch_stage_variant_sharded(const WorkRecord* records, const int32_t* ref_rows, int work_count, const BodyBuffers& B, const FrameParams* fp, int launch_flags, const ShardPeers& peers, long long peer_delta,
@@ -67,40 +76,40 @@
     else launch_stage_variant_sharded<STAGE, 1>(records, ref_rows, work_count, B, fp, launch_flags, peers, peer_delta, shard, s);
 }
 template <int STAGE>
-static void launch_stage_t(const WorkRecord* records, const int32_t* ref_rows, int work_count, const BodyBuffers& B, const FrameParams* fp, int launch_flags, cudaStream_t s) {
-    if (STAGE != kStageIncremental && work_count >= kDeepBatchBundles) launch_stage_variant<STAGE, BEPU_DEEP_MINB>(records, ref_rows, work_count, B, fp, launch_flags, s);
-    else launch_stage_variant<STAGE, 1>(records, ref_rows, work_count, B, fp, launch_flags, s);
+static void launch_stage_t(const WorkRecord* records, const int32_t* ref_rows, int work_count, const BodyBuffers& B, const FrameParams* fp, int launch_flags, float* projection, cudaStream_t s) {
+    if (STAGE != kStageIncremental && work_count >= kDeepBatchBundles) launch_stage_variant<STAGE, BEPU_DEEP_MINB>(records, ref_rows, work_count, B, fp, launch_flags, projection, s);
+    else launch_stage_variant<STAGE, 1>(records, ref_rows, work_count, B, fp, launch_flags, projection, s);
 }
 
 #if BEPU_UNIT == 0
-void launch_stage_warm_start_first(const WorkRecord* records, const int32_t* ref_rows, int work_count, const BodyBuffers& B, const FrameParams* fp, int launch_flags, cudaStream_t s) {
-    launch_stage_t<kStageWarmStartFirst>(records, ref_rows, work_count, B, fp, launch_flags, s);
+void launch_stage_warm_start_first(const WorkRecord* records, const int32_t* ref_rows, int work_count, const BodyBuffers& B, const FrameParams* fp, int launch_flags, float* projection, cudaStream_t s) {
+    launch_stage_t<kStageWarmStartFirst>(records, ref_rows, work_count, B, fp, launch_flags, projection, s);
 }
 void launch_stage_warm_start_first_sharded(const WorkRecord* records, const int32_t* ref_rows, int work_count, const BodyBuffers& B, const FrameParams* fp, int launch_flags, const ShardPeers& peers, long long peer_delta, const ShardStage& shard, cudaStream_t s) {
     launch_stage_sharded_t<kStageWarmStartFirst>(records, ref_rows, work_count, B, fp, launch_flags, peers, peer_delta, shard, s);
 }
 #elif BEPU_UNIT == 1
-void launch_stage_warm_start(const WorkRecord* records, const int32_t* ref_rows, int work_count, const BodyBuffers& B, const FrameParams* fp, int launch_flags, cudaStream_t s) {
-    launch_stage_t<kStageWarmStart>(records, ref_rows, work_count, B, fp, launch_flags, s);
+void launch_stage_warm_start(const WorkRecord* records, const int32_t* ref_rows, int work_count, const BodyBuffers& B, const FrameParams* fp, int launch_flags, float* projection, cudaStream_t s) {
+    launch_stage_t<kStageWarmStart>(records, ref_rows, work_count, B, fp, launch_flags, projection, s);
 }
 void launch_stage_warm_start_sharded(const WorkRecord* records, const int32_t* ref_rows, int work_count, const BodyBuffers& B, const FrameParams* fp, int launch_flags, const ShardPeers& peers, long long peer_delta, const ShardStage& shard, cudaStream_t s) {
     launch_stage_sharded_t<kStageWarmStart>(records, ref_rows, work_count, B, fp, launch_flags, peers, peer_delta, shard, s);
 }
 #elif BEPU_UNIT == 2
-void launch_stage_solve(const WorkRecord* records, const int32_t* ref_rows, int work_count, const BodyBuffers& B, const FrameParams* fp, int launch_flags, cudaStream_t s) {
-    launch_stage_t<kStageSolve>(records, ref_rows, work_count, B, fp, launch_flags, s);
+void launch_stage_solve(const WorkRecord* records, const int32_t* ref_rows, int work_count, const BodyBuffers& B, const FrameParams* fp, int launch_flags, float* projection, cudaStream_t s) {
+    launch_stage_t<kStageSolve>(records, ref_rows, work_count, B, fp, launch_flags, projection, s);
 }
 void launch_stage_solve_sharded(const WorkRecord* records, const int32_t* ref_rows, int work_count, const BodyBuffers& B, const FrameParams* fp, int launch_flags, const ShardPeers& peers, long long peer_delta, const ShardStage& shard, cudaStream_t s) {
     launch_stage_sharded_t<kStageSolve>(records, ref_rows, work_count, B, fp, launch_flags, peers, peer_delta, shard, s);
 }
 #elif BEPU_UNIT == 3
-static void launch_constraint_stage(int stage, const WorkRecord* records, const int32_t* ref_rows, int work_count, const BodyBuffers& B, const FrameParams* fp, int launch_flags, cudaStream_t s) {
+static void launch_constraint_stage(int stage, const WorkRecord* records, const int32_t* ref_rows, int work_count, const BodyBuffers& B, const FrameParams* fp, int launch_flags, float* projection, cudaStream_t s) {
     if (work_count <= 0) return;
     switch (stage) {
-        case kStageWarmStartFirst: launch_stage_warm_start_first(records, ref_rows, work_count, B, fp, launch_flags, s); break;
-        case kStageWarmStart: launch_stage_warm_start(records, ref_rows, work_count, B, fp, launch_flags, s); break;
-        case kStageSolve: launch_stage_solve(records, ref_rows, work_count, B, fp, launch_flags, s); break;
-        case kStageIncremental: launch_stage_t<kStageIncremental>(records, ref_rows, work_count, B, fp, launch_flags, s); break;
+        case kStageWarmStartFirst: launch_stage_warm_start_first(records, ref_rows, work_count, B, fp, launch_flags, projection, s); break;
+        case kStageWarmStart: launch_stage_warm_start(records, ref_rows, work_count, B, fp, launch_flags, projection, s); break;
+        case kStageSolve: launch_stage_solve(records, ref_rows, work_count, B, fp, launch_flags, projection, s); break;
+        case kStageIncremental: launch_stage_t<kStageIncremental>(records, ref_rows, work_count, B, fp, launch_flags, nullptr, s); break;
         default: break;
     }
 }
diff --git a/bepuphysics2_b200/csrc/bepu_solver_kernels.cuh b/bepuphysics2_b200/csrc/bepu_solver_kernels.cuh
--- a/bepuphysics2_b200/csrc/bepu_solver_kernels.cuh
+++ b/bepuphysics2_b200/csrc/bepu_solver_kernels.cuh
@@ -105,6 +105,14 @@
     else if constexpr (T::kBodies == 2) T::solve(b[0].inertia, b[1].inertia, dt, inverseDt, p, a, v[0], v[1]);
     else T::solve(b[0].inertia, dt, inverseDt, p, a, v[0]);
 }
+template <class T, class PR, class QR> BEPU_DI void call_project(const BodyState* b, float dt, float inverseDt, PR p, QR q) {
+    if constexpr (T::kBodies == 2) T::project(b[0].inertia, b[1].inertia, dt, inverseDt, p, q);
+    else T::project(b[0].inertia, dt, inverseDt, p, q);
+}
+template <class T, class PR, class AR, class QR> BEPU_DI void call_solve_projected(const BodyState* b, PR p, AR a, QR q, Velocity* v) {
+    if constexpr (T::kBodies == 2) T::solve_projected(b[0].inertia, b[1].inertia, p, a, q, v[0], v[1]);
+    else T::solve_projected(b[0].inertia, p, a, q, v[0]);
+}
 template <class T> BEPU_DI void call_incremental(float dt, const Velocity* v, float* p) {
     if constexpr (T::kIncremental) {
         if constexpr (T::kBodies == 2) T::incremental_update(dt, v[0], v[1], p);
@@ -112,6 +120,7 @@
     }
 }
 
+struct NoProjection {};
 BEPU_DI uint32_t ldg_nc_u32(const void* p) {
     uint32_t v;
     asm volatile("ld.global.nc.u32 %0, [%1];" : "=r"(v) : "l"(p));
@@ -126,9 +135,9 @@
         dst[1] = make_float4(e, f, g, h);
     }
 }
-template <class T, int STAGE, bool kSharded, class PR, class AR>
+template <class T, int STAGE, bool kSharded, bool kProjected = false, class PR, class AR, class QR = NoProjection>
 BEPU_DI void run_lane(const int32_t* refs, PR p, AR a, float* p_rw, uint32_t enc0, uint32_t enc1, const BodyBuffers& B, const FrameParams& fp, const ShardPeers* peers = nullptr,
-                      long long peer_delta = 0) {
+                      long long peer_delta = 0, QR q = QR{}) {
     constexpr int NB = T::kBodies;
     uint32_t enc[NB];
     enc[0] = enc0;
@@ -156,7 +165,8 @@
             if (T::kNeedsPose) load_pose(B.pose, idx, b[s].pos, b[s].q);
         }
         rows_ready(p);
-        call_solve<T>(b, fp.dt, fp.inverse_dt, p, a, v);
+        if constexpr (kProjected) call_solve_projected<T>(b, p, a, q, v);
+        else call_solve<T>(b, fp.dt, fp.inverse_dt, p, a, v);
 #pragma unroll
         for (int s = 0; s < NB; ++s)
             if (!(enc[s] & kRefKinematicBit)) {
@@ -170,6 +180,7 @@
 #pragma unroll
         for (int s = 0; s < NB; ++s) gather_for_warm_start<STAGE, T::kNeedsPose>(enc[s], B, fp, b[s], v[s]);
         rows_ready(p);
+        if constexpr (kProjected) call_project<T>(b, fp.dt, fp.inverse_dt, p, q);
         call_warm_start<T>(b, p, a, v);
 #pragma unroll
         for (int s = 0; s < NB; ++s)
@@ -211,9 +222,11 @@
     return w;
 }
 
+#define BEPU_CONVEX_TYPES(X)                                                                                                      \
+    X(0, ConvexOneBody<1>) X(1, ConvexOneBody<2>) X(2, ConvexOneBody<3>) X(3, ConvexOneBody<4>)                                   \
+    X(4, ConvexTwoBody<1>) X(5, ConvexTwoBody<2>) X(6, ConvexTwoBody<3>) X(7, ConvexTwoBody<4>)
 #define BEPU_CONTACT_TYPES(X)                                                                                                     \
-    X(0, ConvexOneBody<1>) X(1, ConvexOneBody<2>) X(2, ConvexOneBody<3>) X(3, ConvexOneBody<4>)                                   \
-    X(4, ConvexTwoBody<1>) X(5, ConvexTwoBody<2>) X(6, ConvexTwoBody<3>) X(7, ConvexTwoBody<4>)                                   \
+    BEPU_CONVEX_TYPES(X)                                                                                                          \
     X(8, NonconvexOneBody<2>) X(9, NonconvexOneBody<3>) X(10, NonconvexOneBody<4>)                                                \
     X(15, NonconvexTwoBody<2>) X(16, NonconvexTwoBody<3>) X(17, NonconvexTwoBody<4>)
 
@@ -236,6 +249,18 @@
 BEPU_DI void run_bundle_rows(const WorkRecord& rec, int lane, PR p, AR a, uint32_t enc0, uint32_t enc1, const BodyBuffers& B, const FrameParams& fp) {
     run_bundle_rows<STAGE, false>(rec, lane, p, a, enc0, enc1, B, fp);
 }
+template <int STAGE, class PR, class AR, class QR>
+BEPU_DI void run_bundle_rows_projected(const WorkRecord& rec, int lane, PR p, AR a, QR q, uint32_t enc0, uint32_t enc1, const BodyBuffers& B, const FrameParams& fp) {
+    const int32_t* refs = rec.refs + lane;
+    float* p_rw = rec.prestep + lane;
+    switch (rec.type_id) {
+#define BEPU_CASE(ID, T) \
+    case ID: run_lane<T, STAGE, false, true>(refs, p, a, p_rw, enc0, enc1, B, fp, nullptr, 0, q); break;
+        BEPU_CONVEX_TYPES(BEPU_CASE)
+#undef BEPU_CASE
+        default: break;
+    }
+}
 template <int STAGE>
 BEPU_DI void run_bundle(const WorkRecord& rec, int lane, uint32_t enc0, uint32_t enc1, const BodyBuffers& B, const FrameParams& fp) {
     run_bundle_rows<STAGE>(rec, lane, GlobalRows{rec.prestep + lane}, GlobalAcc{rec.impulses + lane}, enc0, enc1, B, fp);
@@ -245,7 +270,7 @@
     run_bundle<STAGE>(rec, lane, enc0, enc1, B, fp);
 }
 
-struct StageRowCounts { uint8_t prestep[64], impulses[64]; };
+struct StageRowCounts { uint8_t prestep[64], impulses[64], projection[64]; };
 __host__ __device__ constexpr StageRowCounts make_stage_row_counts() {
     StageRowCounts c{};
 #define BEPU_ROWS(ID, T) c.prestep[ID] = (uint8_t)T::kPrestepRows; c.impulses[ID] = (uint8_t)T::kImpulseRows;
@@ -253,11 +278,19 @@
     BEPU_JOINT_TYPES(BEPU_ROWS)
     BEPU_JOINT_TYPES_MORE(BEPU_ROWS)
 #undef BEPU_ROWS
+#define BEPU_ROWS(ID, T) c.projection[ID] = (uint8_t)T::L::kProjectionRows;
+    BEPU_CONVEX_TYPES(BEPU_ROWS)
+#undef BEPU_ROWS
     return c;
 }
 __constant__ StageRowCounts kStageRowCounts = make_stage_row_counts();
 constexpr int kStageSlabRows = 48;
 constexpr int kStageSlabBytes = kStageSlabRows * kLanes * 4;
+#define BEPU_CHECK(ID, T)                                                                                                                     \
+    static_assert(T::kPrestepRows + T::kImpulseRows + T::L::kProjectionRows <= kStageSlabRows, "projected Solve block exceeds the slab");    \
+    static_assert(T::L::kProjectionRows <= kProjectionStrideRows && ID < kConvexTypeCount, "projection arena layout");
+BEPU_CONVEX_TYPES(BEPU_CHECK)
+#undef BEPU_CHECK
 
 BEPU_DI uint32_t smem_u32(const void* p) { return (uint32_t)__cvta_generic_to_shared(p); }
 BEPU_DI void mbar_init(uint32_t bar, uint32_t count) {
@@ -301,9 +334,10 @@
     }
     __syncwarp();
 }
-template <int STAGE, bool kSharded>
+template <int STAGE, bool kSharded, bool kProjected = false>
 BEPU_DI void constraint_stage_body(const WorkRecord* __restrict__ records, const int32_t* __restrict__ ref_rows, int work_count, const BodyBuffers& B, const FrameParams* __restrict__ fpp, int flags, const ShardPeers* peers,
-                                   long long peer_delta, const ShardStage* shard = nullptr) {
+                                   long long peer_delta, const ShardStage* shard = nullptr, float* __restrict__ projection = nullptr) {
+    static_assert(!(kProjected && (kSharded || STAGE == kStageIncremental)), "projected stages: WarmStart / Solve, single GPU");
     constexpr bool kStaged = STAGE != kStageIncremental;
     constexpr int kWarps = kStageBlockThreads / 32;
     __shared__ __align__(128) float slab[kStaged ? kWarps * kStageSlabRows * kLanes : 1];
@@ -318,19 +352,22 @@
     const uint32_t slab_addr = kStaged ? smem_u32(slab) + warp_in_block * kStageSlabBytes : 0;
     const uint32_t bar = smem_u32(&bars[warp_in_block]);
     const bool early_rows = kStaged && (flags & kStagePrefetchRows);
-    uint32_t prestep_bytes = 0, impulse_bytes = 0;
+    uint32_t prestep_bytes = 0, impulse_bytes = 0, projection_bytes = 0;
+    float* const projection_rows = kProjected ? projection + (size_t)warp * (kProjectionStrideRows * kLanes) : nullptr;
     if (active) {
         rec = load_record(records + warp);
         if constexpr (kStaged) {
             prestep_bytes = kStageRowCounts.prestep[rec.type_id] * (kLanes * 4);
             impulse_bytes = kStageRowCounts.impulses[rec.type_id] * (kLanes * 4);
+            if constexpr (kProjected && STAGE == kStageSolve) projection_bytes = kStageRowCounts.projection[rec.type_id] * (kLanes * 4);
             if (lane == 0) {
                 mbar_init(bar, 1);
                 if (early_rows) {
                     const uint64_t policy = l2_evict_first_policy();
-                    mbar_expect_tx(bar, prestep_bytes + impulse_bytes);
+                    mbar_expect_tx(bar, prestep_bytes + impulse_bytes + projection_bytes);
                     bulk_copy_g2s(slab_addr, rec.prestep, prestep_bytes, bar, policy);
                     bulk_copy_g2s(slab_addr + prestep_bytes, rec.impulses, impulse_bytes, bar, policy);
+                    if (projection_bytes) bulk_copy_g2s(slab_addr + prestep_bytes + impulse_bytes, projection_rows, projection_bytes, bar, policy);
                 }
             }
         }
@@ -349,11 +386,19 @@
     if constexpr (kStaged) {
         if (!early_rows && lane == 0) {
             const uint64_t policy = l2_evict_first_policy();
-            mbar_expect_tx(bar, prestep_bytes + impulse_bytes);
+            mbar_expect_tx(bar, prestep_bytes + impulse_bytes + projection_bytes);
             bulk_copy_g2s(slab_addr, rec.prestep, prestep_bytes, bar, policy);
             bulk_copy_g2s(slab_addr + prestep_bytes, rec.impulses, impulse_bytes, bar, policy);
+            if (projection_bytes) bulk_copy_g2s(slab_addr + prestep_bytes + impulse_bytes, projection_rows, projection_bytes, bar, policy);
         }
         __syncwarp();
+        if constexpr (kProjected) {
+            const StagedRows p{slab_addr + lane * 4, bar, 0u};
+            const StagedAcc a{slab_addr + prestep_bytes + lane * 4, rec.impulses + lane};
+            if constexpr (STAGE == kStageSolve) run_bundle_rows_projected<STAGE>(rec, lane, p, a, StagedAcc{slab_addr + prestep_bytes + impulse_bytes + lane * 4, nullptr}, enc0, enc1, B, fp);
+            else run_bundle_rows_projected<STAGE>(rec, lane, p, a, ProjectionOut{projection_rows + lane}, enc0, enc1, B, fp);
+            return;
+        }
         run_bundle_rows<STAGE, kSharded>(rec, lane, StagedRows{slab_addr + lane * 4, bar, 0u}, StagedAcc{slab_addr + prestep_bytes + lane * 4, rec.impulses + lane}, enc0, enc1, B, fp,
                                          peers, boundary && !(fp.tune[0] & 4) ? peer_delta : 0);
         if constexpr (kSharded) {
@@ -370,6 +415,12 @@
 template <int STAGE, int MINB>
 __global__ void __launch_bounds__(kStageBlockThreads, MINB) constraint_stage_kernel(const WorkRecord* __restrict__ records, const int32_t* __restrict__ ref_rows, int work_count, BodyBuffers B, const FrameParams* __restrict__ fpp, int flags) {
     constraint_stage_body<STAGE, false>(records, ref_rows, work_count, B, fpp, flags, nullptr, 0);
+}
+template <int STAGE, int MINB>
+__global__ void __launch_bounds__(kStageBlockThreads, MINB)
+constraint_stage_kernel_projected(const WorkRecord* __restrict__ records, const int32_t* __restrict__ ref_rows, int work_count, BodyBuffers B, const FrameParams* __restrict__ fpp, int flags,
+                                  float* __restrict__ projection) {
+    constraint_stage_body<STAGE, false, true>(records, ref_rows, work_count, B, fpp, flags, nullptr, 0, nullptr, projection);
 }
 template <int STAGE, int MINB>
 __global__ void __launch_bounds__(kStageBlockThreads, MINB)
diff --git a/bepuphysics2_b200/csrc/bepucuda_api.cu b/bepuphysics2_b200/csrc/bepucuda_api.cu
--- a/bepuphysics2_b200/csrc/bepucuda_api.cu
+++ b/bepuphysics2_b200/csrc/bepucuda_api.cu
@@ -152,13 +152,14 @@
     bool constraints_open = false, constraints_ready = false, data_dirty = false, descs_dirty = false;
     std::vector<SourceTypeBatch> sources;
     ChunkArena raw_arena, pinned_arena;
-    DeviceBuffer record_table, ref_rows, source_bundle_flags, refs32, prestep32, impulses32, tb_table, tdesc_table, work_table, map_table, bodies_per_type, kinematics_dev, program_dev, frame_params_dev, error_dev;
+    DeviceBuffer record_table, ref_rows, source_bundle_flags, refs32, prestep32, impulses32, projection, tb_table, tdesc_table, work_table, map_table, bodies_per_type, kinematics_dev, program_dev, frame_params_dev, error_dev;
     std::vector<DeviceTypeBatch> tbs;
     std::vector<TransposeDesc> tdescs;
     std::vector<WorkItem> work;
     std::vector<int32_t> bundle_live;
     std::vector<WorkRecord> records;
     std::vector<std::pair<int, int>> batch_work;
+    std::vector<uint8_t> batch_projected;
     bool exchange_failed = false;
     bepucuda_exchange_fn exchange = nullptr;
     void* exchange_user = nullptr;
@@ -288,6 +289,10 @@
     ctx->graph_valid = false;
 }
 
+float* projection_rows(bepucuda_ctx* ctx, const StageOp& op) {
+    return op.projected ? ctx->projection.as<float>() + (size_t)op.work_begin * kProjectionStrideRows * 32 : nullptr;
+}
+
 void issue_stage_sequence(bepucuda_ctx* ctx, cudaStream_t s, int64_t* launches) {
     const WorkRecord* records = ctx->record_table.as<WorkRecord>();
     const int32_t* ref_rows = ctx->ref_rows.as<int32_t>();
@@ -317,7 +322,7 @@
                     previous = &op;
                     continue;
                 }
-                ctx->launchers->constraint_stage(op.stage, records + op.work_begin, ref_rows + (size_t)op.work_begin * 64, op.work_count, ctx->B, fp, launch_flags, s);
+                ctx->launchers->constraint_stage(op.stage, records + op.work_begin, ref_rows + (size_t)op.work_begin * 64, op.work_count, ctx->B, fp, launch_flags, nullptr, s);
                 ++n;
             }
             if (fused_pushes) { ++exchange_index; continue; }
@@ -334,7 +339,7 @@
                     bool prefetch = op.stage != kStageIncremental && previous != nullptr && previous->stage != kStageIncremental;
                     if (prefetch && previous->stage <= kStageSolve && previous->work_begin == op.work_begin) prefetch = false;
                     if (ctx->exchange) {
-                        ctx->launchers->constraint_stage(op.stage, records + op.work_begin, ref_rows + (size_t)op.work_begin * 64, op.work_count, ctx->B, fp, 0, s);
+                        ctx->launchers->constraint_stage(op.stage, records + op.work_begin, ref_rows + (size_t)op.work_begin * 64, op.work_count, ctx->B, fp, 0, nullptr, s);
                         ++n;
                         if (op.stage != kStageIncremental) {
                             const int planes = op.stage == kStageSolve ? 1 : (op.stage == kStageWarmStart ? 3 : 2);
@@ -349,7 +354,8 @@
                         previous = &op;
                         break;
                     }
-                    ctx->launchers->constraint_stage(op.stage, records + op.work_begin, ref_rows + (size_t)op.work_begin * 64, op.work_count, ctx->B, fp, (pdl ? kLaunchPdl : 0) | (prefetch ? kLaunchPrefetchRows : 0), s);
+                    ctx->launchers->constraint_stage(op.stage, records + op.work_begin, ref_rows + (size_t)op.work_begin * 64, op.work_count, ctx->B, fp, (pdl ? kLaunchPdl : 0) | (prefetch ? kLaunchPrefetchRows : 0),
+                                                     projection_rows(ctx, op), s);
                     previous = &op;
                     ++n;
                 }
@@ -381,12 +387,13 @@
         if (ctx->peer_mode) ctx->program.push_back({kStageKinematic, 0, 0, -1});
         for (size_t b = 0; b < ctx->batch_work.size(); ++b) {
             auto& bw = ctx->batch_work[b];
-            if (bw.second > 0 || (ctx->peer_mode && (int)b < ctx->sync_batch_count)) ctx->program.push_back({s == 0 ? kStageWarmStartFirst : kStageWarmStart, bw.first, bw.second, ctx->peer_mode ? (int)b + 2 : 0});
+            if (bw.second > 0 || (ctx->peer_mode && (int)b < ctx->sync_batch_count))
+                ctx->program.push_back({s == 0 ? kStageWarmStartFirst : kStageWarmStart, bw.first, bw.second, ctx->peer_mode ? (int)b + 2 : 0, ctx->batch_projected[b]});
         }
         for (int it = 0; it < ctx->iterations[s]; ++it)
             for (size_t b = 0; b < ctx->batch_work.size(); ++b) {
                 auto& bw = ctx->batch_work[b];
-                if (bw.second > 0 || (ctx->peer_mode && (int)b < ctx->sync_batch_count)) ctx->program.push_back({kStageSolve, bw.first, bw.second, ctx->peer_mode ? (int)b + 2 : 0});
+                if (bw.second > 0 || (ctx->peer_mode && (int)b < ctx->sync_batch_count)) ctx->program.push_back({kStageSolve, bw.first, bw.second, ctx->peer_mode ? (int)b + 2 : 0, ctx->batch_projected[b]});
             }
     }
     if (ctx->peer_mode) ctx->program.push_back({kStageKinematic, 0, 0, -1});
@@ -529,7 +536,7 @@
     invalidate_graph(ctx);
     for (void* p : ctx->opened_ipc) cudaIpcCloseMemHandle(p);
     DeviceBuffer* bufs[] = {&ctx->shard_flags, &ctx->pushes_dev, &ctx->peer32, &ctx->body_masks_dev, &ctx->boundary_flags_dev, &ctx->raw_bodies, &ctx->pose, &ctx->velocity, &ctx->inertia_local, &ctx->inertia_world, &ctx->constrained, &ctx->first_batch, &ctx->sync_refcount,
-                            &ctx->sync_mask, &ctx->chunk_table, &ctx->record_table, &ctx->ref_rows, &ctx->body_shapes, &ctx->body_activities, &ctx->body_bounds, &ctx->color_refs, &ctx->color_priorities, &ctx->color_body_min, &ctx->color_body_mask, &ctx->color_out, &ctx->color_lists, &ctx->color_counts, &ctx->source_bundle_flags, &ctx->refs32, &ctx->prestep32, &ctx->impulses32, &ctx->tb_table, &ctx->tdesc_table, &ctx->work_table, &ctx->map_table,
+                            &ctx->sync_mask, &ctx->chunk_table, &ctx->record_table, &ctx->ref_rows, &ctx->body_shapes, &ctx->body_activities, &ctx->body_bounds, &ctx->color_refs, &ctx->color_priorities, &ctx->color_body_min, &ctx->color_body_mask, &ctx->color_out, &ctx->color_lists, &ctx->color_counts, &ctx->source_bundle_flags, &ctx->refs32, &ctx->prestep32, &ctx->impulses32, &ctx->projection, &ctx->tb_table, &ctx->tdesc_table, &ctx->work_table, &ctx->map_table,
                             &ctx->bodies_per_type, &ctx->kinematics_dev, &ctx->program_dev, &ctx->frame_params_dev, &ctx->error_dev, &ctx->exchange_staging};
     for (auto b : bufs) b->release();
     ctx->raw_arena.release();
@@ -885,6 +892,16 @@
         if (get_type_info(ctx->tbs[tb].type_id)->incremental)
             for (int k = 0; k < ctx->tbs[tb].bundle_count; ++k) { ctx->work.push_back({(int)tb, k}); ctx->bundle_live.push_back(live_in_bundle((int)tb, k)); }
     ctx->inc_work_count = (int)ctx->work.size() - ctx->inc_work_begin;
+    ctx->batch_projected.assign(batch_tbs.size(), 0);
+    bool any_projected = false;
+    if (!ctx->exchange && !ctx->peer_mode)
+        for (size_t b = (size_t)ctx->sync_batch_count; b < batch_tbs.size(); ++b) {
+            bool convex = !batch_tbs[b].empty();
+            for (int tb : batch_tbs[b]) convex = convex && ctx->tbs[tb].type_id < kConvexTypeCount;
+            ctx->batch_projected[b] = convex;
+            any_projected |= convex;
+        }
+    if (any_projected) CK(ctx->projection.reserve((size_t)ctx->all_work_count * kProjectionStrideRows * 32 * 4));
 
     ctx->records.resize(ctx->work.size());
     for (size_t i = 0; i < ctx->work.size(); ++i) {
@@ -1333,7 +1350,7 @@
         const bool has_work = op.stage == kStageFinalPose ? ctx->B.count > 0 : op.work_count > 0;
         if (!has_work) continue;
         CK(cudaEventRecord(ctx->profile_events[2 * i], ctx->stream));
-        if (op.stage <= kStageIncremental) ctx->launchers->constraint_stage(op.stage, records + op.work_begin, ref_rows + (size_t)op.work_begin * 64, op.work_count, ctx->B, fp, 0, ctx->stream);
+        if (op.stage <= kStageIncremental) ctx->launchers->constraint_stage(op.stage, records + op.work_begin, ref_rows + (size_t)op.work_begin * 64, op.work_count, ctx->B, fp, 0, projection_rows(ctx, op), ctx->stream);
         else if (op.stage <= kStageKinematic) ctx->launchers->kinematic_stage(op.stage, kin, op.work_count, ctx->B, fp, ctx->stream);
         else ctx->launchers->final_pose(ctx->B, fp, ctx->stream);
         CK(cudaEventRecord(ctx->profile_events[2 * i + 1], ctx->stream));
```

Result: no change. 2.012 billion, median of 6 (+0.1%).
